# xaskasdf/ntransformer

Measured on AMD Instinct MI355X. Metric: decode tokens/sec (Llama-3.1-8B Q8_0 class, resident weights, greedy, batch 1), higher is better.
Workload: dtype f32; 1 GPU; Llama-3.1-8B-shaped Q8_0 GGUF tensors (seed 20260925), resident in HBM, 16-token prompt, greedy decode; ctx=4096, replicas=1, hipgraph=True

## Files before the change

### include/ntk_engine.h

```cpp
#ifndef NTK_ENGINE_H
#define NTK_ENGINE_H

#include "ntk.h"

#if defined(__GNUC__)
#pragma GCC visibility push(default)
#endif
#ifdef __cplusplus
extern "C" {
#endif

int ntk_rope_kv_store(float* q, const float* k, const float* v, const int* positions, int seq_len, int n_heads, int n_kv_heads, int head_dim,
                      float theta_base, float freq_scale, int interleaved, void* k_cache, void* v_cache, int start_pos, int max_seq, void* stream);
int ntk_rope_tab(float* q, float* k, const int* positions, int batch_size, int seq_len, int n_heads, int n_kv_heads, int head_dim, float theta_base,
                 float freq_scale, int interleaved, const float* inv_freq, void* stream);
int ntk_rope_kv_store_tab(float* q, const float* k, const float* v, const int* positions, int seq_len, int n_heads, int n_kv_heads, int head_dim,
                          float theta_base, float freq_scale, int interleaved, void* k_cache, void* v_cache, int start_pos, int max_seq,
                          const float* inv_freq, void* stream);
typedef struct ntk_gemv_seg {
    const void* W;
    float*      y;
    int         rows;
    int         dtype;
} ntk_gemv_seg;
// ... 17 lines not shown
#define NTK_ARENA_GATE 3
#define NTK_ARENA_HIDDEN_FLOATS 8192
#define NTK_ARENA_ATTN_FLOATS 8192
#define NTK_ARENA_GATE_FLOATS 32768
int ntk_decode_arena_acquire(void);
void ntk_decode_arena_release(int device);
float* ntk_decode_arena_slot(int slot);
int ntk_debug_gemv_static_x(void);

int ntk_debug_rp_prologue(uint8_t* out, const float* x, const float* norm_w, float eps, int in_features, int nsub, int nwaves, void* stream);
int ntk_debug_mfma_i8_probe(int* D, const int8_t* A, const int8_t* B, void* stream);

int ntk_attention_decode_fused(float* output, const float* q, const float* k, const float* v, void* k_cache,
                               void* v_cache, const int* d_pos, const float* inv_freq, int n_heads, int n_kv_heads,
                               int head_dim, int max_seq, float scale, float theta_base, float freq_scale,
                               void* stream);

size_t ntk_attention_split_scratch_bytes(int n_heads, int head_dim, int nsplit);
int ntk_attention_decode_split(float* output, const float* q, const float* k, const float* v, void* k_cache,
                               void* v_cache, const int* d_pos, const float* inv_freq, int n_heads, int n_kv_heads,
                               int head_dim, int max_seq, float scale, float theta_base, float freq_scale, int nsplit,
                               float* scratch, void* stream);
int ntk_attention_split_scratch_init(float* scratch, int n_heads, void* stream);
int ntk_attention_decode_split_merged(float* output, const float* q, const float* k, const float* v, void* k_cache,
                                      void* v_cache, const int* d_pos, const float* inv_freq, int n_heads, int n_kv_heads,
                                      int head_dim, int max_seq, float scale, float theta_base, float freq_scale, int nsplit,
                                      float* scratch, void* stream);

#define NTK_ATTN_BATCH_MAX 16
typedef struct ntk_kv_batch {
    void* k[NTK_ATTN_BATCH_MAX];
    void* v[NTK_ATTN_BATCH_MAX];
} ntk_kv_batch;
int ntk_attention_decode_batch(float* output, const float* q, const float* k, const float* v, const ntk_kv_batch* caches, const int* positions,
                               int n_rows, const float* inv_freq, int n_heads, int n_kv_heads, int head_dim, int max_seq, float scale,
                               float theta_base, float freq_scale, int nsplit, float* scratch, void* stream);

typedef struct ntk_kv_segments {
    int   n_seg;
    int   row0[NTK_ATTN_BATCH_MAX];
    int   n_rows[NTK_ATTN_BATCH_MAX];
    int   start_pos[NTK_ATTN_BATCH_MAX];
    void* k[NTK_ATTN_BATCH_MAX];
    void* v[NTK_ATTN_BATCH_MAX];
} ntk_kv_segments;
int ntk_kv_segments_validate(const ntk_kv_segments* segs, int total_rows, int max_seq);
int ntk_rope_kv_store_segments(float* q, const float* k, const float* v, const ntk_kv_segments* segs, int n_heads, int n_kv_heads, int head_dim,
                               float theta_base, float freq_scale, int interleaved, int max_seq, void* stream);
int ntk_rope_kv_store_segments_tab(float* q, const float* k, const float* v, const ntk_kv_segments* segs, int n_heads, int n_kv_heads, int head_dim,
                                   float theta_base, float freq_scale, int interleaved, int max_seq, const float* inv_freq, void* stream);
int ntk_attention_prefill_segments(float* output, const float* Q, const ntk_kv_segments* segs, int n_heads, int n_kv_heads, int head_dim, int max_seq,
                                   float scale, void* stream);

size_t ntk_kv_q8_cache_bytes(int max_seq, int n_kv_heads, int head_dim);
int ntk_kv_store_q8(void* k_cache, void* v_cache, const float* k, const float* v, int seq_len, int n_kv_heads, int head_dim, int start_pos,
                    int max_seq, void* stream);
int ntk_rope_kv_store_q8(float* q, const float* k, const float* v, const int* positions, int seq_len, int n_heads, int n_kv_heads, int head_dim,
                         float theta_base, float freq_scale, int interleaved, void* k_cache, void* v_cache, int start_pos, int max_seq,
                         void* stream);
int ntk_rope_kv_store_q8_tab(float* q, const float* k, const float* v, const int* positions, int seq_len, int n_heads, int n_kv_heads, int head_dim,
                             float theta_base, float freq_scale, int interleaved, void* k_cache, void* v_cache, int start_pos, int max_seq,
                             const float* inv_freq, void* stream);
int ntk_attention_decode_q8(float* output, const float* q, const float* k, const float* v, void* k_cache, void* v_cache, const int* d_pos,
                            const float* inv_freq, int n_heads, int n_kv_heads, int head_dim, int max_seq, float scale, float theta_base,
                            float freq_scale, int nsplit, float* scratch, void* stream);
int ntk_kv_dequant_q8_f16(void* k_f16, void* v_f16, const void* k_cache, const void* v_cache, int n_rows, int n_kv_heads, int head_dim,
                          int max_seq, void* stream);
int ntk_attention_decode_q8_batch(float* output, const float* q, const float* k, const float* v, const ntk_kv_batch* caches, const int* positions,
                                  int n_rows, const float* inv_freq, int n_heads, int n_kv_heads, int head_dim, int max_seq, float scale,
                                  float theta_base, float freq_scale, int nsplit, float* scratch, void* stream);

int ntk_kv_shift(uint16_t* k_cache, uint16_t* v_cache, int n_layers, int max_seq, int n_kv_heads, int head_dim, int src0, int dst0, int n_rows,
                 const float* inv_freq, float theta_base, float freq_scale, int interleaved, void* stream);
int ntk_kv_shift_q8(void* k_cache_q8, void* v_cache_q8, int n_layers, int max_seq, int n_kv_heads, int head_dim, int src0, int dst0, int n_rows,
                    const float* inv_freq, float theta_base, float freq_scale, int interleaved, void* stream);

int ntk_debug_gemv_fused_form(const ntk_gemv_seg* segs, int nseg, const float* x, int in_features, const float* norm_w, float eps,
                              const float* resid, int silu_pair, int integer_activations, void* stream);

size_t   ntk_tp_comm_bytes(size_t max_floats);
void*    ntk_tp_comm_alloc(size_t bytes);
int      ntk_tp_comm_reset(void* comm, void* stream);
float*   ntk_tp_slot(void* comm, size_t max_floats, unsigned call_index);
int      ntk_tp_allreduce_add(float* hidden, void* const* peers, int rank, int world, size_t max_floats, unsigned call_index, int n, void* stream);
int      ntk_tp_advance_epoch(void* comm, void* stream);
unsigned ntk_tp_error(void* comm);
int      ntk_ipc_export(void* devptr, void* handle64);
int      ntk_ipc_open(const void* handle64, void** devptr);
int      ntk_ipc_close(void* devptr);

int ntk_gemm_quant(float* Y, const void* W, const float* X, int n_tokens, int out_features, int in_features,
                   int weight_dtype, const float* resid, void* stream);

typedef struct ntk_gemm_partials {
    const float* part[3];
    float*       y[3];
    int          rows[3];
    int          nseg, n_tokens, nsplit;
} ntk_gemm_partials;
typedef struct ntk_gemm_desc {
    const ntk_gemv_seg* segs;
    int                 nseg;
    const float*        X;
    int                 n_tokens, in_features;
    const float*        resid;
    void*               workspace;
    size_t              workspace_bytes;
    int                 reuse_x;
    const float*        row_max;
    ntk_gemm_partials*  partials;
    int                 weights_repacked;
    int                 full_form;
} ntk_gemm_desc;
size_t ntk_gemm_quant_workspace_bytes(int in_features, int out_features);
int ntk_gemm_quant_f16(const ntk_gemm_desc* desc, void* stream);
int ntk_reduce_rmsnorm_rowmax(float* hidden, const ntk_gemm_partials* partials, const float* weight, float eps, float* x_out, float* row_max,
                              float* zero_tokens, void* stream);
int ntk_reduce_silu_mul_rowmax(float* output, const ntk_gemm_partials* partials, float* row_max, void* stream);
int ntk_rmsnorm_rowmax(float* output, const float* input, const float* weight, int n_tokens, int hidden_size, float eps, float* row_max,
                       float* zero_tokens, void* stream);
int ntk_silu_mul_rowmax(float* output, const float* gate, const float* up, int n_tokens, int width, float* row_max, void* stream);
int ntk_gemm_prepare_x(const float* X, int n_tokens, int in_features, void* workspace, void* stream);
int ntk_rmsnorm_prepare_x(float* output, const float* input, const float* weight, int n_tokens, int hidden_size, float eps, void* workspace, void* stream);
int ntk_reduce_rmsnorm_prepare_x(float* hidden, const ntk_gemm_partials* partials, const float* weight, float eps, float* x_out, void* workspace, void* stream);
int ntk_silu_mul_prepare_x(float* output, const float* gate, const float* up, int n_tokens, int width, void* workspace, void* stream);
int ntk_reduce_silu_mul_prepare_x(float* output, const ntk_gemm_partials* partials, void* workspace, void* stream);

size_t ntk_gemm_dense16_workspace_bytes(int in_features, int out_features, int dtype);
int ntk_gemm_dense16(const ntk_gemm_desc* desc, void* stream);

int ntk_embed_rows(float* out, const void* table, const int* tokens, int n_tokens, int hidden, int dtype,
                   void* stream);

int ntk_argmax(const float* logits, int n, int* d_out_token, int* h_mirror, float* scratch, void* stream);

int ntk_logprob_rows(const float* logits, int n_rows, int vocab, int ld, const int* targets, float* logprob, int* top1, void* stream);

size_t ntk_sample_scratch_bytes(int n);
int ntk_sample_top_k(float* logits, int n, const int* d_recent, int n_recent, float repeat_penalty, float temperature,
                     int top_k, float top_p, float r, int* d_out_token, int* h_mirror, void* scratch, void* stream);
int ntk_repeat_penalty(float* logits, int n, const int* d_recent, int n_recent, float repeat_penalty, void* stream);

#define NTK_SAMPLE_ROWS_MAX 16
typedef struct ntk_sample_rows {
    float temperature[NTK_SAMPLE_ROWS_MAX], top_p[NTK_SAMPLE_ROWS_MAX], repeat_penalty[NTK_SAMPLE_ROWS_MAX], r[NTK_SAMPLE_ROWS_MAX];
    int   top_k[NTK_SAMPLE_ROWS_MAX], n_recent[NTK_SAMPLE_ROWS_MAX];
} ntk_sample_rows;
size_t ntk_sample_rows_scratch_bytes(int n_rows, int vocab);
int ntk_sample_rows_top_k(float* logits, int n_rows, int vocab, int ld, const int* d_recent, int recent_ld, const ntk_sample_rows* rows, int* d_out,
                          int* h_mirror, void* scratch, void* stream);

int ntk_argmax_advance(const float* logits, int n, int* d_out_token, int* h_mirror, unsigned long long* h_ring4, int* d_pos,
                       float* scratch, void* stream);

int ntk_debug_sclk(unsigned long long* d_out2, void* stream);
int ntk_debug_sclk_begin(unsigned* d_flag, unsigned long long* d_out2, void* side_stream);
int ntk_debug_sclk_end(unsigned* d_flag, void* other_stream);

void ntk_debug_malloc_budget(long long bytes);

int ntk_advance_pos(int* d_pos, void* stream);

#ifdef __cplusplus
}
#endif
#if defined(__GNUC__)
#pragma GCC visibility pop
#endif
#endif
```

### ntransformer_amd/csrc/common.hip.h

```cpp
#pragma once
#include <hip/hip_runtime.h>
#include <stdint.h>
#include "../../include/ntk_engine.h"

#define NTK_WAVE 64

#define NTK_HIP_TRY(expr)                                   \
    do {                                                    \
        hipError_t e__ = (expr);                            \
        if (e__ != hipSuccess) return NTK_E_LAUNCH;         \
    } while (0)

#define NTK_EXTRA_API extern "C" __attribute__((visibility("default")))
#ifdef NTK_TUNE
#include <cstdlib>
#define NTK_TUNE_ENV_INT(name, dflt) ([] { const char* e__ = getenv(name); return e__ ? atoi(e__) : (dflt); }())
#else
#define NTK_TUNE_ENV_INT(name, dflt) (dflt)
#endif

namespace ntk {

hipStream_t resolve_stream(void* s);
int         last_launch_status();
int         q8l_gemv_fused(const ntk_gemv_seg* segs, int nseg, const float* x, int in, const float* norm_w, float eps, const float* resid,
                           int silu_pair, hipStream_t st);
int         dense16_gemv_fused(const ntk_gemv_seg* segs, int nseg, const float* x, int in, const float* norm_w, float eps, const float* resid,
                               int silu_pair, hipStream_t st);

__device__ __forceinline__ float h2f(uint16_t bits) {
    _Float16 h;
    __builtin_memcpy(&h, &bits, 2);
    return (float)h;
}
__device__ __forceinline__ uint16_t f2h(float f) {
    _Float16 h = (_Float16)f;
    uint16_t bits;
    __builtin_memcpy(&bits, &h, 2);
    return bits;
}

__device__ __forceinline__ void rope_rotate(const float a, const float b, const float c, const float s, float& ra, float& rb) {
#pragma clang fp contract(off)
    ra = a * c - b * s;
    rb = b * c + a * s;
}

__device__ __forceinline__ float rope_freq(const float* __restrict__ inv_freq, const int i, const int head_dim, const float theta) {
    return inv_freq ? inv_freq[i] : 1.0f / (float)pow((double)theta, (double)((2.0f * i) / head_dim));
}

template <int CTRL, int ROW_MASK>
__device__ __forceinline__ float dpp_or_zero(float v) {
    return __int_as_float(__builtin_amdgcn_update_dpp(0, __float_as_int(v), CTRL, ROW_MASK, 0xF, false));
}
template <int CTRL, int ROW_MASK>
__device__ __forceinline__ float dpp_or_self(float v) {
    return __int_as_float(__builtin_amdgcn_update_dpp(__float_as_int(v), __float_as_int(v), CTRL, ROW_MASK, 0xF, false));
}
constexpr int DPP_QUAD_1032 = 0xB1, DPP_QUAD_2301 = 0x4E, DPP_ROW_HALF_MIRROR = 0x141, DPP_ROW_MIRROR = 0x140,
              DPP_ROW_BCAST15 = 0x142, DPP_ROW_BCAST31 = 0x143;

__device__ __forceinline__ float wave_sum_lane63(float v) {
    v += dpp_or_zero<DPP_QUAD_1032, 0xF>(v);
    v += dpp_or_zero<DPP_QUAD_2301, 0xF>(v);
    v += dpp_or_zero<DPP_ROW_HALF_MIRROR, 0xF>(v);
    v += dpp_or_zero<DPP_ROW_MIRROR, 0xF>(v);
    v += dpp_or_zero<DPP_ROW_BCAST15, 0xA>(v);
    v += dpp_or_zero<DPP_ROW_BCAST31, 0xC>(v);
    return v;
}
__device__ __forceinline__ float wave_sum(float v) {
    return __int_as_float(__builtin_amdgcn_readlane(__float_as_int(wave_sum_lane63(v)), 63));
}
__device__ __forceinline__ float wave_max(float v) {
    v = fmaxf(v, dpp_or_self<DPP_QUAD_1032, 0xF>(v));
    v = fmaxf(v, dpp_or_self<DPP_QUAD_2301, 0xF>(v));
    v = fmaxf(v, dpp_or_self<DPP_ROW_HALF_MIRROR, 0xF>(v));
    v = fmaxf(v, dpp_or_self<DPP_ROW_MIRROR, 0xF>(v));
    v = fmaxf(v, dpp_or_self<DPP_ROW_BCAST15, 0xA>(v));
    v = fmaxf(v, dpp_or_self<DPP_ROW_BCAST31, 0xC>(v));
    return __int_as_float(__builtin_amdgcn_readlane(__float_as_int(v), 63));
}

template <int N>
__device__ __forceinline__ float group_sum(float v) {
    static_assert(N == 1 || N == 2 || N == 4 || N == 8 || N == 16 || N == 32, "group size");
    if constexpr (N >= 2) v += dpp_or_zero<DPP_QUAD_1032, 0xF>(v);
    if constexpr (N >= 4) v += dpp_or_zero<DPP_QUAD_2301, 0xF>(v);
    if constexpr (N >= 8) v += dpp_or_zero<DPP_ROW_HALF_MIRROR, 0xF>(v);
    if constexpr (N >= 16) v += dpp_or_zero<DPP_ROW_MIRROR, 0xF>(v);
    if constexpr (N >= 32) v += __shfl_xor(v, 16, 64);
    return v;
}

__device__ __forceinline__ float block_sum(float v, float* red) {
    const int lane = threadIdx.x & 63, wave = threadIdx.x >> 6, nw = (blockDim.x + 63) >> 6;
    v = wave_sum(v);
    __syncthreads();
    if (lane == 0) red[wave] = v;
    __syncthreads();
    float t = 0.0f;
    for (int i = 0; i < nw; ++i) t += red[i];
    return t;
}
__device__ __forceinline__ float block_max(float v, float* red) {
    const int lane = threadIdx.x & 63, wave = threadIdx.x >> 6, nw = (blockDim.x + 63) >> 6;
    v = wave_max(v);
    __syncthreads();
    if (lane == 0) red[wave] = v;
    __syncthreads();
    float t = red[0];
    for (int i = 1; i < nw; ++i) t = fmaxf(t, red[i]);
    return t;
}

template <int N>
__device__ __forceinline__ void lds_read_dwords(uint32_t (&dst)[N], const uint8_t* base, int off) {
    const int a = off & ~3;
    const uint32_t sh = (uint32_t)(off & 3);
    uint32_t w[N + 1];
#pragma unroll
    for (int i = 0; i <= N; ++i) w[i] = *reinterpret_cast<const uint32_t*>(base + a + 4 * i);
#pragma unroll
    for (int i = 0; i < N; ++i) dst[i] = __builtin_amdgcn_alignbyte(w[i + 1], w[i], sh);
}
__device__ __forceinline__ uint16_t lds_u16_at(const uint8_t* base, int off) {
    return *reinterpret_cast<const uint16_t*>(base + off);
}

__device__ __forceinline__ float ub2f(uint32_t w, int k) { return (float)((w >> (8 * k)) & 0xFFu); }
__device__ __forceinline__ float sb2f(uint32_t w, int k) { return (float)(int)(int8_t)(w >> (8 * k)); }

__device__ __forceinline__ void kq_scale_min(uint32_t s0, uint32_t s1, uint32_t s2, int j, float& sc, float& mn) {
    const uint64_t lo = (uint64_t)s0 | ((uint64_t)s1 << 32);
    auto byte = [&](int n) -> uint32_t {
        return n < 8 ? (uint32_t)((lo >> (8 * n)) & 0xFFu) : ((s2 >> (8 * (n - 8))) & 0xFFu);
    };
    uint32_t s, m;
    if (j < 4) {
        s = byte(j) & 63u;
        m = byte(j + 4) & 63u;
    } else {
        s = (byte(j + 4) & 0xFu) | ((byte(j - 4) >> 6) << 4);
        m = (byte(j + 4) >> 4) | ((byte(j) >> 6) << 4);
    }
    sc = (float)s;
    mn = (float)m;
}

}
```

### ntransformer_amd/csrc/elementwise.hip

```cpp
#include "common.hip.h"
#include <cfloat>

namespace ntk {

template <bool HALF_OUT>
__global__ __launch_bounds__(1024) void rmsnorm_kernel(void* __restrict__ output, const float* __restrict__ input,
                                                       const float* __restrict__ weight, int hidden, float eps) {
    __shared__ float red[16];
    const float* x = input + (size_t)blockIdx.x * hidden;
    float ssq = 0.0f;
    for (int i = threadIdx.x; i < hidden; i += blockDim.x) ssq = fmaf(x[i], x[i], ssq);
    const float tot = block_sum(ssq, red);
    const float rms_inv = 1.0f / sqrtf(tot / (float)hidden + eps);
    for (int i = threadIdx.x; i < hidden; i += blockDim.x) {
        const float v = x[i] * rms_inv * weight[i];
        if constexpr (HALF_OUT) reinterpret_cast<uint16_t*>(output)[(size_t)blockIdx.x * hidden + i] = f2h(v);
        else reinterpret_cast<float*>(output)[(size_t)blockIdx.x * hidden + i] = v;
    }
}

template <bool MASKED>
__global__ __launch_bounds__(1024) void softmax_kernel(float* __restrict__ out, const float* __restrict__ in,
                                                       const uint8_t* __restrict__ mask, int cols) {
    __shared__ float red[16];
    const float* x = in + (size_t)blockIdx.x * cols;
    const uint8_t* mk = MASKED ? mask + (size_t)blockIdx.x * cols : nullptr;
    float* y = out + (size_t)blockIdx.x * cols;
    float m = -FLT_MAX;
    for (int i = threadIdx.x; i < cols; i += blockDim.x)
        if (!MASKED || mk[i]) m = fmaxf(m, x[i]);
    m = block_max(m, red);
    float l = 0.0f;
    for (int i = threadIdx.x; i < cols; i += blockDim.x)
        if (!MASKED || mk[i]) l += expf(x[i] - m);
    l = block_sum(l, red);
    const float inv = l > 0.0f ? 1.0f / l : 0.0f;
    for (int i = threadIdx.x; i < cols; i += blockDim.x) y[i] = (!MASKED || mk[i]) ? expf(x[i] - m) * inv : 0.0f;
}

__global__ void silu_mul_kernel(float* __restrict__ out, const float* __restrict__ gate, const float* __restrict__ up, int n) {
    const int i = blockIdx.x * blockDim.x + threadIdx.x;
    if (i < n) {
        const float g = gate[i];
        out[i] = g / (1.0f + expf(-g)) * up[i];
    }
}
__global__ void add_kernel(float* __restrict__ o, const float* __restrict__ a, const float* __restrict__ b, int n) {
    const int i = blockIdx.x * blockDim.x + threadIdx.x;
    if (i < n) o[i] = a[i] + b[i];
}
__global__ void copy_kernel(float* __restrict__ d, const float* __restrict__ s, int n) {
    const int i = blockIdx.x * blockDim.x + threadIdx.x;
    if (i < n) d[i] = s[i];
}
__global__ void gemm_f32_kernel(float* __restrict__ C, const float* __restrict__ A, const float* __restrict__ B, int M, int N, int K) {
    const int col = blockIdx.x * blockDim.x + threadIdx.x, row = blockIdx.y * blockDim.y + threadIdx.y;
    if (row >= M || col >= N) return;
    float s = 0.0f;
    for (int k = 0; k < K; ++k) s = fmaf(A[(size_t)row * K + k], B[(size_t)col * K + k], s);
    C[(size_t)row * N + col] = s;
}
__global__ __launch_bounds__(256) void cosine_kernel(float* __restrict__ result, const float* __restrict__ a,
                                                     const float* __restrict__ b, int n) {
    __shared__ float red[16];
    float d = 0.0f, na = 0.0f, nb = 0.0f;
    for (int i = threadIdx.x; i < n; i += blockDim.x) {
        d = fmaf(a[i], b[i], d); na = fmaf(a[i], a[i], na); nb = fmaf(b[i], b[i], nb);
    }
    d = block_sum(d, red); na = block_sum(na, red); nb = block_sum(nb, red);
    if (threadIdx.x == 0) {
        const float den = sqrtf(na) * sqrtf(nb);
        *result = den > 1e-8f ? d / den : 0.0f;
    }
}

__device__ float embed_elem(const uint8_t* __restrict__ table, int tok, int hidden, int dt, int e) {
    switch (dt) {
        case NTK_DT_F32: return reinterpret_cast<const float*>(table)[(size_t)tok * hidden + e];
        case NTK_DT_F16: return h2f(reinterpret_cast<const uint16_t*>(table)[(size_t)tok * hidden + e]);
        case NTK_DT_BF16: return __uint_as_float((uint32_t)reinterpret_cast<const uint16_t*>(table)[(size_t)tok * hidden + e] << 16);
        case NTK_DT_Q8_0: {
            const uint8_t* b = table + ((size_t)tok * (hidden / 32) + e / 32) * 34;
            const float d = h2f((uint16_t)(b[0] | (b[1] << 8)));
            return __fmul_rn(d, (float)(int8_t)b[2 + (e & 31)]);
        }
        case NTK_DT_Q4_0: {
            const uint8_t* b = table + ((size_t)tok * (hidden / 32) + e / 32) * 18;
            const float d = h2f((uint16_t)(b[0] | (b[1] << 8)));
            const int j = e & 31;
            const int nib = j < 16 ? (b[2 + j] & 0x0F) : (b[2 + j - 16] >> 4);
            return __fmul_rn(d, (float)(nib - 8));
        }
        case NTK_DT_Q4_K: {
            const uint8_t* b = table + ((size_t)tok * (hidden / 256) + e / 256) * 144;
            const float d = h2f((uint16_t)(b[0] | (b[1] << 8))), dmin = h2f((uint16_t)(b[2] | (b[3] << 8)));
            const int w = e & 255, sub = w >> 5, l = w & 31, chunk = sub >> 1;
            const uint8_t* s = b + 4;
            uint32_t sc, mn;
            if (sub < 4) { sc = s[sub] & 63; mn = s[sub + 4] & 63; }
            else { sc = (s[sub + 4] & 0x0F) | ((s[sub - 4] >> 6) << 4); mn = (s[sub + 4] >> 4) | ((s[sub] >> 6) << 4); }
            const uint8_t qb = b[16 + 32 * chunk + l];
            const int nib = (sub & 1) ? (qb >> 4) : (qb & 0x0F);
            return __fsub_rn(__fmul_rn(__fmul_rn(d, (float)sc), (float)nib), __fmul_rn(dmin, (float)mn));
        }
        case NTK_DT_Q6_K: {
            const uint8_t* b = table + ((size_t)tok * (hidden / 256) + e / 256) * 210;
            const float d = h2f((uint16_t)(b[208] | (b[209] << 8)));
            const int w = e & 255, hf = w >> 7, g = (w >> 5) & 3, l = w & 31, is = l >> 4;
            const uint8_t* ql = b + 64 * hf;
            const uint8_t* qh = b + 128 + 32 * hf;
            const int8_t sc = (int8_t)b[192 + 8 * hf + is + 2 * g];
            const uint8_t qlb = ql[l + 32 * (g & 1)];
            const int lo = (g >> 1) ? (qlb >> 4) : (qlb & 0x0F);
            const int q = (lo | (((qh[l] >> (2 * g)) & 3) << 4)) - 32;
            return __fmul_rn(__fmul_rn(d, (float)sc), (float)q);
        }
        default: return 0.0f;
    }
}
__global__ void embed_rows_kernel(float* __restrict__ out, const uint8_t* __restrict__ table, const int* __restrict__ tokens,
                                  int hidden, int dt) {
    const int tok = tokens[blockIdx.x];
    const int e = blockIdx.y * blockDim.x + threadIdx.x;
    if (e < hidden) out[(size_t)blockIdx.x * hidden + e] = embed_elem(table, tok, hidden, dt, e);
}

__device__ __forceinline__ void amax_merge(float& v, int& i, float ov, int oi) {
    if (ov > v || (ov == v && oi < i)) { v = ov; i = oi; }
}
__global__ __launch_bounds__(256) void argmax_stage1(const float* __restrict__ x, int n, float* __restrict__ sv, int* __restrict__ si) {
    __shared__ float rv[4];
    __shared__ int ri[4];
    float v = -FLT_MAX;
    int idx = 0x7FFFFFFF;
    for (int i = blockIdx.x * blockDim.x + threadIdx.x; i < n; i += gridDim.x * blockDim.x) amax_merge(v, idx, x[i], i);
    for (int off = 32; off > 0; off >>= 1) amax_merge(v, idx, __shfl_xor(v, off, 64), __shfl_xor(idx, off, 64));
    if ((threadIdx.x & 63) == 0) { rv[threadIdx.x >> 6] = v; ri[threadIdx.x >> 6] = idx; }
    __syncthreads();
    if (threadIdx.x == 0) {
        for (int w = 1; w < 4; ++w) amax_merge(v, idx, rv[w], ri[w]);
        sv[blockIdx.x] = v; si[blockIdx.x] = idx;
    }
}
__global__ __launch_bounds__(256) void argmax_stage2(const float* __restrict__ sv, const int* __restrict__ si, int nblk,
                                                     int* __restrict__ d_out, int* __restrict__ h_mirror) {
    __shared__ float rv[4];
    __shared__ int ri[4];
    float v = -FLT_MAX;
    int idx = 0x7FFFFFFF;
    for (int i = threadIdx.x; i < nblk; i += blockDim.x) amax_merge(v, idx, sv[i], si[i]);
    for (int off = 32; off > 0; off >>= 1) amax_merge(v, idx, __shfl_xor(v, off, 64), __shfl_xor(idx, off, 64));
    if ((threadIdx.x & 63) == 0) { rv[threadIdx.x >> 6] = v; ri[threadIdx.x >> 6] = idx; }
    __syncthreads();
    if (threadIdx.x == 0) {
        for (int w = 1; w < 4; ++w) amax_merge(v, idx, rv[w], ri[w]);
        if (idx == 0x7FFFFFFF) idx = 0;
        *d_out = idx;
        if (h_mirror) *h_mirror = idx;
    }
}
__global__ void advance_pos_kernel(int* p) { if (threadIdx.x == 0 && blockIdx.x == 0) *p += 1; }

__global__ __launch_bounds__(64) void sclk_probe_kernel(unsigned long long* out) {
    const unsigned long long t0 = __builtin_amdgcn_s_memtime(), r0 = __builtin_amdgcn_s_memrealtime();
    unsigned long long r1 = r0;
    float acc = (float)threadIdx.x;
    while (r1 - r0 < 5000ull) {
#pragma unroll
        for (int i = 0; i < 64; ++i) acc = fmaf(acc, 1.0000001f, 1e-9f);
        r1 = __builtin_amdgcn_s_memrealtime();
    }
    const unsigned long long t1 = __builtin_amdgcn_s_memtime();
    if (threadIdx.x == 0) { out[0] = t1 - t0; out[1] = r1 - r0; }
    if (acc == 12345.678f) out[2] = 0;
}

__global__ __launch_bounds__(64) void sclk_span_kernel(const unsigned* flag, unsigned long long* out) {
    const unsigned long long t0 = __builtin_amdgcn_s_memtime(), r0 = __builtin_amdgcn_s_memrealtime();
    unsigned long long r1 = r0;
    for (;;) {
        __builtin_amdgcn_s_sleep(64);
        r1 = __builtin_amdgcn_s_memrealtime();
        if (__hip_atomic_load(flag, __ATOMIC_RELAXED, __HIP_MEMORY_SCOPE_SYSTEM) != 0u || r1 - r0 > 300000000ull) break;
    }
    const unsigned long long t1 = __builtin_amdgcn_s_memtime();
    if (threadIdx.x == 0) { out[0] = t1 - t0; out[1] = r1 - r0; }
}

__global__ __launch_bounds__(256) void argmax_advance_stage2(const float* __restrict__ sv, const int* __restrict__ si, int nblk,
                                                             int* __restrict__ d_out, int* __restrict__ h_mirror,
                                                             unsigned long long* __restrict__ h_ring, int* __restrict__ d_pos) {
    __shared__ float rv[4];
    __shared__ int ri[4];
    float v = -FLT_MAX;
    int idx = 0x7FFFFFFF;
    for (int i = threadIdx.x; i < nblk; i += blockDim.x) amax_merge(v, idx, sv[i], si[i]);
    for (int off = 32; off > 0; off >>= 1) amax_merge(v, idx, __shfl_xor(v, off, 64), __shfl_xor(idx, off, 64));
    if ((threadIdx.x & 63) == 0) { rv[threadIdx.x >> 6] = v; ri[threadIdx.x >> 6] = idx; }
    __syncthreads();
    if (threadIdx.x == 0) {
        for (int w = 1; w < 4; ++w) amax_merge(v, idx, rv[w], ri[w]);
        if (idx == 0x7FFFFFFF) idx = 0;
        const int pos = *d_pos;
        *d_out = idx;
        if (h_mirror) *h_mirror = idx;
        if (h_ring)
            __hip_atomic_store(h_ring + (pos & 3), (unsigned long long)(unsigned)idx | ((unsigned long long)(unsigned)(pos + 1) << 32),
                               __ATOMIC_RELEASE, __HIP_MEMORY_SCOPE_SYSTEM);
        *d_pos = pos + 1;
    }
}

static inline dim3 g1(int n) { return dim3((n + 255) / 256); }

}

extern "C" {
using namespace ntk;

static int rms_block(int hidden) { return hidden <= 1024 ? 256 : (hidden <= 4096 ? 512 : 1024); }

int ntk_rmsnorm(float* output, const float* input, const float* weight, int batch_size, int hidden_size, float eps, void* stream) {
    if (!output || !input || !weight) return NTK_E_NULL;
    if (batch_size < 0 || hidden_size <= 0) return NTK_E_SHAPE;
    if (batch_size == 0) return NTK_OK;
    hipLaunchKernelGGL(rmsnorm_kernel<false>, dim3(batch_size), dim3(rms_block(hidden_size)), 0, resolve_stream(stream),
                       (void*)output, input, weight, hidden_size, eps);
    return last_launch_status();
}
int ntk_rmsnorm_f16(void* output, const float* input, const float* weight, int batch_size, int hidden_size, float eps, void* stream) {
    if (!output || !input || !weight) return NTK_E_NULL;
    if (batch_size < 0 || hidden_size <= 0) return NTK_E_SHAPE;
    if (batch_size == 0) return NTK_OK;
    hipLaunchKernelGGL(rmsnorm_kernel<true>, dim3(batch_size), dim3(rms_block(hidden_size)), 0, resolve_stream(stream),
                       output, input, weight, hidden_size, eps);
    return last_launch_status();
}
int ntk_softmax(float* output, const float* input, int rows, int cols, void* stream) {
    if (!output || !input) return NTK_E_NULL;
    if (rows < 0 || cols <= 0) return NTK_E_SHAPE;
    if (rows == 0) return NTK_OK;
    hipLaunchKernelGGL(softmax_kernel<false>, dim3(rows), dim3(cols <= 1024 ? 256 : 1024), 0, resolve_stream(stream), output,
                       input, (const uint8_t*)nullptr, cols);
    return last_launch_status();
}
int ntk_masked_softmax(float* output, const float* input, const uint8_t* mask, int rows, int cols, void* stream) {
    if (!output || !input || !mask) return NTK_E_NULL;
    if (rows < 0 || cols <= 0) return NTK_E_SHAPE;
    if (rows == 0) return NTK_OK;
    hipLaunchKernelGGL(softmax_kernel<true>, dim3(rows), dim3(cols <= 1024 ? 256 : 1024), 0, resolve_stream(stream), output,
                       input, mask, cols);
    return last_launch_status();
}
int ntk_gemm_f32(float* C, const float* A, const float* B, int M, int N, int K, void* stream) {
    if (!C || !A || !B) return NTK_E_NULL;
    if (M < 0 || N < 0 || K < 0) return NTK_E_SHAPE;
    if (M == 0 || N == 0) return NTK_OK;
    hipLaunchKernelGGL(gemm_f32_kernel, dim3((N + 15) / 16, (M + 15) / 16), dim3(16, 16), 0, resolve_stream(stream), C, A, B, M, N, K);
    return last_launch_status();
}
int ntk_silu_mul(float* output, const float* gate, const float* up, int size, void* stream) {
    if (!output || !gate || !up) return NTK_E_NULL;
    if (size < 0) return NTK_E_SHAPE;
    if (size == 0) return NTK_OK;
    hipLaunchKernelGGL(silu_mul_kernel, g1(size), dim3(256), 0, resolve_stream(stream), output, gate, up, size);
    return last_launch_status();
}
int ntk_add(float* out, const float* a, const float* b, int size, void* stream) {
    if (!out || !a || !b) return NTK_E_NULL;
    if (size < 0) return NTK_E_SHAPE;
    if (size == 0) return NTK_OK;
    hipLaunchKernelGGL(add_kernel, g1(size), dim3(256), 0, resolve_stream(stream), out, a, b, size);
    return last_launch_status();
}
int ntk_add_inplace(float* a, const float* b, int size, void* stream) { return ntk_add(a, a, b, size, stream); }
int ntk_add_bias(float* y, const float* bias, int size, void* stream) { return ntk_add(y, y, bias, size, stream); }
int ntk_copy(float* dst, const float* src, int size, void* stream) {
    if (!dst || !src) return NTK_E_NULL;
    if (size < 0) return NTK_E_SHAPE;
    if (size == 0) return NTK_OK;
    hipLaunchKernelGGL(copy_kernel, g1(size), dim3(256), 0, resolve_stream(stream), dst, src, size);
    return last_launch_status();
}
int ntk_cosine_similarity(float* result, const float* a, const float* b, int size, void* stream) {
    if (!result || !a || !b) return NTK_E_NULL;
    if (size < 0) return NTK_E_SHAPE;
    hipLaunchKernelGGL(cosine_kernel, dim3(1), dim3(256), 0, resolve_stream(stream), result, a, b, size);
    return last_launch_status();
}
int ntk_embed_rows(float* out, const void* table, const int* tokens, int n_tokens, int hidden, int dtype, void* stream) {
    if (!out || !table || !tokens) return NTK_E_NULL;
    if (n_tokens < 0 || hidden <= 0) return NTK_E_SHAPE;
    if (n_tokens == 0) return NTK_OK;
    hipLaunchKernelGGL(embed_rows_kernel, dim3(n_tokens, (hidden + 255) / 256), dim3(256), 0, resolve_stream(stream), out, (const uint8_t*)table,
                       tokens, hidden, dtype);
    const int st = last_launch_status();
    if (st != NTK_OK) return st;
    switch (dtype) {
        case NTK_DT_F32: case NTK_DT_F16: case NTK_DT_BF16: case NTK_DT_Q8_0: case NTK_DT_Q4_0: case NTK_DT_Q4_K: case NTK_DT_Q6_K: return NTK_OK;
        default: return NTK_E_DTYPE;
    }
}
int ntk_argmax(const float* logits, int n, int* d_out_token, int* h_mirror, float* scratch, void* stream) {
    if (!logits || !d_out_token || !scratch) return NTK_E_NULL;
    if (n <= 0) return NTK_E_SHAPE;
    const int nblk = n < 256 * 8 ? 1 : (n / (256 * 8) < 1024 ? n / (256 * 8) : 1024);
    float* sv = scratch;
    int* si = reinterpret_cast<int*>(scratch + 1024);
    hipStream_t st = resolve_stream(stream);
    hipLaunchKernelGGL(argmax_stage1, dim3(nblk), dim3(256), 0, st, logits, n, sv, si);
    hipLaunchKernelGGL(argmax_stage2, dim3(1), dim3(256), 0, st, (const float*)sv, (const int*)si, nblk, d_out_token, h_mirror);
    return last_launch_status();
}
int ntk_argmax_advance(const float* logits, int n, int* d_out_token, int* h_mirror, unsigned long long* h_ring4, int* d_pos, float* scratch,
                       void* stream) {
    if (!logits || !d_out_token || !scratch || !d_pos) return NTK_E_NULL;
    if (n <= 0) return NTK_E_SHAPE;
    const int nblk = n < 256 * 8 ? 1 : (n / (256 * 8) < 1024 ? n / (256 * 8) : 1024);
    float* sv = scratch;
    int* si = reinterpret_cast<int*>(scratch + 1024);
    hipStream_t st = resolve_stream(stream);
    hipLaunchKernelGGL(argmax_stage1, dim3(nblk), dim3(256), 0, st, logits, n, sv, si);
    hipLaunchKernelGGL(argmax_advance_stage2, dim3(1), dim3(256), 0, st, (const float*)sv, (const int*)si, nblk, d_out_token, h_mirror, h_ring4, d_pos);
    return last_launch_status();
}
int ntk_debug_sclk(unsigned long long* d_out2, void* stream) {
    if (!d_out2) return NTK_E_NULL;
    hipLaunchKernelGGL(sclk_probe_kernel, dim3(1), dim3(64), 0, resolve_stream(stream), d_out2);
    return last_launch_status();
}
int ntk_debug_sclk_begin(unsigned* d_flag, unsigned long long* d_out2, void* side_stream) {
    if (!d_flag || !d_out2 || !side_stream) return NTK_E_NULL;
    hipStream_t st = static_cast<hipStream_t>(side_stream);
    if (hipMemsetAsync(d_flag, 0, 4, st) != hipSuccess) return NTK_E_LAUNCH;
    hipLaunchKernelGGL(sclk_span_kernel, dim3(1), dim3(64), 0, st, (const unsigned*)d_flag, d_out2);
    return last_launch_status();
}
int ntk_debug_sclk_end(unsigned* d_flag, void* other_stream) {
    if (!d_flag || !other_stream) return NTK_E_NULL;
    static const unsigned one = 1u;
    return hipMemcpyAsync(d_flag, &one, 4, hipMemcpyHostToDevice, static_cast<hipStream_t>(other_stream)) == hipSuccess ? NTK_OK : NTK_E_LAUNCH;
}
int ntk_advance_pos(int* d_pos, void* stream) {
    if (!d_pos) return NTK_E_NULL;
    hipLaunchKernelGGL(advance_pos_kernel, dim3(1), dim3(64), 0, resolve_stream(stream), d_pos);
    return last_launch_status();
}

}
```

### ntransformer_amd/csrc/engine/capi.cpp

```cpp
#include "../../../include/ntransformer.h"
#include "../../../include/ntk_engine.h"
#include "engine.h"

#include <cstdlib>
#include <cstring>
#include <new>
#include <thread>

using nt::Engine;

namespace {
Engine* E(nt_engine_t e) { return static_cast<Engine*>(e); }
nt::SynthSpec to_spec(const nt_synth_spec& s) {
    nt::SynthSpec o;
    o.hidden = s.hidden; o.inter = s.inter; o.layers = s.layers; o.heads = s.heads; o.kv_heads = s.kv_heads;
    o.vocab = s.vocab; o.ctx = s.ctx; o.eps = s.eps; o.theta = s.theta; o.bos = s.bos; o.eos = s.eos;
    o.mix = s.mix ? s.mix : "Q8_0";
    o.seed = s.seed;
    return o;
}
int threads_or_default(int n) {
    if (n > 0) return n;
    const int h = (int)std::thread::hardware_concurrency();
    return h > 0 ? h : 8;
}
}

extern "C" {

nt_engine_t nt_engine_create(void) { return new (std::nothrow) Engine(); }
void nt_engine_destroy(nt_engine_t e) { delete E(e); }

int nt_engine_load(nt_engine_t e, const char* path) { return nt_engine_load_ex(e, path, 4096); }

int nt_engine_load_ex(nt_engine_t e, const char* path, int max_context) {
    if (!e || !path) return NTK_E_NULL;
    try { return E(e)->load(path, max_context > 0 ? max_context : 4096); } catch (...) { return NTK_E_NOMEM; }
}

int nt_engine_load_synthetic(nt_engine_t e, const nt_synth_spec* spec, int max_context) {
    if (!e || !spec) return NTK_E_NULL;
    try { return E(e)->load_synthetic(to_spec(*spec), max_context > 0 ? max_context : 4096); } catch (...) { return NTK_E_NOMEM; }
}

int nt_engine_load_shared(nt_engine_t e, nt_engine_t src, int max_context) {
    if (!e || !src || e == src) return NTK_E_NULL;
    try { return E(e)->load_shared(*E(src), max_context > 0 ? max_context : 4096); } catch (...) { return NTK_E_NOMEM; }
}

int nt_engine_set_option(nt_engine_t e, const char* key, const char* value) {
    if (!e || !key || !value) return NTK_E_NULL;
    const bool on = atoi(value) != 0;
    const std::string k = key;
    auto before_load = [&](auto set) -> int {
        if (E(e)->loaded()) { E(e)->set_error(k + " must be set before the model is loaded"); return NTK_E_SHAPE; }
        const int rc = set();
        if (rc != NTK_OK) E(e)->set_error(E(e)->model().error());
        return rc;
    };
    if (k == "fused") E(e)->options().fused = on;
    else if (k == "graph") E(e)->options().graph = on;
    else if (k == "batched_prefill") { E(e)->options().batched_prefill = on; E(e)->model().set_batched_prefill(on); }
    else if (k == "device_sampling") E(e)->options().device_sampling = on;
    else if (k == "f16_prefill" || k == "bf16_prefill") E(e)->model().set_bf16_prefill(on);
    else if (k == "dense_fused") {
        const std::string v = value;
        if (v != "0" && v != "1") { E(e)->set_error("dense_fused must be 0 or 1"); return NTK_E_SHAPE; }
        return E(e)->model().set_dense_fused(on);
    }
    else if (k == "dense_mfma16") {
        const std::string v = value;
        if (v != "0" && v != "1") { E(e)->set_error("dense_mfma16 must be 0 or 1"); return NTK_E_SHAPE; }
        E(e)->model().set_dense_mfma16(on);
    }
    else if (k == "persistent" || k == "fuse_attention") {
        if (on) fprintf(stderr, "note: \"%s\" selected an experiment that lost to the fused launches and was removed (profiles/NEGATIVE_RESULTS.md); the option does nothing\n", key);
    }
    else if (k == "kv_cache") return before_load([&] { return E(e)->model().set_kv_cache(value); });
    else if (k == "rope_scaling") return before_load([&] { return E(e)->model().set_rope_scaling(value); });
    else if (k == "rope_freq_base") return before_load([&] { return E(e)->model().set_rope_freq_base(value); });
    else if (k == "rope_freq_scale") return before_load([&] { return E(e)->model().set_rope_freq_scale(value); });
    else if (k == "sequences") return before_load([&] { return E(e)->model().set_sequences(atoi(value)); });
    else if (k == "batch_kv_q8") {
        const std::string v = value;
        if (v != "0" && v != "1") { E(e)->set_error("batch_kv_q8 must be 0 or 1"); return NTK_E_SHAPE; }
        return before_load([&] { return E(e)->model().set_batch_kv_q8(on); });
    }
    else if (k == "static_activations") {
        const std::string v = value;
        if (v != "0" && v != "1") { E(e)->set_error("static_activations must be 0 or 1"); return NTK_E_SHAPE; }
        return before_load([&] { return E(e)->model().set_static_activations(on); });
    }
    else if (k == "batch_prefill") {
        const std::string v = value;
        if (v != "0" && v != "1") { E(e)->set_error("batch_prefill must be 0 or 1"); return NTK_E_SHAPE; }
        E(e)->options().batch_prefill = on;
    }
    else if (k == "context_shift") {
        const std::string v = value;
        if (v != "0" && v != "1") { E(e)->set_error("context_shift must be 0 or 1"); return NTK_E_SHAPE; }
        E(e)->options().context_shift = on;
    }
    else if (k == "context_keep") {
        char* end = nullptr;
        const long n = strtol(value, &end, 10);
        if (end == value || *end != 0 || n < 0 || n > 0x7FFFFFFF) { E(e)->set_error("context_keep must be an integer >= 0"); return NTK_E_SHAPE; }
        E(e)->options().context_keep = (int)n;
    }
    else if (k == "prefill_row_max") E(e)->model().set_prefill_row_max(on);
    else if (k == "prefill_fused_split") E(e)->model().set_prefill_fused_split(on);
    else if (k == "attention_merge") return E(e)->model().set_attention_merge(on);
    else if (k == "repack") return E(e)->model().set_repack(atoi(value));
    else if (k == "score_rows") {
        const int rc = E(e)->model().set_score_rows(atoi(value));
        if (rc != NTK_OK) E(e)->set_error(E(e)->model().error());
        return rc;
    }
    else if (k == "synth_threads") E(e)->options().synth_threads = atoi(value);
    else return NTK_E_SHAPE;
    return NTK_OK;
}

const char* nt_engine_last_error(nt_engine_t e) { return e ? E(e)->error().c_str() : "null engine"; }

void nt_gen_params_default(nt_gen_params* p) {
    if (!p) return;
    const nt::GenerateConfig d;
    p->max_tokens = d.max_tokens; p->temperature = d.temperature; p->top_k = d.top_k; p->top_p = d.top_p;
    p->repeat_penalty = d.repeat_penalty; p->repeat_window = d.repeat_window; p->seed = d.seed; p->stop_at_eos = 1;
}

char* nt_engine_generate(nt_engine_t e, const char* prompt, int max_tokens, float temperature, int top_k, float top_p) {
    if (!e || !prompt || !E(e)->loaded()) return nullptr;
    try {
        nt::GenerateConfig c;
        c.max_tokens = max_tokens; c.temperature = temperature; c.top_k = top_k; c.top_p = top_p;
        c.verbose = false;
        const std::string out = E(e)->generate(prompt, c);
        char* r = static_cast<char*>(malloc(out.size() + 1));
        if (!r) return nullptr;
        memcpy(r, out.c_str(), out.size() + 1);
        return r;
    } catch (...) { return nullptr; }
}
void nt_free(char* p) { free(p); }

int nt_engine_vocab_size(nt_engine_t e) { return e && E(e)->loaded() ? E(e)->model().config().vocab_size : -1; }
int nt_engine_n_layers(nt_engine_t e) { return e && E(e)->loaded() ? E(e)->model().config().n_layers : -1; }
int nt_engine_hidden_size(nt_engine_t e) { return e && E(e)->loaded() ? E(e)->model().config().hidden_size : -1; }
int nt_engine_max_context(nt_engine_t e) { return e && E(e)->loaded() ? E(e)->model().config().max_seq_len : -1; }

int nt_engine_generate_tokens(nt_engine_t e, const int* prompt, int n_prompt, const nt_gen_params* p, int* out, int out_cap) {
    if (!e || !prompt || !p || (!out && out_cap > 0)) return NTK_E_NULL;
    if (n_prompt <= 0) return NTK_E_SHAPE;
    try {
        nt::GenerateConfig c;
        c.max_tokens = p->max_tokens; c.temperature = p->temperature; c.top_k = p->top_k; c.top_p = p->top_p;
        c.repeat_penalty = p->repeat_penalty; c.repeat_window = p->repeat_window; c.seed = p->seed;
        std::vector<int> gen;
        const int rc = E(e)->generate_tokens(std::vector<int>(prompt, prompt + n_prompt), c, gen, p->stop_at_eos != 0);
        if (rc != NTK_OK) return rc;
        const int n = (int)std::min<size_t>(gen.size(), (size_t)out_cap);
        for (int i = 0; i < n; ++i) out[i] = gen[i];
        return n;
    } catch (...) { return NTK_E_NOMEM; }
}

int nt_engine_last_stats(nt_engine_t e, nt_stats* o) {
    if (!e || !o) return NTK_E_NULL;
    const nt::Stats& s = E(e)->last_stats();
    o->prompt_tokens = s.prompt_tokens; o->gen_tokens = s.gen_tokens; o->prefill_ms = s.prefill_ms;
    o->decode_ms = s.decode_ms; o->decode_tok_s = s.decode_tok_s();
    return NTK_OK;
}

int nt_engine_forward(nt_engine_t e, const int* tokens, int n, int start_pos, float* logits_out) {
    if (!e || !tokens || !logits_out) return NTK_E_NULL;
    if (!E(e)->loaded()) return NTK_E_NULL;
    float* d = E(e)->model().forward(tokens, n, start_pos);
    if (!d) return NTK_E_LAUNCH;
    return E(e)->model().copy_logits(logits_out);
}

int nt_engine_seq_forward(nt_engine_t e, int slot, const int* tokens, int n, int start_pos, float* logits_out) {
    if (!e || !tokens || !logits_out) return NTK_E_NULL;
    if (!E(e)->loaded()) return NTK_E_NULL;
    if (slot < 0 || slot >= E(e)->model().sequences()) { E(e)->set_error("seq_forward: no such sequence slot"); return NTK_E_SHAPE; }
    float* d = E(e)->model().forward(tokens, n, start_pos, slot);
    if (!d) { E(e)->set_error(E(e)->model().error()); return NTK_E_LAUNCH; }
    return E(e)->model().copy_logits(logits_out);
}

int nt_engine_decode_batch(nt_engine_t e, const int* slots, const int* tokens, const int* positions, int n, float* logits_out, int* next_out) {
    if (!e || !E(e)->loaded()) return NTK_E_NULL;
    try {
        const int rc = E(e)->model().decode_batch(slots, tokens, positions, n, logits_out, next_out);
        if (rc != NTK_OK) E(e)->set_error(E(e)->model().error());
        return rc;
    } catch (...) { return NTK_E_NOMEM; }
}

int nt_engine_forward_batch(nt_engine_t e, const int* slots, const int* tokens, const int* lens, const int* start_pos, int n, float* logits_out,
                            int* next_out) {
    if (!e || !E(e)->loaded()) return NTK_E_NULL;
    try {
        E(e)->model().set_batched_prefill(E(e)->options().batched_prefill);
        const int rc = E(e)->model().forward_batch(slots, tokens, lens, start_pos, n, logits_out, next_out);
        if (rc != NTK_OK) E(e)->set_error(E(e)->model().error());
        return rc;
    } catch (...) { return NTK_E_NOMEM; }
}

int nt_forward_batch_validate(const int* slots, const int* lens, const int* start_pos, int n, int sequences, int max_seq) {
    return nt::Model::validate_forward_batch(slots, lens, start_pos, n, sequences, max_seq, nullptr);
}

int nt_engine_generate_batch(nt_engine_t e, const int* const* prompts, const int* prompt_lens, int n, const nt_gen_params* p, int* out, int out_stride,
                             int* out_counts) {
    if (!e || !prompts || !prompt_lens || !p || !out || !out_counts) return NTK_E_NULL;
    try { return E(e)->generate_batch(prompts, prompt_lens, n, *p, out, out_stride, out_counts); } catch (...) { return NTK_E_NOMEM; }
}

int nt_engine_decode_batch_sample(nt_engine_t e, const int* slots, const int* tokens, const int* positions, int n, const nt_gen_params* params,
                                  const int* const* recent, const int* n_recent, const float* r, float* logits_out, int* next_out) {
    if (!e || !E(e)->loaded()) return NTK_E_NULL;
    try { return E(e)->decode_batch_sample(slots, tokens, positions, n, params, recent, n_recent, r, logits_out, next_out); } catch (...) { return NTK_E_NOMEM; }
}

int nt_engine_generate_batch_ex(nt_engine_t e, const int* const* prompts, const int* prompt_lens, int n, const nt_gen_params* params, int* out, int out_stride,
                                int* out_counts) {
    if (!e || !prompts || !prompt_lens || !params || !out || !out_counts) return NTK_E_NULL;
    try { return E(e)->generate_batch_ex(prompts, prompt_lens, n, params, out, out_stride, out_counts); } catch (...) { return NTK_E_NOMEM; }
}

int nt_engine_kv_shift(nt_engine_t e, int slot, int keep, int discard, int n_past) {
    if (!e || !E(e)->loaded()) return NTK_E_NULL;
    try {
        const int rc = E(e)->model().kv_shift(slot, keep, discard, n_past);
        if (rc < 0) E(e)->set_error(E(e)->model().error());
        return rc;
    } catch (...) { return NTK_E_NOMEM; }
}

int nt_engine_kv_copy(nt_engine_t e, int src_slot, int dst_slot, int pos0, int n) {
    if (!e || !E(e)->loaded()) return NTK_E_NULL;
    try {
        const int rc = E(e)->model().kv_copy(src_slot, dst_slot, pos0, n);
        if (rc < 0) E(e)->set_error(E(e)->model().error());
        return rc;
    } catch (...) { return NTK_E_NOMEM; }
}

int nt_kv_shift_validate(int slot, int keep, int discard, int n_past, int sequences, int max_seq) {
    return nt::Model::validate_kv_shift(slot, keep, discard, n_past, sequences, max_seq, nullptr);
}
int nt_kv_copy_validate(int src_slot, int dst_slot, int pos0, int n, int sequences, int max_seq) {
    return nt::Model::validate_kv_copy(src_slot, dst_slot, pos0, n, sequences, max_seq, nullptr);
}
int nt_context_shift_discard(int n_past, int keep) { return nt::Model::context_shift_discard(n_past, keep); }

int nt_batch_validate(const int* slots, const int* tokens, const int* positions, int n, int sequences, int max_seq, int vocab) {
    return nt::Model::validate_batch(slots, tokens, positions, n, sequences, max_seq, vocab, nullptr);
}

// ... 293 lines not shown
```

### ntransformer_amd/csrc/engine/model.cpp

```cpp
#include "model_impl.h"
#include <thread>

namespace nt {

Model::~Model() { free_all(); }

void Model::drop_graphs() {
    for (auto& row : graphs_)
        for (auto& g : row) {
            if (g) (void)hipGraphExecDestroy(reinterpret_cast<hipGraphExec_t>(g));
            g = nullptr;
        }
}

void* Model::dev_alloc(size_t bytes, bool zero) {
    void* p = nt_hip_malloc(bytes + 256);
    if (!p) return nullptr;
    allocs_.push_back(p);
    if (zero) nt_hip_memset(p, 0, bytes);
    return p;
}

void Model::dev_free(void* p) {
    if (!p) return;
    allocs_.erase(std::remove(allocs_.begin(), allocs_.end(), p), allocs_.end());
    nt_hip_free(p);
}

void Model::free_all() {
    drop_graphs();
    for (int r = 0; r < 8; ++r) {
        if (tp_peer_opened_[r] && tp_peers_[r]) (void)ntk_ipc_close(tp_peers_[r]);
        tp_peers_[r] = nullptr;
        tp_peer_opened_[r] = false;
    }
    tp_connected_ = false;
    tp_comm_ = nullptr;
    tp_call_ = 0;
    if (own_stream_ && stream_) (void)hipStreamDestroy(static_cast<hipStream_t>(stream_));
    own_stream_ = false;
    stream_ = nullptr;
    for (void* p : allocs_) nt_hip_free(p);
    allocs_.clear();
    if (arena_owner_) ntk_decode_arena_release(arena_device_);
    arena_owner_ = false;
    arena_device_ = -1;
    hidden1_ = arena_attn_ = arena_gate_ = nullptr;
    auto free_host = [](auto*& p) { if (p) nt_hip_free_host(p); p = nullptr; };
    free_host(h_token_); free_host(h_ring_); free_host(h_recent_); free_host(h_batch_recent_); free_host(h_batch_next_);
    sample_scratch_ = gemm_ws_ = gemm_ws2_ = nullptr;
    d_recent_ = nullptr;
    shares_weights_ = false;
    layers_.clear();
    token_embd_ = output_norm_ = output_ = DevTensor();
    weight_bytes_ = repack_bytes_ = raw_freed_bytes_ = 0;
    raw_scratch_ = nullptr; raw_scratch_bytes_ = raw_cursor_ = 0; raw_err_ = 0;
    repack_done_ = output_tied_ = false;
    host_pos_ = attn_regime_ = 0;
    kv_.reset();
    rope_factors_.clear();
    batch_logits_ = batch_logprob_ = batch_attn_scratch_ = nullptr; batch_in_ = batch_next_ = batch_recent_ = nullptr; batch_sample_scratch_ = nullptr;
    kv_capture_ = nullptr; kv_capture_layer_ = -1; kv_capture_T_ = 0;
    hidden_ = residual_ = workspace_ = logits_ = argmax_scratch_ = rope_inv_freq_ = attn_scratch_ = row_max_ = nullptr;
    positions_ = tokens_dev_ = d_pos_ = d_token_ = nullptr;
    score_logits_ = score_logprob_ = nullptr; score_targets_ = score_top1_ = nullptr; score_cap_ = 0;
    score_ws_ = nullptr; score_ws_bytes_ = 0;
}

int Model::share_weights(const Model& src, int max_context) {
    if (&src == this) { err_ = "share_weights: a model cannot share its own weights"; return NTK_E_NULL; }
    free_all();
    if (src.layers_.empty()) { err_ = "share_weights: the source model is not loaded"; return NTK_E_NULL; }
    if (src.tp_world_ != 1 || src.shares_weights_) {
        err_ = "share_weights: the source must hold whole tensors of its own (no tensor parallelism, not itself a sharing sequence)";
        return NTK_E_SHAPE;
    }
    cfg_ = src.cfg_;
    rope_factors_ = src.rope_factors_;
    cfg_full_ = src.cfg_;
    if (max_context > 0) cfg_.max_seq_len = max_context;
    vocab_ = src.vocab_;
    layers_ = src.layers_;
    token_embd_ = src.token_embd_; output_norm_ = src.output_norm_; output_ = src.output_;
    output_tied_ = src.output_tied_;
    weight_bytes_ = src.weight_bytes_;
    repack_ = src.repack_; repack_wanted_ = src.repack_; repack_done_ = true;
    repack_bytes_ = 0;
    shares_weights_ = true;
    if (src.raw_freed_bytes_ > 0 && src.raw_scratch_bytes_ > 0) {
        void* d = dev_alloc(src.raw_scratch_bytes_, false);
        if (!d) { err_ = "share_weights: no device memory for the unpack scratch"; free_all(); return NTK_E_NOMEM; }
        raw_scratch_ = d; raw_scratch_bytes_ = src.raw_scratch_bytes_;
        raw_freed_bytes_ = src.raw_freed_bytes_;
    }
    int rc = own_stream();
    if (rc == NTK_OK) rc = alloc_buffers();
    if (rc != NTK_OK) free_all();
    return rc;
}

int Model::set_attention_merge(bool on) {
    if (on == attn_merge_) return NTK_OK;
    if (!layers_.empty()) {
        NT_TRY(sync());
        drop_graphs();
    }
    attn_merge_ = on;
    return NTK_OK;
}

int Model::set_dense_fused(bool on) {
    if (on == dense_fused_) return NTK_OK;
    if (!layers_.empty()) {
        NT_TRY(sync());
        drop_graphs();
    }
    dense_fused_ = on;
    return NTK_OK;
}

bool Model::fusable(int dt) const { return is_quant(dt) || (dense_fused_ && is_dense16(dt)); }

int Model::set_repack(int level) {
    level = level < 0 ? 0 : level > 3 ? 3 : level;
    if (shares_weights_) { err_ = "set_repack: this sequence shares another model's tensors"; return NTK_E_SHAPE; }
    repack_wanted_ = level;
    if (layers_.empty()) { repack_ = level; return NTK_OK; }
    if (level == 3) level = 2;
    if (level == repack_) return NTK_OK;
    NT_TRY(sync());
    drop_graphs();
    int rc = NTK_OK;
    if (level < 2 && raw_freed_bytes_ > 0) rc = restore_raw_all();
    if (rc == NTK_OK && level > 0 && !repack_done_) {
        rc = repack_all();
        if (rc == NTK_E_NOMEM) { fprintf(stderr, "warning: decode repack incomplete (device memory): the rest stays on the raw path\n"); rc = NTK_OK; err_.clear(); }
    }
    if (rc != NTK_OK) { err_ = std::string("set_repack: ") + ntk_status_string(rc); return rc; }
    repack_ = level;
    if (level == 2) rc = drop_raw_all();
    return rc;
}

uint64_t Model::bytes_per_token(int pos) const {
    uint64_t b = 0;
    for (const auto& L : layers_)
        for (auto m : kLayerMatrices) b += (L.*m).nbytes;
    b += output_.nbytes;
    b += (uint64_t)(2 * cfg_.n_layers + 1) * cfg_.hidden_size * 4;
    const uint64_t kv_row = kv_.row_bytes();
    b += 2ull * cfg_.n_layers * kv_row * (uint64_t)(pos + 1) + 2ull * cfg_.n_layers * kv_row;
    b += ntk_row_bytes(token_embd_.dtype, cfg_.hidden_size);
    return b;
}

int Model::set_device_token(int token) {
    if (token < 0 || token >= cfg_.vocab_size) { err_ = "token id out of range"; return NTK_E_SHAPE; }
    *h_token_ = token;
    return ntk_memcpy_h2d_async(d_token_, h_token_, 4, stream_);
}
int Model::set_device_pos(int pos) {
    host_pos_ = pos;
    NT_TRY(ntk_memcpy_h2d_async(d_pos_, &pos, 4, stream_));
    NT_TRY(ntk_stream_synchronize(stream_));
    if (h_ring_) memset(h_ring_, 0, 64);
    return NTK_OK;
}
int Model::sync() { return ntk_stream_synchronize(stream_); }
int Model::host_token() const { return *h_token_; }
int Model::copy_logits(float* host) {
    NT_TRY(ntk_memcpy_d2h_async(host, logits_, (size_t)cfg_.vocab_size * 4, stream_));
    return ntk_stream_synchronize(stream_);
}

int Model::sample_on_device(const int* recent, int n_recent, float repeat_penalty, float temperature, int top_k, float top_p, float r) {
    if (!sample_scratch_ || !d_recent_ || !h_recent_) return NTK_E_NOMEM;
    if (n_recent > kRecentCap) { recent += n_recent - kRecentCap; n_recent = kRecentCap; }
    void* s = stream_;
    if (repeat_penalty > 1.0f && n_recent > 0) {
        memcpy(h_recent_, recent, (size_t)n_recent * 4);
        NT_TRY(ntk_memcpy_h2d_async(d_recent_, h_recent_, (size_t)n_recent * 4, s));
    } else {
        n_recent = 0;
    }
    if (temperature <= 0.0f) {
        NT_TRY(ntk_repeat_penalty(logits_, cfg_.vocab_size, d_recent_, n_recent, repeat_penalty, s));
        return ntk_argmax(logits_, cfg_.vocab_size, d_token_, h_token_, argmax_scratch_, s);
    }
    return ntk_sample_top_k(logits_, cfg_.vocab_size, d_recent_, n_recent, repeat_penalty, temperature, top_k, top_p, r, d_token_,
                            h_token_, sample_scratch_, s);
}

int Model::wait_token(int pos, int* token) {
    volatile unsigned long long* slot = h_ring_ + (pos & 3);
    const unsigned want = (unsigned)(pos + 1);
    for (unsigned spins = 0;; ++spins) {
        const unsigned long long v = *slot;
        if ((unsigned)(v >> 32) == want) { *token = (int)(unsigned)v; return NTK_OK; }
#if defined(__x86_64__) || defined(__i386__)
        __builtin_ia32_pause();
#else
        std::this_thread::yield();
#endif
        if ((spins & 0xFFFFu) == 0xFFFFu) {
            const auto now = std::chrono::steady_clock::now();
            if (spins == 0xFFFFu) wait_t0_ = now;
            else if (std::chrono::duration<double>(now - wait_t0_).count() > 2.0) break;
        }
    }
    static bool warned = false;
    if (!warned) { warned = true; fprintf(stderr, "warning: the pinned token ring was not seen updating for 2 s (host memory not coherent with a running kernel?); falling back to a stream synchronisation per token\n"); }
    NT_TRY(ntk_stream_synchronize(stream_));
    const unsigned long long v = *slot;
    if ((unsigned)(v >> 32) != want) { err_ = "decode step finished without publishing its token"; return NTK_E_LAUNCH; }
    *token = (int)(unsigned)v;
    return NTK_OK;
}

int Model::set_sequences(int n) {
    if (n < 1 || n > kMaxSequences) { err_ = "sequences must lie in 1 .. " + std::to_string(kMaxSequences); return NTK_E_SHAPE; }
    sequences_ = n;
    return NTK_OK;
}

int Model::set_batch_kv_q8(bool on) {
    if (!layers_.empty()) { err_ = "batch_kv_q8 must be set before the model is loaded"; return NTK_E_SHAPE; }
    batch_kv_q8_ = on;
    return NTK_OK;
}

int Model::set_static_activations(bool on) {
    if (!layers_.empty()) { err_ = "static_activations must be set before the model is loaded"; return NTK_E_SHAPE; }
    static_act_ = on;
    return NTK_OK;
}

int Model::set_kv_cache(const std::string& kind) {
    if (kind != "f16" && kind != "q8_0") { err_ = "kv_cache: unknown format '" + kind + "' (f16 or q8_0)"; return NTK_E_DTYPE; }
    if (!layers_.empty()) { err_ = "kv_cache must be set before the model is loaded"; return NTK_E_SHAPE; }
    const bool q8 = kind == "q8_0";
    kv_q8_ = q8;
    return NTK_OK;
}

int Model::set_rope_scaling(const std::string& text) {
    if (!layers_.empty()) { err_ = "rope_scaling must be set before the model is loaded"; return NTK_E_SHAPE; }
    RopeScalingOption o;
    if (!parse_rope_scaling(text, &o, &err_)) return NTK_E_SHAPE;
    rope_opt_ = o;
    return NTK_OK;
}

int Model::set_rope_freq_base(const std::string& text) {
    if (!layers_.empty()) { err_ = "rope_freq_base must be set before the model is loaded"; return NTK_E_SHAPE; }
    if (!parse_positive_float(text, &rope_base_opt_)) { err_ = "rope_freq_base must be a number > 0"; return NTK_E_SHAPE; }
    return NTK_OK;
}

int Model::set_rope_freq_scale(const std::string& text) {
    if (!layers_.empty()) { err_ = "rope_freq_scale must be set before the model is loaded"; return NTK_E_SHAPE; }
    if (!parse_positive_float(text, &rope_scale_opt_)) { err_ = "rope_freq_scale must be a number > 0"; return NTK_E_SHAPE; }
    return NTK_OK;
}

int Model::resolve_rope(const GgufFile* f) {
    rope_factors_.clear();
    const int half = cfg_.head_dim / 2;
    if (rope_base_opt_ > 0.0f) cfg_.rope_theta = rope_base_opt_;
    const bool file_factors = rope_opt_.mode == RopeScalingOption::FILE || rope_opt_.mode == RopeScalingOption::LINEAR;
    const GgufTensor* t = f && file_factors ? f->find("rope_freqs.weight") : nullptr;
    if (t) {
        if (t->dtype != NTK_DT_F32 || !t->known_type) { err_ = "rope_freqs.weight must be F32"; return NTK_E_DTYPE; }
        if (t->numel() != half) {
            err_ = "rope_freqs.weight holds " + std::to_string(t->numel()) + " factors, head_dim / 2 = " + std::to_string(half) + " are needed";
            return NTK_E_SHAPE;
        }
        rope_factors_.resize((size_t)half);
        memcpy(rope_factors_.data(), f->data(*t), (size_t)half * 4);
        for (int i = 0; i < half; ++i)
            if (!std::isfinite(rope_factors_[i]) || !(rope_factors_[i] > 0.0f)) {
                err_ = "rope_freqs.weight: factor " + std::to_string(i) + " is not a finite number > 0";
                rope_factors_.clear();
                return NTK_E_SHAPE;
            }
    }
    switch (rope_opt_.mode) {
        case RopeScalingOption::FILE:
            if (cfg_.rope_scaling_type != "none" && cfg_.rope_scaling_type != "linear")
                fprintf(stderr, "note: RoPE scaling type '%s' is not applied: the model runs with unscaled positions\n", cfg_.rope_scaling_type.c_str());
            break;
        case RopeScalingOption::NONE:
            cfg_.rope_freq_scale = 1.0f; cfg_.rope_scaling_type = "none"; cfg_.rope_orig_ctx = 0;
            break;
        case RopeScalingOption::LINEAR:
            cfg_.rope_freq_scale = 1.0f / rope_opt_.factor; cfg_.rope_scaling_type = "linear"; cfg_.rope_orig_ctx = 0;
            break;
        case RopeScalingOption::LLAMA3: {
            rope_factors_.resize((size_t)half);
            const int st = rope_llama3_factors(cfg_.head_dim, cfg_.rope_theta, rope_opt_.factor, rope_opt_.low, rope_opt_.high, rope_opt_.orig_ctx, rope_factors_.data());
            if (st != NTK_OK) { rope_factors_.clear(); err_ = "rope_scaling: llama3 factors cannot be computed for this model"; return st; }
            cfg_.rope_freq_scale = 1.0f; cfg_.rope_scaling_type = "llama3"; cfg_.rope_orig_ctx = rope_opt_.orig_ctx;
            break;
        }
    }
    if (!rope_factors_.empty() && cfg_.head_dim != 64 && cfg_.head_dim != 128 && cfg_.head_dim != 256) {
        rope_factors_.clear();
        err_ = "RoPE frequency factors (rope_freqs.weight / rope_scaling=llama3) need head_dim 64, 128 or 256 (this model: " + std::to_string(cfg_.head_dim) + ")";
        return NTK_E_SHAPE;
    }
    if (rope_scale_opt_ > 0.0f) cfg_.rope_freq_scale = rope_scale_opt_;
    cfg_.rope_factors = (int)rope_factors_.size();
    return NTK_OK;
}

const char* Model::decode_path() const {
    return arena_owner_ ? "fused (5 launches/layer; static activations)" : "fused (5 launches/layer)";
}

Model::Views Model::views(int T, bool fused) const {
    const size_t qd = (size_t)T * cfg_.n_heads * cfg_.head_dim, kvd = (size_t)T * cfg_.n_kv_heads * cfg_.head_dim;
    float* const q = workspace_;
    Views v{q, q + qd, q + qd + kvd, q + qd + 2 * kvd, workspace_, workspace_ + (size_t)T * cfg_.intermediate_size};
    if (fused && T == 1 && arena_owner_) { v.attn_out = arena_attn_; v.gate = arena_gate_; }
    return v;
}

int Model::init_device() {
    const char* e = getenv("NTK_DEVICE");
    const int st = ntk_device_init(e ? atoi(e) : 0);
    if (st != NTK_OK) err_ = "no usable GPU (HIP device init failed)";
    return st;
}

int Model::own_stream() {
    hipStream_t own = nullptr;
    if (hipStreamCreateWithFlags(&own, hipStreamNonBlocking) != hipSuccess) { err_ = "stream creation failed"; return NTK_E_LAUNCH; }
    stream_ = own;
    own_stream_ = true;
    return NTK_OK;
}

}
```

### ntransformer_amd/csrc/engine/model.h

```cpp
#pragma once
#include <algorithm>
#include <array>
#include <chrono>
#include <cstdint>
#include <string>
#include <vector>
#include "gguf.h"
#include "kv_cache.h"
#include "rope_scaling.h"
#include "synth.h"

struct ntk_sample_rows;
struct ntk_kv_segments;

struct ihipGraphExec_t;

namespace nt {

struct DevTensor {
    void* ptr = nullptr;
    int dtype = 0;
    int64_t in_f = 0, out_f = 0;
    size_t nbytes = 0;
    void* rp = nullptr;
    size_t rp_bytes = 0;
};

struct PassStatus;

struct LayerWeights {
    DevTensor attn_norm, wq, wk, wv, wo, ffn_norm, w_gate, w_up, w_down;
};
inline constexpr std::array<DevTensor LayerWeights::*, 7> kLayerMatrices = {&LayerWeights::wq, &LayerWeights::wk, &LayerWeights::wv, &LayerWeights::wo,
                                                                            &LayerWeights::w_gate, &LayerWeights::w_up, &LayerWeights::w_down};

enum Shard { WHOLE, ROWS, COLS };

class Model {
public:
    Model() = default;
    ~Model();
    Model(const Model&) = delete;
    Model& operator=(const Model&) = delete;

    int load(const std::string& gguf_path, int max_context);
    int load_synthetic(const SynthSpec& spec, int max_context, int nthreads);
    int share_weights(const Model& src, int max_context);

    float* forward(const int* tokens, int seq_len, int start_pos, int slot = 0);

    int score(const int* tokens, const int* targets, int seq_len, int start_pos, float* logprob_out, int* top1_out, int slot = 0);

    static constexpr int kMaxSequences = 16;
    int set_sequences(int n);
    int sequences() const { return sequences_; }
    int set_batch_kv_q8(bool on);
    int set_static_activations(bool on);
    bool static_activations_active() const { return arena_owner_; }
    bool batch_kv_q8() const { return batch_kv_q8_; }
    int decode_batch(const int* slots, const int* tokens, const int* positions, int B, float* logits_out, int* next_out);
    static constexpr int kMaxRecent = 4096;
    int decode_batch_sample(const int* slots, const int* tokens, const int* positions, int B, const ntk_sample_rows& rows, const int* const* recent,
                            float* logits_out, float* const* row_logits, int* next_out);
    static int validate_batch(const int* slots, const int* tokens, const int* positions, int B, int sequences, int max_seq, int vocab, std::string* why);
    int forward_batch(const int* slots, const int* tokens_flat, const int* lens, const int* start_pos, int n, float* logits_out, int* next_out);
    static int validate_forward_batch(const int* slots, const int* lens, const int* start_pos, int n, int sequences, int max_seq, std::string* why);
    int kv_shift(int slot, int keep, int discard, int n_past);
    int kv_copy(int src_slot, int dst_slot, int pos0, int n);
    static int validate_kv_shift(int slot, int keep, int discard, int n_past, int sequences, int max_seq, std::string* why);
    static int validate_kv_copy(int src_slot, int dst_slot, int pos0, int n, int sequences, int max_seq, std::string* why);
    static int context_shift_discard(int n_past, int keep) { return std::max(1, (n_past - keep) / 2); }
    int set_score_rows(int rows);

    int decode_step_fused(bool greedy, bool use_graph);
    int set_device_token(int token);
    int set_device_pos(int pos);
    static constexpr int kAttnRegimes = 3;
    static int attention_regime(int pos, int head_dim) {
        if (pos < 544) return 0;
        return pos < (head_dim == 128 ? 3072 : 16384) ? 1 : 2;
    }
    static int attention_splits(int regime, int head_dim) { return regime <= 1 ? 8 : head_dim == 128 ? 32 : 16; }
    static constexpr int kMaxAttnSplits = 32;
    void pick_attention_regime();
    int sync();
    int host_token() const;
    int wait_token(int pos, int* token);
    float* logits_ptr() { return logits_; }
    int copy_logits(float* host);
    int sample_on_device(const int* recent, int n_recent, float repeat_penalty, float temperature, int top_k, float top_p, float r);
    static bool device_sampler_supports(float temperature, int top_k, int vocab) {
        return temperature <= 0.0f || (top_k > 0 && top_k <= 64 && top_k < vocab && vocab <= 131072);
    }

    const ModelConfig& config() const { return cfg_; }
    const GgufVocab& vocab() const { return vocab_; }
    const std::string& error() const { return err_; }
    uint64_t weight_bytes() const { return weight_bytes_; }
    uint64_t bytes_per_token(int pos) const;
    void set_batched_prefill(bool on) { batched_prefill_ = on; }
    int set_kv_cache(const std::string& kind);
    int set_rope_scaling(const std::string& text);
    int set_rope_freq_base(const std::string& text);
    int set_rope_freq_scale(const std::string& text);
    int rope_factor_count() const { return (int)rope_factors_.size(); }
    bool kv_q8() const { return kv_q8_; }
    static int kv_q8_splits(int regime) { return regime == 0 ? 4 : regime == 1 ? 16 : 32; }
    uint64_t kv_cache_bytes() const { return kv_.bytes(); }
    int debug_kv_inputs_capture(int layer);
    int debug_kv_inputs_read(int n, float* k, float* v);
    int debug_kv_q8(int layer, int pos0, int n, uint8_t* k_blocks, uint8_t* v_blocks, bool write, int slot = 0);
    void set_prefill_row_max(bool on) { prefill_row_max_ = on; }
    void set_prefill_fused_split(bool on) { prefill_fused_split_ = on; }
    int set_attention_merge(bool on);
    int set_repack(int level);
    bool repack() const { return repack_ != 0; }
    int repack_level() const { return repack_; }
    uint64_t repack_bytes() const { return repack_bytes_; }
    uint64_t resident_weight_bytes() const { return weight_bytes_ - raw_freed_bytes_ + repack_bytes_ + raw_scratch_bytes_; }
    int set_dense_fused(bool on);
    void set_dense_mfma16(bool on) { dense_mfma16_ = on; }
    bool fusable(int dt) const;
    void set_bf16_prefill(bool on) { bf16_prefill_ = on; }
    const char* decode_path() const;
    int check_tp();
    int debug_run_layers(const float* hidden_in, int T, int start_pos, int first, int count, int mode, float* hidden_out);
    int debug_kv(int layer, int pos0, int n, uint16_t* k, uint16_t* v, bool write, int slot = 0);
    int profile_token(float ms[4], int calls[4], bool coarse);
    void* stream() const { return stream_; }

    int tp_configure(int rank, int world);
    int tp_rank() const { return tp_rank_; }
    int tp_world() const { return tp_world_; }
    int tp_export(void* handle64, void** raw);
    int tp_connect(const void* handles, void* const* raws);
    unsigned tp_error();
    static int slice_columns(void* dst, const void* src, int dtype, int64_t out_f, int64_t in_f, int rank, int world);

private:
    int load_impl(const std::string& gguf_path, int max_context);
    int finish_load();
    int resolve_rope(const GgufFile* f);
    int init_device();
    int own_stream();
    int alloc_buffers();
    int upload(DevTensor& dst, const void* host, int dtype, int64_t in_f, int64_t out_f, size_t nbytes);
    int upload_shard(DevTensor& dst, const void* host_full, int dtype, int64_t in_f, int64_t out_f, size_t nbytes_full, Shard how);
    struct TensorSlot { DevTensor* dst; Shard how; int64_t in_f, out_f; };
    bool slot_of(const std::string& name, TensorSlot* slot);
    template <class F> void for_each_projection(F&& fn) { for (auto& L : layers_) for (auto m : kLayerMatrices) fn(L.*m); fn(output_); }
    int repack_all();
    int repack_one(DevTensor& t);
    int drop_raw_all();
    int restore_raw_all();
    void raw_begin() { raw_cursor_ = 0; }
    const void* raw_of(const DevTensor& t);
    int tp_check_shapes();
    int tp_allreduce(float* hidden, int n);
    float* tp_slot() const;
    void free_all();
    void drop_graphs();
    struct Views { float *q, *k, *v, *attn_out, *gate, *up; };
    Views views(int T, bool fused = false) const;
    int enqueue_token(bool greedy);
    int enqueue_layers(int first, int last);
    int decode_project(const DevTensor* const* ws, float* const* ys, int n, const float* x, const DevTensor* norm, const float* resid, int kind,
                       int silu_pair = 0, bool timed = true);
    struct KvTarget { int slot; const int* slots; int max_pos; const ntk_kv_segments* segs; };
    int layers_1to1(int T, int start_pos, int first, int last, const KvTarget& kv = KvTarget{0, nullptr, 0, nullptr});
    int attend(int layer, int T, int start_pos, const KvTarget& kv, const Views& act, bool fused_store);
    int embed_rows(float* out, const int* ids_dev, int n);
    int upload_positions(int T, int start_pos);
    const float* final_norm(float* dst, const float* src, int n, PassStatus& ok);
    int finish_pass(const char* failed, int rc);
    int gemv_logged(float* y, const DevTensor& w, const void* wp, const float* x);
    int lm_head(float* logits, const float* X, int n, const float* row_max);
    bool lm_head_f16() const;
    int lm_head_workspace(const char* who);
    int batch_buffers();
    int batch_logits(const int* slots, const int* tokens, const int* positions, int B);
    int batch_sample_buffers();
    int score_buffers();
    void* dev_alloc(size_t bytes, bool zero);
    void dev_free(void* p);
    template <class T> void dev_release(T*& p) { dev_free(p); p = nullptr; }
    template <class T> bool dev_need(T*& p, size_t bytes, bool zero) { if (!p) p = static_cast<T*>(dev_alloc(bytes, zero)); return p != nullptr; }
    void prof_mark(int cls, bool begin);

    ModelConfig cfg_;
    GgufVocab vocab_;
    std::string err_;
    std::vector<LayerWeights> layers_;
    DevTensor token_embd_, output_norm_, output_;
    bool output_tied_ = false;
    uint64_t weight_bytes_ = 0;
    std::vector<void*> allocs_;
    bool shares_weights_ = false;

    KvCache kv_;
    bool kv_q8_ = false;
    int sequences_ = 1;
    float* batch_logits_ = nullptr;
    int* batch_in_ = nullptr;
    int batch_host_[3 * 16] = {};
    std::vector<int> packed_tokens_;
    float* batch_logprob_ = nullptr;
    int* batch_next_ = nullptr;
    float* batch_attn_scratch_ = nullptr;
    int* batch_recent_ = nullptr;
    int* h_batch_recent_ = nullptr;
    void* batch_sample_scratch_ = nullptr;
    int* h_batch_next_ = nullptr;
    bool batch_kv_q8_ = false;
    float* kv_capture_ = nullptr;
    int kv_capture_layer_ = -1, kv_capture_T_ = 0;
    float* hidden_ = nullptr;
    float* hidden1_ = nullptr;
    bool static_act_ = true;
    bool arena_owner_ = false;
    int arena_device_ = -1;
    float* arena_attn_ = nullptr;
    float* arena_gate_ = nullptr;
    float* residual_ = nullptr;
    float* workspace_ = nullptr;
    size_t workspace_floats_ = 0;
    float* logits_ = nullptr;
    int score_rows_ = 256;
    float* score_logits_ = nullptr;
    int score_cap_ = 0;
    int* score_targets_ = nullptr;
    float* score_logprob_ = nullptr;
    int* score_top1_ = nullptr;
    void* score_ws_ = nullptr;
    size_t score_ws_bytes_ = 0;
    int* positions_ = nullptr;
    std::vector<int> host_positions_;
    int* tokens_dev_ = nullptr;
    int* d_pos_ = nullptr;
    int* d_token_ = nullptr;
    int* h_token_ = nullptr;
    unsigned long long* h_ring_ = nullptr;
    std::chrono::steady_clock::time_point wait_t0_;
    float* argmax_scratch_ = nullptr;
    void* sample_scratch_ = nullptr;
    int* d_recent_ = nullptr;
    int* h_recent_ = nullptr;
    static constexpr int kRecentCap = kMaxRecent;
    float* rope_inv_freq_ = nullptr;
    std::vector<float> rope_factors_;
    const float* rope_tab() const { return rope_factors_.empty() ? nullptr : rope_inv_freq_; }
    RopeScalingOption rope_opt_;
    float rope_base_opt_ = 0.0f, rope_scale_opt_ = 0.0f;
    void* stream_ = nullptr;
    bool batched_prefill_ = true;
    struct Timed { int cls; void* a; void* b; int n; bool shared_a; };
    bool prof_coarse_ = false;
    std::vector<Timed>* prof_ = nullptr;
    ihipGraphExec_t* graphs_[2][kAttnRegimes] = {};
    int host_pos_ = 0;
    int attn_regime_ = 0;
    float* attn_scratch_ = nullptr;
    bool prefill_row_max_ = true;
    float* row_max_ = nullptr;
    void* gemm_ws_ = nullptr;
    void* gemm_ws2_ = nullptr;
    bool prefill_fused_split_ = true;
    size_t gemm_ws_bytes_ = 0;
    bool bf16_prefill_ = true;
    bool dense_fused_ = true;
    bool dense_mfma16_ = true;
    int repack_ = 3;
    int repack_wanted_ = 3;
    bool repack_done_ = false;
    uint64_t repack_bytes_ = 0;
    uint64_t raw_freed_bytes_ = 0;
    void* raw_scratch_ = nullptr;
    size_t raw_scratch_bytes_ = 0, raw_cursor_ = 0;
    int raw_err_ = 0;
    bool attn_merge_ = false;
    int tp_rank_ = 0, tp_world_ = 1;
    void* tp_comm_ = nullptr;
    size_t tp_max_floats_ = 0;
    void* tp_peers_[8] = {nullptr, nullptr, nullptr, nullptr, nullptr, nullptr, nullptr, nullptr};
    bool tp_peer_opened_[8] = {false, false, false, false, false, false, false, false};
    bool tp_connected_ = false;
    unsigned tp_call_ = 0;
    bool own_stream_ = false;
    ModelConfig cfg_full_;
};

}
```

### ntransformer_amd/csrc/engine/model_debug.cpp

```cpp
#include "model_impl.h"

namespace nt {

int Model::debug_run_layers(const float* hidden_in, int T, int start_pos, int first, int count, int mode, float* hidden_out) {
    if (!hidden_in || !hidden_out) return NTK_E_NULL;
    if (T <= 0 || start_pos < 0 || start_pos + T > cfg_.max_seq_len || first < 0 || count < 0 || first + count > cfg_.n_layers) return NTK_E_SHAPE;
    if (mode != 0 && T != 1) return NTK_E_SHAPE;
    if (tp_world_ > 1) return NTK_E_SHAPE;
    const size_t bytes = (size_t)T * cfg_.hidden_size * 4;
    void* s = stream_;
    float* const hid = mode == 0 ? hidden_ : hidden1_;
    NT_TRY(ntk_memcpy_h2d_async(hid, hidden_in, bytes, s));
    int rc;
    if (mode == 0) {
        NT_TRY(upload_positions(T, start_pos));
        NT_TRY(ntk_stream_synchronize(s));
        rc = layers_1to1(T, start_pos, first, first + count);
    } else {
        NT_TRY(set_device_pos(start_pos));
        pick_attention_regime();
        if (mode == 1) {
            rc = enqueue_layers(first, first + count);
        } else {
            hipStream_t st = static_cast<hipStream_t>(s);
            hipGraphExec_t ex = nullptr;
            rc = capture_graph(st, hipStreamCaptureModeThreadLocal, [&] { return enqueue_layers(first, first + count); }, &ex);
            if (rc == NTK_OK && hipGraphLaunch(ex, st) != hipSuccess) rc = NTK_E_LAUNCH;
            if (rc == NTK_OK) rc = ntk_stream_synchronize(s);
            if (ex) (void)hipGraphExecDestroy(ex);
        }
    }
    if (rc != NTK_OK) return rc;
    NT_TRY(ntk_memcpy_d2h_async(hidden_out, hid, bytes, s));
    return ntk_stream_synchronize(s);
}

int Model::debug_kv(int layer, int pos0, int n, uint16_t* k, uint16_t* v, bool write, int slot) {
    if (!k || !v) return NTK_E_NULL;
    if (kv_q8_) { err_ = "debug_kv: the KV cache is q8_0 (use the _q8 form)"; return NTK_E_DTYPE; }
    if (layer < 0 || layer >= cfg_.n_layers || pos0 < 0 || n < 0 || pos0 + n > cfg_.max_seq_len || slot < 0 || slot >= kv_.slots()) return NTK_E_SHAPE;
    KvRange r[2];
    kv_.row_ranges(pos0, n, r);
    uint8_t* const kd = static_cast<uint8_t*>(kv_.k(slot, layer)) + r[0].off;
    uint8_t* const vd = static_cast<uint8_t*>(kv_.v(slot, layer)) + r[0].off;
    void* s = stream_;
    NT_TRY(write ? ntk_memcpy_h2d_async(kd, k, r[0].bytes, s) : ntk_memcpy_d2h_async(k, kd, r[0].bytes, s));
    NT_TRY(write ? ntk_memcpy_h2d_async(vd, v, r[0].bytes, s) : ntk_memcpy_d2h_async(v, vd, r[0].bytes, s));
    return ntk_stream_synchronize(s);
}

int Model::debug_kv_q8(int layer, int pos0, int n, uint8_t* k_blocks, uint8_t* v_blocks, bool write, int slot) {
    if (!k_blocks || !v_blocks) return NTK_E_NULL;
    if (!kv_q8_) { err_ = "debug_kv_q8: the KV cache is f16"; return NTK_E_DTYPE; }
    if (layer < 0 || layer >= cfg_.n_layers || pos0 < 0 || n < 0 || pos0 + n > cfg_.max_seq_len || slot < 0 || slot >= kv_.slots()) return NTK_E_SHAPE;
    if (n == 0) return NTK_OK;
    const size_t nb = (size_t)cfg_.n_kv_heads * cfg_.head_dim / 32;
    KvRange r[2];
    kv_.row_ranges(pos0, n, r);
    const size_t qbytes = r[0].bytes, sbytes = r[1].bytes;
    void* s = stream_;
    std::vector<uint8_t> qh(qbytes), sh(sbytes);
    for (int side = 0; side < 2; ++side) {
        uint8_t* base = static_cast<uint8_t*>(side ? kv_.v(slot, layer) : kv_.k(slot, layer));
        uint8_t *qd = base + r[0].off, *sd = base + r[1].off;
        uint8_t* blocks = side ? v_blocks : k_blocks;
        if (write) {
            for (size_t b = 0; b < (size_t)n * nb; ++b) {
                memcpy(&sh[2 * b], blocks + 34 * b, 2);
                memcpy(&qh[32 * b], blocks + 34 * b + 2, 32);
            }
            NT_TRY(ntk_memcpy_h2d_async(qd, qh.data(), qbytes, s));
            NT_TRY(ntk_memcpy_h2d_async(sd, sh.data(), sbytes, s));
            NT_TRY(ntk_stream_synchronize(s));
        } else {
            NT_TRY(ntk_memcpy_d2h_async(qh.data(), qd, qbytes, s));
            NT_TRY(ntk_memcpy_d2h_async(sh.data(), sd, sbytes, s));
            NT_TRY(ntk_stream_synchronize(s));
            for (size_t b = 0; b < (size_t)n * nb; ++b) {
                memcpy(blocks + 34 * b, &sh[2 * b], 2);
                memcpy(blocks + 34 * b + 2, &qh[32 * b], 32);
            }
        }
    }
    return NTK_OK;
}

int Model::debug_kv_inputs_capture(int layer) {
    if (layers_.empty()) return NTK_E_NULL;
    if (layer >= cfg_.n_layers) return NTK_E_SHAPE;
    kv_capture_layer_ = layer < 0 ? -1 : layer;
    kv_capture_T_ = 0;
    if (layer >= 0 && !kv_capture_) {
        const size_t bytes = 2 * (size_t)cfg_.max_seq_len * cfg_.n_kv_heads * cfg_.head_dim * 4;
        kv_capture_ = (float*)dev_alloc(bytes, false);
        if (!kv_capture_) { err_ = "debug_kv_inputs_capture: out of device memory"; return NTK_E_NOMEM; }
    }
    return NTK_OK;
}
int Model::debug_kv_inputs_read(int n, float* k, float* v) {
    if (!k || !v) return NTK_E_NULL;
    if (!kv_capture_ || kv_capture_layer_ < 0 || n < 0 || n > kv_capture_T_) return NTK_E_SHAPE;
    const size_t kvd = (size_t)cfg_.n_kv_heads * cfg_.head_dim;
    NT_TRY(ntk_memcpy_d2h_async(k, kv_capture_, (size_t)n * kvd * 4, stream_));
    NT_TRY(ntk_memcpy_d2h_async(v, kv_capture_ + (size_t)cfg_.max_seq_len * kvd, (size_t)n * kvd * 4, stream_));
    return ntk_stream_synchronize(stream_);
}

}
```

### ntransformer_amd/csrc/engine/model_decode.cpp

```cpp
#include "model_impl.h"

namespace nt {

void Model::prof_mark(int cls, bool begin) {
    if (!prof_) return;
    void* s = stream_;
    if (prof_coarse_) {
        if (!begin) return;
        if (!prof_->empty() && prof_->back().cls == cls) { ++prof_->back().n; return; }
        void* e = ntk_event_create();
        ntk_event_record(e, s);
        const bool shared = !prof_->empty();
        if (shared) prof_->back().b = e;
        prof_->push_back({cls, e, nullptr, 1, shared});
        return;
    }
    void* e = ntk_event_create();
    ntk_event_record(e, s);
    if (begin) prof_->push_back({cls, e, nullptr, 1, false}); else prof_->back().b = e;
}

int Model::enqueue_token(bool greedy) {
    const int H = cfg_.hidden_size;
    void* s = stream_;
    tp_call_ = 0;
    prof_mark(2, true);
    const int est = ntk_embed_rows(hidden1_, token_embd_.ptr, d_token_, 1, H, token_embd_.dtype, s);
    prof_mark(2, false);
    if (est != NTK_OK && est != NTK_E_DTYPE) return est;
    NT_TRY(enqueue_layers(0, cfg_.n_layers));
    const DevTensor* const w = &output_;
    const bool timed = fusable(w->dtype);
    if (timed) prof_mark(0, true);
    NT_TRY(decode_project(&w, &logits_, 1, hidden1_, &output_norm_, nullptr, 16, 0, false));
    if (timed) prof_mark(0, false);
    prof_mark(2, true);
    if (greedy) NT_TRY(ntk_argmax_advance(logits_, cfg_.vocab_size, d_token_, h_token_, h_ring_, d_pos_, argmax_scratch_, s));
    else NT_TRY(ntk_advance_pos(d_pos_, s));
    if (tp_world_ > 1) NT_TRY(ntk_tp_advance_epoch(tp_comm_, s));
    prof_mark(2, false);
    return NTK_OK;
}

int Model::decode_project(const DevTensor* const* ws, float* const* ys, int n, const float* x, const DevTensor* norm, const float* resid, int kind,
                          int silu_pair, bool timed) {
    const int H = cfg_.hidden_size;
    void* s = stream_;
    auto mark = [&](bool begin) { if (timed) prof_mark(0, begin); };
    const float* nw = norm ? (const float*)norm->ptr : nullptr;
    auto one_launch = [&](bool rp, const float* r, int silu) {
        ntk_gemv_seg segs[3];
        if (!rp) raw_begin();
        for (int a = 0; a < n; ++a) segs[a] = {rp ? ws[a]->rp : raw_of(*ws[a]), ys[a], (int)ws[a]->out_f, ws[a]->dtype};
        mark(true);
        const int st = (rp ? ntk_gemv_rp_fused : ntk_gemv_fused)(segs, n, x, (int)ws[0]->in_f, nw, cfg_.norm_eps, r, silu, s);
        mark(false);
        return st;
    };
    bool all_rp = repack_ && (rp_mask() & kind), all_quant = true, mixed = false;
    for (int a = 0; a < n; ++a) {
        all_rp = all_rp && ws[a]->rp != nullptr && ws[a]->in_f == ws[0]->in_f;
        all_quant = all_quant && is_quant(ws[a]->dtype);
        mixed = mixed || ws[a]->dtype != ws[0]->dtype;
    }
    if (all_rp) {
        const int st = one_launch(true, resid, silu_pair);
        if (!not_taken(st)) return st;
    }
    if (n > 1 && !resid && all_quant && mixed) {
        const int st = one_launch(false, nullptr, 0);
        if (!not_taken(st)) return st;
    }
    bool done[3] = {false, false, false};
    auto one_to_one = [&](int a) -> int {
        const DevTensor& w = *ws[a];
        const float* xin = x;
        if (nw) {
            NT_TRY(ntk_rmsnorm(residual_ + H, x, nw, 1, (int)w.in_f, cfg_.norm_eps, s));
            xin = residual_ + H;
        }
        float* y = resid ? residual_ : ys[a];
        raw_begin();
        NT_TRY(ntk_gemv(y, raw_of(w), xin, (int)w.out_f, (int)w.in_f, w.dtype, s));
        if (resid) NT_TRY(ntk_add(ys[a], resid, residual_, (int)w.out_f, s));
        done[a] = true;
        return NTK_OK;
    };
    for (int a = 0; a < n; ++a) {
        if (done[a]) continue;
        const DevTensor& w = *ws[a];
        if (!fusable(w.dtype)) { NT_TRY(one_to_one(a)); continue; }
        ntk_gemv_seg segs[3];
        int idx[3], m = 0;
        raw_begin();
        for (int b = a; b < n; ++b) {
            if (done[b] || ws[b]->dtype != w.dtype) continue;
            idx[m] = b;
            segs[m++] = {raw_of(*ws[b]), ys[b], (int)ws[b]->out_f, ws[b]->dtype};
        }
        mark(true);
        const int st = ntk_gemv_fused(segs, m, x, (int)w.in_f, nw, cfg_.norm_eps, resid, silu_pair, s);
        mark(false);
        if (is_dense16(w.dtype) && (st == NTK_E_ALIGN || st == NTK_E_SHAPE)) {
            for (int k = 0; k < m; ++k) NT_TRY(one_to_one(idx[k]));
            if (silu_pair) NT_TRY(ntk_silu_mul(ys[idx[0]], ys[idx[0]], ys[idx[1]], (int)w.out_f, s));
            continue;
        }
        NT_TRY(st);
        for (int k = 0; k < m; ++k) done[idx[k]] = true;
    }
    return NTK_OK;
}

int Model::enqueue_layers(int first, int last_layer) {
    const int H = cfg_.hidden_size, I = cfg_.intermediate_size, hd = cfg_.head_dim, nh = cfg_.n_heads, nkv = cfg_.n_kv_heads;
    void* s = stream_;
    const float scale = 1.0f / sqrtf((float)hd);
    const Views act = views(1, true);
    auto project_add = [&](const DevTensor& w, const float* x, int kind) -> int {
        const DevTensor* const wp = &w;
        float* y = tp_world_ > 1 ? tp_slot() : hidden1_;
        NT_TRY(decode_project(&wp, &y, 1, x, nullptr, tp_world_ > 1 ? nullptr : hidden1_, kind));
        return tp_world_ > 1 ? tp_allreduce(hidden1_, H) : (int)NTK_OK;
    };

    for (int i = first; i < last_layer; ++i) {
        const LayerWeights& L = layers_[i];
        const DevTensor* const qkv[3] = {&L.wq, &L.wk, &L.wv};
        float* const qkv_out[3] = {act.q, act.k, act.v};
        NT_TRY(decode_project(qkv, qkv_out, 3, hidden1_, &L.attn_norm, nullptr, 1));
        prof_mark(1, true);
        if (kv_q8_)
            NT_TRY(ntk_attention_decode_q8(act.attn_out, act.q, act.k, act.v, kv_.k(0, i), kv_.v(0, i), d_pos_, rope_inv_freq_, nh, nkv, hd,
                                           cfg_.max_seq_len, scale, cfg_.rope_theta, cfg_.rope_freq_scale, kv_q8_splits(attn_regime_), attn_scratch_, s));
        else if (attn_regime_ == 0)
            NT_TRY(ntk_attention_decode_fused(act.attn_out, act.q, act.k, act.v, kv_.k_f16(0, i), kv_.v_f16(0, i), d_pos_, rope_inv_freq_, nh, nkv, hd,
                                              cfg_.max_seq_len, scale, cfg_.rope_theta, cfg_.rope_freq_scale, s));
        else
            NT_TRY((attn_merge_ ? ntk_attention_decode_split_merged : ntk_attention_decode_split)(
                act.attn_out, act.q, act.k, act.v, kv_.k_f16(0, i), kv_.v_f16(0, i), d_pos_, rope_inv_freq_, nh, nkv, hd, cfg_.max_seq_len, scale,
                cfg_.rope_theta, cfg_.rope_freq_scale, attention_splits(attn_regime_, hd), attn_scratch_, s));
        prof_mark(1, false);
        NT_TRY(project_add(L.wo, act.attn_out, 2));
        const DevTensor* const ffn[2] = {&L.w_gate, &L.w_up};
        float* const ffn_out[2] = {act.gate, act.up};
        const bool pair = fusable(L.w_gate.dtype) && L.w_gate.dtype == L.w_up.dtype;
        if (pair) prof_mark(0, true);
        NT_TRY(decode_project(ffn, ffn_out, 2, hidden1_, &L.ffn_norm, nullptr, 4, pair, !pair));
        if (pair) prof_mark(0, false);
        else NT_TRY(ntk_silu_mul(act.gate, act.gate, act.up, I, s));
        NT_TRY(project_add(L.w_down, act.gate, 8));
    }
    return NTK_OK;
}

void Model::pick_attention_regime() {
    attn_regime_ = (attn_scratch_ && (cfg_.head_dim == 64 || cfg_.head_dim == 128 || cfg_.head_dim == 256))
                       ? attention_regime(host_pos_, cfg_.head_dim) : 0;
    ++host_pos_;
}

int Model::decode_step_fused(bool greedy, bool use_graph) {
    pick_attention_regime();
    if (!use_graph) return enqueue_token(greedy);
    ihipGraphExec_t*& slot = graphs_[greedy ? 1 : 0][attn_regime_];
    hipStream_t st = static_cast<hipStream_t>(stream_);
    if (!slot) {
        hipGraphExec_t ex = nullptr;
        NT_TRY(capture_graph(st, tp_world_ > 1 ? hipStreamCaptureModeRelaxed : hipStreamCaptureModeThreadLocal, [&] { return enqueue_token(greedy); }, &ex));
        slot = reinterpret_cast<ihipGraphExec_t*>(ex);
    }
    return hipGraphLaunch(reinterpret_cast<hipGraphExec_t>(slot), st) == hipSuccess ? NTK_OK : NTK_E_LAUNCH;
}

int Model::profile_token(float ms[4], int calls[4], bool coarse) {
    std::vector<Timed> rec;
    rec.reserve(1024);
    prof_ = &rec;
    prof_coarse_ = coarse;
    pick_attention_regime();
    int rc = enqueue_token(true);
    if (coarse && !rec.empty()) {
        void* e = ntk_event_create();
        ntk_event_record(e, stream_);
        rec.back().b = e;
    }
    prof_ = nullptr;
    prof_coarse_ = false;
    if (rc == NTK_OK) rc = ntk_stream_synchronize(stream_);
    for (int c = 0; c < 4; ++c) { ms[c] = 0.0f; calls[c] = 0; }
    for (auto& t : rec) {
        float m = 0.0f;
        if (t.a && t.b && ntk_event_elapsed_ms(t.a, t.b, &m) == NTK_OK) { ms[t.cls] += m; calls[t.cls] += t.n; }
        ++calls[3];
    }
    for (auto& t : rec) {
        if (t.a && !t.shared_a) ntk_event_destroy(t.a);
        if (t.b) ntk_event_destroy(t.b);
    }
    return rc;
}

}
```

### ntransformer_amd/csrc/engine/model_prompt.cpp

```cpp
#include "model_impl.h"
#include "../gemm_dense16_plan.h"

namespace nt {

float* Model::forward(const int* tokens, int T, int start_pos, int slot) {
    if (T <= 0 || start_pos < 0 || start_pos + T > cfg_.max_seq_len) { err_ = "forward: sequence exceeds context"; return nullptr; }
    if (slot < 0 || slot >= sequences_) { err_ = "forward: no such sequence slot"; return nullptr; }
    for (int i = 0; i < T; ++i)
        if (tokens[i] < 0 || tokens[i] >= cfg_.vocab_size) { err_ = "forward: token id out of range"; return nullptr; }
    const int H = cfg_.hidden_size;
    void* s = stream_;
    tp_call_ = 0;
    if (ntk_memcpy_h2d_async(tokens_dev_, tokens, (size_t)T * 4, s) != NTK_OK) return nullptr;
    if (embed_rows(hidden_, tokens_dev_, T) != NTK_OK) return nullptr;
    if (upload_positions(T, start_pos) != NTK_OK) return nullptr;
    if (ntk_stream_synchronize(s) != NTK_OK) return nullptr;

    const KvTarget kv{slot, nullptr, 0};
    PassStatus ok{layers_1to1(T, start_pos, 0, cfg_.n_layers, kv)};
    float* last = hidden_ + (size_t)(T - 1) * H;
    ok(ntk_rmsnorm(last, last, (const float*)output_norm_.ptr, 1, H, cfg_.norm_eps, s));
    raw_begin();
    const int st = gemv_logged(logits_, output_, raw_of(output_), last);
    if (st != NTK_E_DTYPE) ok(st);
    if (tp_world_ > 1) ok(ntk_tp_advance_epoch(tp_comm_, s));
    int rc = finish_pass("forward failed: ", ok.rc);
    if (rc == NTK_OK) rc = check_tp();
    return rc == NTK_OK ? logits_ : nullptr;
}

int Model::embed_rows(float* out, const int* ids_dev, int n) {
    const int st = ntk_embed_rows(out, token_embd_.ptr, ids_dev, n, cfg_.hidden_size, token_embd_.dtype, stream_);
    if (st != NTK_E_DTYPE) return st;
    fprintf(stderr, "Error: Unsupported embedding dtype: %s\n", dtype_name(token_embd_.dtype));
    return NTK_OK;
}

int Model::upload_positions(int T, int start_pos) {
    host_positions_.resize((size_t)T);
    for (int i = 0; i < T; ++i) host_positions_[i] = start_pos + i;
    return ntk_memcpy_h2d_async(positions_, host_positions_.data(), (size_t)T * 4, stream_);
}

const float* Model::final_norm(float* dst, const float* src, int n, PassStatus& ok) {
    const float* nw = (const float*)output_norm_.ptr;
    const float* rm = lm_head_f16() && row_max_ && prefill_row_max_ ? row_max_ : nullptr;
    if (rm) ok(ntk_rmsnorm_rowmax(dst, src, nw, n, cfg_.hidden_size, cfg_.norm_eps, row_max_, nullptr, stream_));
    else ok(ntk_rmsnorm(dst, src, nw, n, cfg_.hidden_size, cfg_.norm_eps, stream_));
    return rm;
}

int Model::finish_pass(const char* failed, int rc) {
    const int sy = ntk_stream_synchronize(stream_);
    if (rc == NTK_OK) rc = sy;
    if (raw_err_ != NTK_OK) { rc = raw_err_; raw_err_ = NTK_OK; }
    if (rc != NTK_OK && (err_.empty() || rc != NTK_E_LAUNCH)) err_ = std::string(failed) + ntk_status_string(rc);
    return rc;
}

int Model::gemv_logged(float* y, const DevTensor& w, const void* wp, const float* x) {
    const int st = ntk_gemv(y, wp, x, (int)w.out_f, (int)w.in_f, w.dtype, stream_);
    if (st == NTK_E_DTYPE) fprintf(stderr, "Unsupported dtype for GEMV: %s\n", dtype_name(w.dtype));
    return st;
}

struct OperandPlanes {
    enum Kind { fp16, bf16 };
    void* ws[2];
    int cur = 0;
    const float* of = nullptr;
    Kind kind = fp16;
    void* current() const { return ws[cur]; }
    bool hold(const float* X, Kind k = fp16) const { return X == of && k == kind; }
    void* other() { cur ^= 1; of = nullptr; return ws[cur]; }
    void written(const float* X, bool split) { of = split ? X : nullptr; kind = fp16; }
    void in_current(const float* X, Kind k = fp16) { of = X; kind = k; }
};

static bool f16_ok(const DevTensor& w) {
    const bool kq = w.dtype == NTK_DT_Q4_0 || w.dtype == NTK_DT_Q4_K || w.dtype == NTK_DT_Q5_K || w.dtype == NTK_DT_Q6_K;
    return (w.dtype == NTK_DT_Q8_0 || kq) && w.in_f % (kq ? 256 : 128) == 0 && w.out_f % 16 == 0 && (w.ptr || w.rp);
}
static bool dense16_ok(const DevTensor& w) { return is_dense16(w.dtype) && w.in_f % 32 == 0 && w.out_f % 16 == 0 && w.ptr; }
static bool rp_only(const DevTensor& w) {
    return !w.ptr && w.rp && (w.dtype == NTK_DT_Q4_K || w.dtype == NTK_DT_Q5_K || w.dtype == NTK_DT_Q6_K) && w.out_f % 16 == 0;
}

int Model::layers_1to1(int T, int start_pos, int first, int last_layer, const KvTarget& kv) {
    const int H = cfg_.hidden_size, I = cfg_.intermediate_size, qd = cfg_.n_heads * cfg_.head_dim, kvd = cfg_.n_kv_heads * cfg_.head_dim;
    void* s = stream_;
    const Views act = views(T);
    PassStatus ok;
    const bool batched = batched_prefill_ && T > 1;
    const bool bf16_now = bf16_prefill_ && gemm_ws_ && T > 1;
    OperandPlanes planes{{gemm_ws_, gemm_ws2_}};
    const bool with_max = batched && bf16_now && row_max_ != nullptr && prefill_row_max_;
    float* rm_a = with_max ? row_max_ : nullptr;
    float* rm_b = with_max ? row_max_ + cfg_.max_seq_len : nullptr;
    enum class XForm { plain, row_max, split };
    auto x_form = [&](int width, const DevTensor& next_w) {
        const bool f16_planes = f16_ok(next_w) || (dense_mfma16_ && fusable(next_w.dtype) && next_w.dtype == NTK_DT_F16 && dense16_ok(next_w) && ntk::gd_worth(T));
        if (with_max && prefill_fused_split_ && gemm_ws2_ != nullptr && T <= 64 && tp_world_ == 1 && f16_planes && (int)next_w.in_f == width) return XForm::split;
        return with_max ? XForm::row_max : XForm::plain;
    };
    auto gemm_group = [&](float* const* Ys, const DevTensor* const* Ws, int n, const float* X, const float* resid, const float* rm, ntk_gemm_partials* pt,
                          const void* const* raw) {
        bool repacked = raw == nullptr;
        for (int k = 0; k < n; ++k) repacked = repacked && rp_only(*Ws[k]);
        if (!repacked && !raw) raw_begin();
        ntk_gemv_seg segs[3];
        for (int k = 0; k < n; ++k) segs[k] = {repacked ? Ws[k]->rp : raw ? raw[k] : raw_of(*Ws[k]), Ys[k], (int)Ws[k]->out_f, Ws[k]->dtype};
        ntk_gemm_desc d{};
        d.segs = segs; d.nseg = n; d.X = X; d.n_tokens = T; d.in_features = (int)Ws[0]->in_f; d.resid = resid;
        d.workspace = planes.current(); d.workspace_bytes = gemm_ws_bytes_; d.reuse_x = planes.hold(X) ? 1 : 0; d.row_max = rm; d.partials = pt;
        d.weights_repacked = repacked ? 1 : 0;
        const int st = ntk_gemm_quant_f16(&d, s);
        if (st == NTK_OK) planes.in_current(X);
        return st;
    };
    auto dense16_group = [&](float* const* Ys, const DevTensor* const* Ws, int n, const float* X, const float* resid) {
        if (!dense_mfma16_ || !gemm_ws_ || !ntk::gd_worth(T)) return (int)NTK_E_DTYPE;
        ntk_gemv_seg segs[3];
        for (int k = 0; k < n; ++k) {
            if (!dense16_ok(*Ws[k])) return (int)NTK_E_SHAPE;
            segs[k] = {Ws[k]->ptr, Ys[k], (int)Ws[k]->out_f, Ws[k]->dtype};
        }
        const OperandPlanes::Kind kind = Ws[0]->dtype == NTK_DT_BF16 ? OperandPlanes::bf16 : OperandPlanes::fp16;
        ntk_gemm_desc d{};
        d.segs = segs; d.nseg = n; d.X = X; d.n_tokens = T; d.in_features = (int)Ws[0]->in_f; d.resid = resid;
        d.workspace = planes.current(); d.workspace_bytes = gemm_ws_bytes_; d.reuse_x = planes.hold(X, kind) ? 1 : 0;
        const int st = ntk_gemm_dense16(&d, s);
        if (st == NTK_OK) planes.in_current(X, kind);
        return st;
    };
    auto gemm_f16 = [&](float* Y, const DevTensor& w, const float* X, const float* resid, const float* rm, ntk_gemm_partials* pt, const void** wp) {
        const DevTensor* const one = &w;
        if (bf16_now && rp_only(w)) {
            const int st = gemm_group(&Y, &one, 1, X, resid, rm, pt, nullptr);
            if (!not_taken(st)) return st;
        }
        raw_begin();
        *wp = raw_of(w);
        return bf16_now ? gemm_group(&Y, &one, 1, X, resid, rm, pt, wp) : (int)NTK_E_DTYPE;
    };
    auto gemm_mfma = [&](float* Y, const DevTensor& w, const float* X, const float* resid, const float* rm, const void** wp) {
        int st = NTK_E_DTYPE;
        if (is_dense16(w.dtype)) {
            raw_begin(); *wp = raw_of(w);
            const DevTensor* const one = &w;
            st = dense16_group(&Y, &one, 1, X, resid);
        }
        else st = gemm_f16(Y, w, X, resid, rm, nullptr, wp);
        if (not_taken(st)) st = ntk_gemm_quant(Y, *wp, X, T, (int)w.out_f, (int)w.in_f, w.dtype, resid, s);
        if (st == NTK_E_ALIGN || st == NTK_E_SHAPE) return false;
        ok(st);
        return true;
    };
    auto project = [&](float* Y, const DevTensor& w, const float* X, size_t ystride, size_t xstride, const float* rm) {
        const bool dense = ystride == (size_t)w.out_f && xstride == (size_t)w.in_f;
        const void* wp = nullptr;
        if (batched && fusable(w.dtype) && dense) {
            if (gemm_mfma(Y, w, X, nullptr, rm, &wp)) return;
        } else { raw_begin(); wp = raw_of(w); }
        for (int t = 0; t < T; ++t) {
            const int st = gemv_logged(Y + (size_t)t * ystride, w, wp, X + (size_t)t * xstride);
            if (st != NTK_E_DTYPE) ok(st);
        }
    };
    auto project_many = [&](float* const* Ys, const DevTensor* const* Ws, int n, const float* X, const float* rm) {
        bool done[3] = {false, false, false};
        for (int a = 0; a < n && batched && (bf16_now || is_dense16(Ws[a]->dtype)); ++a) {
            if (done[a]) continue;
            const bool d16 = is_dense16(Ws[a]->dtype);
            if (d16 ? !(fusable(Ws[a]->dtype) && dense_mfma16_) : !bf16_now) continue;
            float* ys[3];
            const DevTensor* ws[3];
            int idx[3], m = 0;
            for (int b = a; b < n; ++b)
                if (!done[b] && Ws[b]->dtype == Ws[a]->dtype && Ws[b]->in_f == Ws[a]->in_f) { ys[m] = Ys[b]; ws[m] = Ws[b]; idx[m++] = b; }
            if (m < 2) continue;
            const int st = d16 ? dense16_group(ys, ws, m, X, nullptr) : gemm_group(ys, ws, m, X, nullptr, rm, nullptr, nullptr);
            if (st == NTK_OK) for (int k = 0; k < m; ++k) done[idx[k]] = true;
            else if (!not_taken(st)) { ok(st); return; }
        }
        for (int a = 0; a < n; ++a)
            if (!done[a]) project(Ys[a], *Ws[a], X, (size_t)Ws[a]->out_f, (size_t)Ws[a]->in_f, rm);
    };
    auto prepare_x = [&](const float* X, const DevTensor& w) {
        if (x_form((int)w.in_f, w) != XForm::split || planes.hold(X)) return;
        planes.written(X, ntk_gemm_prepare_x(X, T, (int)w.in_f, planes.other(), s) == NTK_OK);
    };
    auto project_add = [&](const DevTensor& w, const float* X, size_t xstride, const float* rm) {
        if (tp_world_ > 1) {
            project(tp_slot(), w, X, H, xstride, rm);
            ok(tp_allreduce(hidden_, T * H));
            return;
        }
        const bool dense = batched && (size_t)w.out_f == (size_t)H && xstride == (size_t)w.in_f;
        if (dense && (bf16_now || is_dense16(w.dtype))) prepare_x(X, w);
        const void* wp = nullptr;
        if (dense && fusable(w.dtype) && gemm_mfma(hidden_, w, X, hidden_, rm, &wp)) return;
        project(residual_, w, X, H, xstride, rm);
        ok(ntk_add_inplace(hidden_, residual_, T * H, s));
    };
    auto norm = [&](const DevTensor& nw, bool zero_b, const DevTensor& next_w) {
        const XForm f = x_form(H, next_w);
        if (f == XForm::split) ok(ntk_rmsnorm_prepare_x(residual_, hidden_, (const float*)nw.ptr, T, H, cfg_.norm_eps, planes.other(), s));
        else if (f == XForm::row_max) ok(ntk_rmsnorm_rowmax(residual_, hidden_, (const float*)nw.ptr, T, H, cfg_.norm_eps, rm_a, zero_b ? rm_b : nullptr, s));
        else ok(ntk_rmsnorm(residual_, hidden_, (const float*)nw.ptr, T, H, cfg_.norm_eps, s));
        planes.written(residual_, f == XForm::split);
    };
    auto project_add_norm = [&](const DevTensor& w, const float* X, const float* rm, const DevTensor& nw, bool zero_b, const DevTensor& next_w) -> bool {
        if (!with_max || tp_world_ > 1 || !is_quant(w.dtype) || (size_t)w.out_f != (size_t)H) return false;
        ntk_gemm_partials pt;
        prepare_x(X, w);
        const void* wp = nullptr;
        int st = gemm_f16(hidden_, w, X, hidden_, rm, &pt, &wp);
        if (not_taken(st)) return false;
        const bool split = st == NTK_OK && x_form(H, next_w) == XForm::split;
        if (split) st = ntk_reduce_rmsnorm_prepare_x(hidden_, &pt, (const float*)nw.ptr, cfg_.norm_eps, residual_, planes.other(), s);
        else if (st == NTK_OK) st = ntk_reduce_rmsnorm_rowmax(hidden_, &pt, (const float*)nw.ptr, cfg_.norm_eps, residual_, rm_a, zero_b ? rm_b : nullptr, s);
        planes.written(residual_, split);
        ok(st);
        return true;
    };
    auto gate_up_silu = [&](const LayerWeights& L) -> bool {
        if (!with_max || !rm_b || tp_world_ > 1 || L.w_gate.dtype != L.w_up.dtype || !is_quant(L.w_gate.dtype) || L.w_gate.in_f != L.w_up.in_f ||
            (size_t)L.w_gate.out_f != (size_t)I || (size_t)L.w_up.out_f != (size_t)I || I % 4 != 0) return false;
        float* const ys[2] = {act.gate, act.up};
        const DevTensor* const ws[2] = {&L.w_gate, &L.w_up};
        ntk_gemm_partials pt;
        int st = gemm_group(ys, ws, 2, residual_, nullptr, rm_a, &pt, nullptr);
        if (not_taken(st)) return false;
        const bool split = st == NTK_OK && x_form(I, L.w_down) == XForm::split;
        if (split) st = ntk_reduce_silu_mul_prepare_x(act.gate, &pt, planes.other(), s);
        else if (st == NTK_OK) st = ntk_reduce_silu_mul_rowmax(act.gate, &pt, rm_b, s);
        planes.written(act.gate, split);
        ok(st);
        return true;
    };
    auto silu_mul = [&](const DevTensor& next_w) {
        const XForm f = x_form(I, next_w);
        int st = NTK_E_SHAPE;
        if (f == XForm::split) st = ntk_silu_mul_prepare_x(act.gate, act.gate, act.up, T, I, planes.other(), s);
        else if (f == XForm::row_max && rm_b) st = ntk_silu_mul_rowmax(act.gate, act.gate, act.up, T, I, rm_b, s);
// ... 192 lines not shown
```

### ntransformer_amd/csrc/gemv.hip

```cpp
#include "gemv_core.hip.h"
#include <algorithm>
#include <atomic>
#include <cmath>
#include <cstddef>
#include <mutex>
#include <cstdio>
#include <cstdlib>

namespace ntk {

enum { NS_ANY = 0, NS_ONE = 1, NS_SPLIT = 2 };

enum { XS_NONE = 0, XS_HIDDEN = NTK_ARENA_HIDDEN, XS_ATTN = NTK_ARENA_ATTN_OUT, XS_GATE = NTK_ARENA_GATE };
struct DecodeArena {
    float hidden[NTK_ARENA_HIDDEN_FLOATS];
    float attn_out[NTK_ARENA_ATTN_FLOATS];
    float gate[NTK_ARENA_GATE_FLOATS];
};
__device__ __attribute__((aligned(256))) DecodeArena g_decode_arena;
template <int XS> struct XSlot { static constexpr int IN = XS == XS_GATE ? 14336 : 4096; };
template <int XS> __device__ __forceinline__ const float* xslot_ptr() {
    return XS == XS_HIDDEN ? g_decode_arena.hidden : XS == XS_ATTN ? g_decode_arena.attn_out : g_decode_arena.gate;
}

template <int DT, bool NORM, bool XFAST, bool A16, bool XI = false, bool LM = false, int NSF = NS_ANY, int XS = XS_NONE>
__device__ __forceinline__ void gemv_quant_body(const GemvParams& p, const int bid, const int nblk) {
    using F = Fmt<DT>;
    static_assert(!LM || (DT == NTK_DT_Q8_0 && !A16 && !XI), "lane-major rows: Q8_0");
    static_assert(NSF == NS_ANY || LM, "compile-time slice forms: the lane-major kernels");
    static_assert(XS == XS_NONE || (LM && XFAST && NSF != NS_ANY), "early-x forms: the lane-major kernels, fast prologue");
    constexpr int NL = LM ? 4 : F::NL;
    constexpr int STAGE = LM ? 0 : NL * 1024 + 64;
    extern __shared__ __attribute__((aligned(16))) uint8_t smem[];
#ifdef NTK_GEMV_TRACE
    unsigned long long gv_t[GT_EV] = {0, 0, 0, 0, 0, 0, 0, 0, 0, 0, 0, 0, 0, 0};
#endif
    GV_STAMP(0);
#ifndef NTK_GEMV_NO_KARG_PREFETCH
    const auto* ka = __builtin_amdgcn_kernarg_segment_ptr();
    unsigned d0, d1, d2, d3, d4;
    if constexpr (XS == XS_NONE) {
        asm volatile("s_load_dword %0, %5, 0x0\n\ts_load_dword %1, %5, 0x40\n\ts_load_dword %2, %5, 0x80\n\ts_load_dword %3, %5, 0xc0\n\t"
                     "s_load_dword %4, %5, 0x100\n\ts_waitcnt lgkmcnt(0)"
                     : "=&s"(d0), "=&s"(d1), "=&s"(d2), "=&s"(d3), "=&s"(d4) : "s"(ka) : "memory");
    } else {
        asm volatile("s_load_dword %0, %5, 0x0\n\ts_load_dword %1, %5, 0x40\n\ts_load_dword %2, %5, 0x80\n\ts_load_dword %3, %5, 0xc0\n\t"
                     "s_load_dword %4, %5, 0x100"
                     : "=&s"(d0), "=&s"(d1), "=&s"(d2), "=&s"(d3), "=&s"(d4) : "s"(ka) : "memory");
    }
    __builtin_amdgcn_sched_barrier(0);
#endif

    const int tid = threadIdx.x;
    constexpr int XIT = 8, WIT = 4;
    u32x4 xv[XIT], wv[WIT];
    if constexpr (XS != XS_NONE) {
        constexpr int IN = XSlot<XS>::IN, step0 = 512 * 4;
        const float* const xs = xslot_ptr<XS>();
#pragma unroll
        for (int i = 0; i < XIT; ++i) {
            xv[i] = u32x4{0u, 0u, 0u, 0u};
            if (i * step0 < IN) xv[i] = *reinterpret_cast<const u32x4*>(xs + min(tid * 4 + i * step0, IN - 4));
        }
        GV_STAMP(7);
        __builtin_amdgcn_sched_barrier(0);
#ifndef NTK_GEMV_NO_KARG_PREFETCH
        asm volatile("s_waitcnt lgkmcnt(0)" : "+s"(d0), "+s"(d1), "+s"(d2), "+s"(d3), "+s"(d4) : : "memory");
        __builtin_amdgcn_sched_barrier(0);
#endif
        if constexpr (NORM) {
#pragma unroll
            for (int i = 0; i < WIT; ++i) {
                wv[i] = u32x4{0u, 0u, 0u, 0u};
                if (i * step0 < IN) wv[i] = *reinterpret_cast<const u32x4*>(p.norm_w + min(tid * 4 + i * step0, IN - 4));
            }
        }
    } else
    if constexpr (XFAST) {
        const int step0 = (int)blockDim.x * 4;
#pragma unroll
        for (int i = 0; i < XIT; ++i) {
            xv[i] = u32x4{0u, 0u, 0u, 0u};
            if (i * step0 < p.in) xv[i] = *reinterpret_cast<const u32x4*>(p.x + min(tid * 4 + i * step0, p.in - 4));
        }
        if constexpr (NORM) {
#pragma unroll
            for (int i = 0; i < WIT; ++i) {
                wv[i] = u32x4{0u, 0u, 0u, 0u};
                if (i * step0 < p.in) wv[i] = *reinterpret_cast<const u32x4*>(p.norm_w + min(tid * 4 + i * step0, p.in - 4));
            }
        }
        GV_STAMP(7);
    }
    const int lane = tid & 63;
    const int wave = __builtin_amdgcn_readfirstlane(tid >> 6);
    const int ns = NSF == NS_ONE ? 1 : p.ns;
    const bool single = NSF == NS_ANY ? p.ns == 1 : NSF == NS_ONE;
    const int nwaves = ns * p.rw;
    const int s = wave % ns;
    const int g = wave / ns;
    constexpr bool norm = NORM;

    const size_t image_bytes = (size_t)std::min(ns, 4) * 64 * XPITCH * 4;
    const size_t stage0 = single ? image_bytes : 0;
    const size_t regionA = single ? image_bytes + (size_t)nwaves * STAGE : std::max((size_t)nwaves * STAGE, image_bytes);
    float* part = reinterpret_cast<float*>(smem + regionA);
    float* red = part + 2 * p.rw * ns * RB;
    const size_t lds_floats_total = regionA / 4 + (size_t)(2 * p.rw * ns * RB + 16 + 16);

    uint8_t* stage = smem + stage0 + (size_t)wave * STAGE;
    const int my_len = min(p.slice_cols, p.in - s * p.slice_cols);
    const int ncols = min(64, max(0, my_len - 64 * lane));
    const unsigned slice_byte0 = (unsigned)((size_t)s * p.slice_cols / F::BW * F::BB);
    const unsigned slice_bytes = (unsigned)(my_len / F::BW * F::BB);
    const int group = bid * p.rw + g;
    const int ngroups = nblk * p.rw;
    const int mats = p.silu_pair ? 2 : 1;
    const int n_my = (p.total_rows > group) ? ((p.total_rows - 1 - group) / ngroups + 1) * mats : 0;

    static_assert(MAX_SEG == 3, "locate / seg_y: unrolled for three segments");
    const int seg_rows0 = p.seg[0].rows, seg_rows1 = p.seg[1].rows;
    float* const seg_y0 = p.seg[0].y;
    float* const seg_y1 = p.seg[1].y;
    float* const seg_y2 = p.seg[2].y;
    auto locate = [&](int q, int& seg, int& row) {
        int r = group + (q >> (mats - 1)) * ngroups;
        if (p.silu_pair) { seg = q & 1; row = r; return; }
        seg = 0;
        if (p.nseg > 1 && r >= seg_rows0) {
            r -= seg_rows0; seg = 1;
            if (p.nseg > 2 && r >= seg_rows1) { r -= seg_rows1; seg = 2; }
        }
        row = r;
    };
    auto seg_y = [&](int seg) { return seg == 0 ? seg_y0 : seg == 1 ? seg_y1 : seg_y2; };
    int cu_seg = 0, cu_row = group, cu_rows = p.silu_pair ? 0x7fffffff : p.seg[0].rows;
    auto cursor_normalise = [&]() {
        while (cu_seg + 1 < p.nseg && cu_row >= cu_rows) { cu_row -= cu_rows; ++cu_seg; cu_rows = p.seg[cu_seg].rows; }
    };
    if (!p.silu_pair) cursor_normalise();
    auto cursor_advance = [&]() {
        if (p.silu_pair) {
            if (cu_seg == 0) { cu_seg = 1; } else { cu_seg = 0; cu_row += ngroups; }
        } else {
            cu_row += ngroups;
            cursor_normalise();
        }
    };

    u32x4 pf[NL], pf2[LM ? NL : 1];
    uint32_t pf_sc = 0u, pf2_sc = 0u;
    const int lm_nl = my_len >> 6, lm_lane = min(lane, max(lm_nl - 1, 0));
    unsigned pre_off[NL];
    if constexpr (A16) {
        const unsigned last0 = (slice_bytes - 1u) & ~15u;
#pragma unroll
        for (int j = 0; j < NL; ++j) pre_off[j] = min(16u * (unsigned)(lane + 64 * j), last0);
    }
    int pf_seg = 0, pf_row = 0, pf_shift = 0;
    float pf_res = 0.0f;
    auto issue = [&]() {
        pf_seg = cu_seg; pf_row = cu_row;
        if (p.resid != nullptr && single) {
            int idx = cu_row;
            asm volatile("" : "+v"(idx));
            pf_res = p.resid[idx];
        }
        if constexpr (LM) return;
        const unsigned rel = (unsigned)p.seg[cu_seg].delta + (unsigned)cu_row * p.row_bytes + slice_byte0;
        pf_shift = (int)(rel & 15u);
        const unsigned nbytes = (rel & 15u) + slice_bytes;
        const unsigned last = (nbytes - 1u) & ~15u;
        const uint8_t* a = p.seg[cu_seg].W + (rel & ~15u);
#pragma unroll
        for (int j = 0; j < NL; ++j) {
            unsigned off;
            if constexpr (A16) off = pre_off[j]; else off = min(16u * (unsigned)(lane + 64 * j), last);
            pf[j] = __builtin_nontemporal_load(reinterpret_cast<const u32x4*>(a + off));
        }
    };
    auto issue_lm = [&](u32x4 (&c)[NL], uint32_t& sc) {
        const uint8_t* a = p.seg[cu_seg].W + ((unsigned)cu_row * p.row_bytes + slice_byte0);
#pragma unroll
// ... 67 lines not shown
            }
            if constexpr (XI) {
                uint8_t* dimg = smem;
                auto xi_store = [&](const u32x4 q, const int sp, const int cc, const bool live) {
                    const float v0 = live ? __uint_as_float(q.x) : 0.0f, v1 = live ? __uint_as_float(q.y) : 0.0f,
                                v2 = live ? __uint_as_float(q.z) : 0.0f, v3 = live ? __uint_as_float(q.w) : 0.0f;
                    float am = fmaxf(fmaxf(fabsf(v0), fabsf(v1)), fmaxf(fabsf(v2), fabsf(v3)));
                    am = fmaxf(am, dpp_or_self<DPP_QUAD_1032, 0xF>(am));
                    am = fmaxf(am, dpp_or_self<DPP_QUAD_2301, 0xF>(am));
                    am = fmaxf(am, dpp_or_self<DPP_ROW_HALF_MIRROR, 0xF>(am));
                    float sm = (v0 + v1) + (v2 + v3);
                    sm += dpp_or_zero<DPP_QUAD_1032, 0xF>(sm);
                    sm += dpp_or_zero<DPP_QUAD_2301, 0xF>(sm);
                    const int e = am > 0.0f ? __builtin_amdgcn_frexp_expf(am) : 0;
                    const float up = __builtin_ldexpf(1.0f, 22 - e), inv = __builtin_ldexpf(1.0f, e - 22);
                    const uint32_t x0 = __float_as_uint(fmaf(v0, up, 12582912.0f)) - 0x4B400000u, x1 = __float_as_uint(fmaf(v1, up, 12582912.0f)) - 0x4B400000u,
                                   x2i = __float_as_uint(fmaf(v2, up, 12582912.0f)) - 0x4B400000u, x3 = __float_as_uint(fmaf(v3, up, 12582912.0f)) - 0x4B400000u;
                    const uint32_t ta = __builtin_amdgcn_perm(x1, x0, 0x05010400u);
                    const uint32_t tb = __builtin_amdgcn_perm(x1, x0, 0x07030602u);
                    const uint32_t tc = __builtin_amdgcn_perm(x3, x2i, 0x05010400u);
                    const uint32_t td = __builtin_amdgcn_perm(x3, x2i, 0x07030602u);
                    const uint32_t p0 = __builtin_amdgcn_perm(tc, ta, 0x05040100u);
                    const uint32_t p1 = __builtin_amdgcn_perm(tc, ta, 0x07060302u);
                    const uint32_t p2 = __builtin_amdgcn_perm(td, tb, 0x05040100u);
                    if (live) {
                        uint8_t* row = dimg + (size_t)(sp * 64 + (cc >> 6)) * (XPITCH * 4);
                        *reinterpret_cast<uint32_t*>(row + (cc & 63)) = p0;
                        *reinterpret_cast<uint32_t*>(row + 64 + (cc & 63)) = p1;
                        *reinterpret_cast<uint32_t*>(row + 128 + (cc & 63)) = p2;
                        float* meta = reinterpret_cast<float*>(row + 192);
                        if ((cc & 31) == 0) meta[(cc >> 5) & 1] = inv;
                        if ((cc & 15) == 0) meta[2 + ((cc >> 4) & 3)] = sm;
                    }
                };
                auto xi_read = [&](const int g0) {
                    const bool have_lo_ = ncols > 0, have_hi_ = ncols > 32;
                    const uint8_t* rowA = dimg + (size_t)((s - g0) * 64 + lane) * (XPITCH * 4);
                    const uint8_t* rowB = rowA;
                    int offA = 0, offB = 32;
                    if constexpr (DT == NTK_DT_Q6_K) {
                        rowA = dimg + (size_t)((s - g0) * 64 + (lane & ~1)) * (XPITCH * 4);
                        rowB = rowA + XPITCH * 4;
                        offA = offB = 32 * (lane & 1);
                    }
#pragma unroll
                    for (int pl = 0; pl < 3; ++pl)
#pragma unroll
                        for (int k4 = 0; k4 < 4; ++k4) {
                            const uint8_t* src = (k4 < 2 ? rowA + offA : rowB + offB) + 64 * pl + 16 * (k4 & 1);
                            const u32x4 v = *reinterpret_cast<const u32x4*>(src);
                            const bool have = k4 < 2 ? have_lo_ : have_hi_;
                            xi.d[pl][4 * k4] = have ? v.x : 0u; xi.d[pl][4 * k4 + 1] = have ? v.y : 0u;
                            xi.d[pl][4 * k4 + 2] = have ? v.z : 0u; xi.d[pl][4 * k4 + 3] = have ? v.w : 0u;
                        }
                    const float* mA = reinterpret_cast<const float*>(rowA + 192);
                    const float* mB = reinterpret_cast<const float*>(rowB + 192);
                    xi.inv[0] = have_lo_ ? mA[offA >> 5] : 0.0f;
                    xi.inv[1] = have_hi_ ? mB[offB >> 5] : 0.0f;
                    xi.sx[0] = have_lo_ ? mA[2 + (offA >> 4)] : 0.0f; xi.sx[1] = have_lo_ ? mA[3 + (offA >> 4)] : 0.0f;
                    xi.sx[2] = have_hi_ ? mB[2 + (offB >> 4)] : 0.0f; xi.sx[3] = have_hi_ ? mB[3 + (offB >> 4)] : 0.0f;
                };
                int isp = 0, icc = tid * 4;
#pragma unroll
                for (int i = 0; i < XIT; ++i) {
                    if (i * step >= p.in) continue;
                    xi_store(xv[i], isp, icc, tid * 4 + i * step < p.in);
                    icc += step;
                    if (icc >= p.slice_cols) { icc -= p.slice_cols; ++isp; }
                }
                __syncthreads();
                xi_read(0);
            } else
            {
                const int cend = min(p.in, GS * p.slice_cols);
                int isp = 0, icc = tid * 4;
#pragma unroll
                for (int i = 0; i < XIT; ++i) {
                    if (i * step >= cend) continue;
                    const int c = tid * 4 + i * step;
                    *reinterpret_cast<u32x4*>(ximg + (c < cend ? (isp * 64 + (icc >> 6)) * XPITCH + (icc & 63) : dummy)) = xv[i];
                    icc += step;
                    if (icc >= p.slice_cols) { icc -= p.slice_cols; ++isp; }
                }
                for (int c = XIT * step + tid * 4; c < cend; c += step)
                    *reinterpret_cast<float4*>(ximg + img_index(c, 0)) = *reinterpret_cast<const float4*>(p.x + c);
                GV_STAMP(9);
                __syncthreads();
                GV_STAMP(10);
                if (s < GS) read_own_row(0);
#ifdef NTK_GEMV_TRACE
                asm volatile("s_waitcnt lgkmcnt(0)" ::: "memory");
                GV_STAMP(11);
#endif
            }
            if constexpr (!XI)
            for (int g0 = GS; g0 < ns; g0 += GS) {
                const int cbeg = g0 * p.slice_cols, cend = min(p.in, (g0 + GS) * p.slice_cols);
                __syncthreads();
                for (int c = cbeg + tid * 4; c < cend; c += step)
                    *reinterpret_cast<float4*>(ximg + img_index(c, g0)) = *reinterpret_cast<const float4*>(p.x + c);
                __syncthreads();
                if (s >= g0 && s < g0 + GS) read_own_row(g0);
            }
        } else {
            issue_first();
            float rms_inv = 1.0f;
            if (NORM && !(kAblate & 1)) {
                float ssq = 0.0f;
                for (int c = tid; c < p.in; c += blockDim.x) ssq = fmaf(p.x[c], p.x[c], ssq);
                ssq = wave_sum(ssq);
                if (lane == 0) red[wave] = ssq;
                __syncthreads();
                float tot = 0.0f;
                for (int w = 0; w < nwaves; ++w) tot += red[w];
                rms_inv = 1.0f / sqrtf(tot / (float)p.in + p.eps);
            }
            for (int g0 = 0; g0 < ns; g0 += GS) {
                const int cbeg = g0 * p.slice_cols, cend = min(p.in, (g0 + GS) * p.slice_cols);
                if (g0 > 0) __syncthreads();
                if (!(kAblate & 1)) {
                    for (int c = cbeg + tid; c < cend; c += blockDim.x)
                        ximg[img_index(c, g0)] = NORM ? p.x[c] * rms_inv * p.norm_w[c] : p.x[c];
                }
                __syncthreads();
                if (s >= g0 && s < g0 + GS) read_own_row(g0);
            }
        }
        if ((kAblate & 1) || XI) {
#pragma unroll
            for (int j = 0; j < 32; ++j) x2[j] = f32x2{1.0f, 1.0f};
        }
        if (!single && !LM) __syncthreads();
        GV_STAMP(2);
    }
    float sx16[4], sx32[2];
#pragma unroll
    for (int r = 0; r < 4; ++r) {
        float t = 0.0f;
#pragma unroll
        for (int j = 0; j < 8; ++j) t += x2[8 * r + j].x + x2[8 * r + j].y;
        sx16[r] = t;
    }
    sx32[0] = sx16[0] + sx16[1];
    sx32[1] = sx16[2] + sx16[3];
    if constexpr (DT == NTK_DT_Q4_K) {
#pragma unroll
        for (int j = 16; j < 32; ++j) x2[j] *= 0.0625f;
    }
    if constexpr (DT == NTK_DT_Q4_0) {
#pragma unroll
        for (int j = 0; j < 32; ++j) if ((j & 8) != 0) x2[j] *= 0.0625f;
    }
    float gate_carry = 0.0f;
    float pair_g = 0.0f, pair_u = 0.0f;
    auto silu_flush = [&](const int last_pair) {
        const int base = last_pair & ~63;
        if (lane <= last_pair - base) {
            const int row = group + (base + lane) * ngroups;
            p.seg[0].y[row] = pair_g / (1.0f + expf(-pair_g)) * pair_u;
        }
    };

    float res_pf = 0.0f;
    auto prefetch_resid = [&](int b) {
        if (p.resid == nullptr || s != 0 || lane >= RB || b * RB + lane >= n_my) return;
        int seg, row;
        locate(b * RB + lane, seg, row);
        res_pf = p.resid[row];
    };
    if (!single) prefetch_resid(0);
    auto combine = [&](int b, int cnt) {
        if (s != 0) return;
        const float* pg = part + (size_t)(b & 1) * p.rw * ns * RB + (size_t)(g * ns) * RB;
        float t = 0.0f;
        if (lane < cnt)
            for (int ss = 0; ss < ns; ++ss) t += pg[ss * RB + lane];
        const float nxt = __shfl_down(t, 1, 64);
        if (lane < cnt) {
            int seg, row;
            locate(b * RB + lane, seg, row);
            if (p.silu_pair) {
                if ((lane & 1) == 0) seg_y0[row] = t / (1.0f + expf(-t)) * nxt;
            } else {
                float v = t;
                if (p.resid != nullptr && seg == 0) v = res_pf + v;
                seg_y(seg)[row] = v;
            }
        }
        prefetch_resid(b + 1);
    };

    auto row_step = [&](const int q, u32x4 (&cur)[NL], uint32_t& cur_sc, u32x4 (&nxt)[LM ? NL : 1], uint32_t& nxt_sc) __attribute__((always_inline)) {
        const int seg = pf_seg, row = pf_row, shift = A16 ? 0 : pf_shift;
        const float res = pf_res;
        float acc;
        if constexpr (LM) {
            asm volatile("" : "+v"(cur[0]), "+v"(cur[1]), "+v"(cur[2]), "+v"(cur[3]), "+v"(cur_sc));
#ifdef NTK_GEMV_TRACE
            if (q == 0) GV_STAMP(3);
            if (q == n_my - 1) GV_STAMP(5);
#endif
            if (q + 1 < n_my) { cursor_advance(); issue(); issue_lm(nxt, nxt_sc); }
            __builtin_amdgcn_sched_barrier(0);
            acc = dot_q8_regs(cur, cur_sc, ncols, x2);
        } else {
#pragma unroll
            for (int j = 0; j < NL; ++j) {
                if (kAblate & 4) { asm volatile("" ::"v"(pf[j])); continue; }
                *reinterpret_cast<u32x4*>(stage + 16 * (lane + 64 * j)) = pf[j];
            }
            __builtin_amdgcn_wave_barrier();
#ifdef NTK_GEMV_TRACE
            if (q == 0) GV_STAMP(3);
            if (q == n_my - 1) GV_STAMP(5);
#endif
            if (q + 1 < n_my) { cursor_advance(); issue(); }
            if constexpr (XI && DT == NTK_DT_Q6_K) acc = DotI<DT>::run(stage, shift, lane, ncols, xi);
            else if constexpr (XI) acc = DotI<DT>::run(stage, lane, ncols, xi);
            else acc = (kAblate & 2) ? x2[0].x + (float)q : Dot<DT, A16>::run(stage, shift, lane, ncols, x2, sx16, sx32);
            __builtin_amdgcn_wave_barrier();
        }
        const float tot = wave_sum_lane63(acc);
#ifdef NTK_GEMV_TRACE
        if (q == 0) { asm volatile("" :: "v"(tot)); GV_STAMP(4); }
#endif

        if (single) {
            if (p.silu_pair) {
                const float t63 = __int_as_float(__builtin_amdgcn_readlane(__float_as_int(tot), 63));
                const int pi = (q >> 1) & 63;
                if ((q & 1) == 0) { if (lane == pi) pair_g = t63; }
                else {
                    if (lane == pi) pair_u = t63;
                    if (pi == 63 || q == n_my - 1) silu_flush(q >> 1);
                }
            } else if (lane == 63) {
                float v = tot;
                if (p.resid != nullptr && seg == 0) v = res + v;
                p.seg[seg].y[row] = v;
            }
        } else {
            const int b = q / RB, i = q % RB;
            if (lane == 63) part[(size_t)(b & 1) * p.rw * ns * RB + (size_t)(g * ns + s) * RB + i] = tot;
            if (i == RB - 1) {
                __syncthreads();
                combine(b, RB);
            }
        }
    };
    for (int q = 0; q < n_my; ++q) {
        row_step(q, pf, pf_sc, pf2, pf2_sc);
        if constexpr (LM) { if (++q < n_my) row_step(q, pf2, pf2_sc, pf, pf_sc); }
    }
    if (!single) {
        int done = n_my / RB;
        if (n_my % RB) {
            __syncthreads();
            combine(done, n_my % RB);
            ++done;
        }
        for (; done < p.nbatch; ++done) __syncthreads();
    }
#ifdef NTK_GEMV_TRACE
    GV_STAMP(6);
    if (tid == 0 && bid < GT_WG) {
        gv_t[13] = (unsigned long long)n_my;
        for (int e = 0; e < GT_EV; ++e) g_gemv_trace[p.trace_slot & (GT_SLOTS - 1)][bid][e] = gv_t[e];
    }
#endif
}

template <bool NORM, bool XFAST, int NSF, int XS = XS_NONE>
__global__ __launch_bounds__(512, Fmt<NTK_DT_Q8_0>::MINW) void gemv_q8l_kernel(const GemvParams p) {
    gemv_quant_body<NTK_DT_Q8_0, NORM, XFAST, false, false, true, NSF, XS>(p, (int)blockIdx.x, (int)gridDim.x);
}
template <bool UNPACK>
__global__ __launch_bounds__(256) void q8l_pack_kernel(uint8_t* __restrict__ dst, const uint8_t* __restrict__ src, const int rows, const int in,
                                                       const int slice_cols) {
    const int lanes_row = in >> 6;
    const size_t t = (size_t)blockIdx.x * blockDim.x + threadIdx.x;
    if (t >= (size_t)rows * lanes_row) return;
    const int row = (int)(t / lanes_row), gl = (int)(t % lanes_row);
    const int lanes_slice = slice_cols >> 6, sl = gl / lanes_slice, l = gl - sl * lanes_slice;
    const int nl = min(lanes_slice, lanes_row - sl * lanes_slice);
    const size_t row0 = (size_t)row * lanes_row * 68;
    uint32_t* file = reinterpret_cast<uint32_t*>(const_cast<uint8_t*>(UNPACK ? dst : src) + row0 + (size_t)gl * 68);
    uint8_t* slice = const_cast<uint8_t*>(UNPACK ? src : dst) + row0 + (size_t)sl * lanes_slice * 68;
    uint32_t w[17], q[16], sc;
    if constexpr (!UNPACK) {
#pragma unroll
        for (int k = 0; k < 17; ++k) w[k] = file[k];
#pragma unroll
        for (int k = 0; k < 8; ++k) { q[k] = (w[k] >> 16) | (w[k + 1] << 16); q[8 + k] = w[9 + k]; }
        sc = (w[0] & 0xFFFFu) | (w[8] & 0xFFFF0000u);
#pragma unroll
        for (int j = 0; j < 4; ++j) *reinterpret_cast<u32x4*>(slice + (size_t)(j * nl + l) * 16) = u32x4{q[4 * j], q[4 * j + 1], q[4 * j + 2], q[4 * j + 3]};
        *reinterpret_cast<uint32_t*>(slice + (size_t)64 * nl + 4 * l) = sc;
    } else {
#pragma unroll
        for (int j = 0; j < 4; ++j) {
            const u32x4 v = *reinterpret_cast<const u32x4*>(slice + (size_t)(j * nl + l) * 16);
            q[4 * j] = v.x; q[4 * j + 1] = v.y; q[4 * j + 2] = v.z; q[4 * j + 3] = v.w;
        }
        sc = *reinterpret_cast<const uint32_t*>(slice + (size_t)64 * nl + 4 * l);
        w[0] = (sc & 0xFFFFu) | (q[0] << 16);
#pragma unroll
        for (int k = 1; k < 8; ++k) w[k] = (q[k - 1] >> 16) | (q[k] << 16);
        w[8] = (q[7] >> 16) | (sc & 0xFFFF0000u);
#pragma unroll
        for (int k = 0; k < 8; ++k) w[9 + k] = q[8 + k];
#pragma unroll
        for (int k = 0; k < 17; ++k) file[k] = w[k];
    }
}

template <int DT, bool NORM, bool XFAST, bool A16>
__global__ __launch_bounds__(512, Fmt<DT>::MINW) void gemv_quant_kernel(const GemvParams p) {
    gemv_quant_body<DT, NORM, XFAST, A16>(p, (int)blockIdx.x, (int)gridDim.x);
}
template <int DT, bool NORM>
__global__ __launch_bounds__(512, Fmt<DT>::MINW) void gemv_quant_xi_kernel(const GemvParams p) {
    gemv_quant_body<DT, NORM, true, A16_OK<DT>, true>(p, (int)blockIdx.x, (int)gridDim.x);
}
template <int DTA, int DTB, bool NORM>
__global__ __launch_bounds__(512, 4) void gemv_quant_pair_kernel(const GemvParams pa, const GemvParams pb, const int split) {
    if ((int)blockIdx.x < split) gemv_quant_body<DTA, NORM, true, A16_OK<DTA>>(pa, (int)blockIdx.x, split);
    else gemv_quant_body<DTB, NORM, true, A16_OK<DTB>>(pb, (int)blockIdx.x - split, (int)gridDim.x - split);
}

template <bool BF> __device__ __forceinline__ float w16f(uint16_t bits) {
    if constexpr (BF) return __uint_as_float((uint32_t)bits << 16); else return h2f(bits);
}
template <typename T, bool ADD, bool BF = false>
__global__ __launch_bounds__(256) void gemv_dense_kernel(float* __restrict__ y, const T* __restrict__ W,
                                                         const float* __restrict__ x, int out, int in) {
    const int lane = threadIdx.x & 63;
    const int wave = blockIdx.x * (blockDim.x >> 6) + (threadIdx.x >> 6);
    const int nwaves = gridDim.x * (blockDim.x >> 6);
    constexpr int V = 16 / (int)sizeof(T);
    for (int r = wave; r < out; r += nwaves) {
        const T* w = W + (size_t)r * in;
        float acc = 0.0f;
        int done = 0;
        if ((reinterpret_cast<uintptr_t>(w) & 15) == 0 && (reinterpret_cast<uintptr_t>(x) & 15) == 0) {
            const int nv = in / V;
            for (int i = lane; i < nv; i += 64) {
                const u32x4 raw = __builtin_nontemporal_load(reinterpret_cast<const u32x4*>(w) + i);
                if constexpr (sizeof(T) == 4) {
                    const float4 xv = *reinterpret_cast<const float4*>(x + 4 * i);
                    acc = fmaf(__uint_as_float(raw.x), xv.x, acc); acc = fmaf(__uint_as_float(raw.y), xv.y, acc);
                    acc = fmaf(__uint_as_float(raw.z), xv.z, acc); acc = fmaf(__uint_as_float(raw.w), xv.w, acc);
                } else {
                    const float4 x0 = *reinterpret_cast<const float4*>(x + 8 * i);
                    const float4 x1 = *reinterpret_cast<const float4*>(x + 8 * i + 4);
                    acc = fmaf(w16f<BF>((uint16_t)(raw.x & 0xFFFF)), x0.x, acc); acc = fmaf(w16f<BF>((uint16_t)(raw.x >> 16)), x0.y, acc);
                    acc = fmaf(w16f<BF>((uint16_t)(raw.y & 0xFFFF)), x0.z, acc); acc = fmaf(w16f<BF>((uint16_t)(raw.y >> 16)), x0.w, acc);
                    acc = fmaf(w16f<BF>((uint16_t)(raw.z & 0xFFFF)), x1.x, acc); acc = fmaf(w16f<BF>((uint16_t)(raw.z >> 16)), x1.y, acc);
                    acc = fmaf(w16f<BF>((uint16_t)(raw.w & 0xFFFF)), x1.z, acc); acc = fmaf(w16f<BF>((uint16_t)(raw.w >> 16)), x1.w, acc);
                }
            }
            done = nv * V;
        }
        for (int i = done + lane; i < in; i += 64) {
            float wv;
            if constexpr (sizeof(T) == 4) wv = (float)w[i]; else wv = w16f<BF>((uint16_t)w[i]);
            acc = fmaf(wv, x[i], acc);
        }
        acc = wave_sum(acc);
        if (lane == 0) y[r] = ADD ? y[r] + acc : acc;
    }
}

static bool is_quant(int dt) {
    return dt == NTK_DT_Q8_0 || dt == NTK_DT_Q4_0 || dt == NTK_DT_Q4_K || dt == NTK_DT_Q5_K || dt == NTK_DT_Q6_K;
}

struct GemvLaunch {
    GemvParams p;
    int grid, nwaves;
    size_t lds;
    bool xfast, a16;
};

static bool raise_lds_limit(const void* fn) {
    return hipFuncSetAttribute(fn, hipFuncAttributeMaxDynamicSharedMemorySize, 160 * 1024) == hipSuccess;
}

template <int DT>
static int prepare_quant(const ntk_gemv_seg* segs, int nseg, const float* x, int in, const float* norm_w, float eps,
                         const float* resid, int silu_pair, int max_wg, GemvLaunch& L, bool lm = false) {
    using F = Fmt<DT>;
    if (in <= 0 || in % F::BW != 0) return NTK_E_SHAPE;
    GemvParams& p = L.p;
    p = GemvParams{};
    long total = 0;
    const size_t row_bytes = (size_t)in / F::BW * F::BB;
    for (int i = 0; i < nseg; ++i) {
        if (segs[i].rows < 0) return NTK_E_SHAPE;
        if (segs[i].rows > 0 && (!segs[i].W || !segs[i].y)) return NTK_E_NULL;
        if ((size_t)segs[i].rows * row_bytes > 0xFFFFFFF0ull) return NTK_E_SHAPE;
        const uintptr_t w = reinterpret_cast<uintptr_t>(segs[i].W);
        if (w & 1) return NTK_E_ALIGN;
        p.seg[i].W = reinterpret_cast<const uint8_t*>(w & ~(uintptr_t)15);
        p.seg[i].delta = (int)(w & 15);
        p.seg[i].y = segs[i].y;
        p.seg[i].rows = segs[i].rows;
        total += segs[i].rows;
    }
    if (silu_pair) {
        if (nseg != 2 || segs[0].rows != segs[1].rows || resid) return NTK_E_SHAPE;
        total = segs[0].rows;
    }
    p.nseg = nseg;
    p.total_rows = (int)total;
    p.x = x;
    p.in = in;
    if (!gemv_slices(in, F::BW == 256 ? 256 : 64, p.ns, p.slice_cols)) return NTK_E_SHAPE;
    static const int env_waves = std::max(1, NTK_TUNE_ENV_INT("NTK_GEMV_WAVES", 8));
    p.rw = std::max(1, env_waves / p.ns);
    L.nwaves = p.ns * p.rw;
    p.x_vec = ((reinterpret_cast<uintptr_t>(x) & 15) == 0 &&
               (!norm_w || (reinterpret_cast<uintptr_t>(norm_w) & 15) == 0) && (p.slice_cols % 4 == 0)) ? 1 : 0;
    p.norm_w = norm_w;
    p.eps = eps;
    p.resid = resid;
    p.silu_pair = silu_pair;
    p.row_bytes = (unsigned)row_bytes;
    const int mats = silu_pair ? 2 : 1;
    int grid = (int)std::min<long>((total + p.rw - 1) / p.rw, max_wg);
    grid = std::max(grid, 1);
    L.grid = grid;
    const long ngroups = (long)grid * p.rw;
    const long rows_per_group = (total + ngroups - 1) / ngroups;
    p.nbatch = (int)((rows_per_group * mats + RB - 1) / RB);
    const int STAGE = lm ? 0 : F::NL * 1024 + 64;
    const size_t image_bytes = (size_t)std::min(p.ns, 4) * 64 * XPITCH * 4;
    const size_t regionA = p.ns == 1 ? image_bytes + (size_t)L.nwaves * STAGE : std::max((size_t)L.nwaves * STAGE, image_bytes);
    L.lds = regionA + (size_t)(2 * p.rw * p.ns * RB + 16 + 16) * sizeof(float);
    L.xfast = p.x_vec && (in % 4 == 0) && in >= 4 && !(kAblate & 1) && (!norm_w || in <= 4 * 4 * 64 * L.nwaves) &&
              (p.ns == 1 || 4 * 64 * L.nwaves <= p.slice_cols);
    bool a16 = (DT == NTK_DT_Q4_K || DT == NTK_DT_Q5_K);
    for (int i = 0; i < nseg; ++i) a16 = a16 && p.seg[i].delta == 0;
    L.a16 = a16;
    return NTK_OK;
}

constexpr size_t kXiMinBytes = (size_t)48 << 20;
enum { XI_DEFAULT = -1, XI_NEVER = 0, XI_ALWAYS = 1 };

static int max_workgroups() {
    static const int max_wg = std::max(1, NTK_TUNE_ENV_INT("NTK_GEMV_MAX_WG", 512));
    return max_wg;
}

template <int DT>
static int launch_quant(const ntk_gemv_seg* segs, int nseg, const float* x, int in, const float* norm_w, float eps,
                        const float* resid, int silu_pair, hipStream_t st, int xi_mode = XI_DEFAULT) {
    GemvLaunch L;
    const int rc = prepare_quant<DT>(segs, nseg, x, in, norm_w, eps, resid, silu_pair, max_workgroups(), L);
    if (rc != NTK_OK) return rc;
    if (L.p.total_rows == 0) return NTK_OK;
    using KernelFn = void (*)(const GemvParams);
    static const KernelFn table[2][2][2] = {
        {{gemv_quant_kernel<DT, false, false, false>, gemv_quant_kernel<DT, false, false, A16_OK<DT>>},
         {gemv_quant_kernel<DT, false, true, false>, gemv_quant_kernel<DT, false, true, A16_OK<DT>>}},
        {{gemv_quant_kernel<DT, true, false, false>, gemv_quant_kernel<DT, true, false, A16_OK<DT>>},
         {gemv_quant_kernel<DT, true, true, false>, gemv_quant_kernel<DT, true, true, A16_OK<DT>>}}};
    if (L.lds > 64 * 1024) {
        static bool once = [] {
            bool ok = true;
            for (int a = 0; a < 2; ++a)
                for (int b = 0; b < 2; ++b)
                    for (int c = 0; c < 2; ++c)
                        ok = ok && hipFuncSetAttribute((const void*)table[a][b][c], hipFuncAttributeMaxDynamicSharedMemorySize,
                                                       160 * 1024) == hipSuccess;
            return ok;
        }();
        if (!once || L.lds > 160 * 1024) return NTK_E_SHAPE;
    }
    const dim3 g(L.grid), b(64 * L.nwaves);
#ifdef NTK_GEMV_TRACE
    static int trace_counter = 0;
    L.p.trace_slot = trace_counter++;
#endif
    if constexpr (DT == NTK_DT_Q4_K || DT == NTK_DT_Q6_K) {
        const size_t launch_bytes = (size_t)L.p.total_rows * (silu_pair ? 2 : 1) * L.p.row_bytes;
        const bool want = xi_mode == XI_ALWAYS || (xi_mode == XI_DEFAULT && launch_bytes >= kXiMinBytes);
        if (want && L.xfast && (L.a16 || DT == NTK_DT_Q6_K) && L.p.ns <= 2 && in <= 8 * 4 * 64 * L.nwaves) {
            using XFn = void (*)(const GemvParams);
            static const XFn xt[2] = {gemv_quant_xi_kernel<DT, false>, gemv_quant_xi_kernel<DT, true>};
            if (L.lds > 64 * 1024) {
                static bool once2 = hipFuncSetAttribute((const void*)xt[0], hipFuncAttributeMaxDynamicSharedMemorySize, 160 * 1024) == hipSuccess &&
                                    hipFuncSetAttribute((const void*)xt[1], hipFuncAttributeMaxDynamicSharedMemorySize, 160 * 1024) == hipSuccess;
                if (!once2) return NTK_E_SHAPE;
            }
            hipLaunchKernelGGL(xt[norm_w ? 1 : 0], g, b, L.lds, st, L.p);
            return last_launch_status();
        }
    }
    hipLaunchKernelGGL(table[norm_w ? 1 : 0][L.xfast ? 1 : 0][L.a16 ? 1 : 0], g, b, L.lds, st, L.p);
    return last_launch_status();
}

static size_t q8l_bytes(int rows, int in) {
    int ns, sc;
    return rows > 0 && q8l_layout(in, ns, sc) ? (size_t)rows * (size_t)(in / 32 * 34) : 0;
}

static int q8l_pack(void* dst, const void* raw, int rows, int in, bool unpack, hipStream_t st) {
    int ns, sc;
    if (rows <= 0 || !q8l_layout(in, ns, sc)) return NTK_E_SHAPE;
    if ((reinterpret_cast<uintptr_t>(unpack ? raw : dst) & 15) || (reinterpret_cast<uintptr_t>(unpack ? dst : raw) & 3)) return NTK_E_ALIGN;
    const size_t n = (size_t)rows * (in / 64);
    if ((n + 255) / 256 > 0x7FFFFFFFull) return NTK_E_SHAPE;
    const dim3 g((unsigned)((n + 255) / 256)), b(256);
    uint8_t* d = static_cast<uint8_t*>(dst);
    const uint8_t* r = static_cast<const uint8_t*>(raw);
    if (unpack) hipLaunchKernelGGL(q8l_pack_kernel<true>, g, b, 0, st, d, r, rows, in, sc);
    else hipLaunchKernelGGL(q8l_pack_kernel<false>, g, b, 0, st, d, r, rows, in, sc);
    return last_launch_status();
}

constexpr int kArenaDevices = 16;
struct ArenaDev {
    std::atomic<int> known{0};
    std::atomic<int> owned{0};
    const float* addr[4] = {nullptr, nullptr, nullptr, nullptr};
};
static ArenaDev g_arena_dev[kArenaDevices];
static std::mutex g_arena_mu;
static thread_local int t_last_static_x = XS_NONE;

static ArenaDev* arena_dev(bool lookup) {
    int dev = -1;
    if (hipGetDevice(&dev) != hipSuccess || dev < 0 || dev >= kArenaDevices) return nullptr;
    ArenaDev& a = g_arena_dev[dev];
    if (a.known.load(std::memory_order_acquire) == 0 && lookup) {
        std::lock_guard<std::mutex> lk(g_arena_mu);
        if (a.known.load(std::memory_order_relaxed) == 0) {
            void* base = nullptr;
            const bool ok = hipGetSymbolAddress(&base, HIP_SYMBOL(g_decode_arena)) == hipSuccess && base != nullptr;
            if (ok) {
                auto* f = static_cast<const float*>(base);
                a.addr[XS_HIDDEN] = f + offsetof(DecodeArena, hidden) / 4;
                a.addr[XS_ATTN] = f + offsetof(DecodeArena, attn_out) / 4;
                a.addr[XS_GATE] = f + offsetof(DecodeArena, gate) / 4;
            }
            a.known.store(ok ? 1 : -1, std::memory_order_release);
        }
    }
    return a.known.load(std::memory_order_acquire) == 1 ? &a : nullptr;
}
static int static_x_slot(const float* x, int in) {
    const ArenaDev* a = arena_dev(false);
    if (!a) return XS_NONE;
    if (x == a->addr[XS_HIDDEN] && in == XSlot<XS_HIDDEN>::IN) return XS_HIDDEN;
    if (x == a->addr[XS_ATTN] && in == XSlot<XS_ATTN>::IN) return XS_ATTN;
    if (x == a->addr[XS_GATE] && in == XSlot<XS_GATE>::IN) return XS_GATE;
    return XS_NONE;
}

int q8l_gemv_fused(const ntk_gemv_seg* segs, int nseg, const float* x, int in, const float* norm_w, float eps, const float* resid,
                   int silu_pair, hipStream_t st) {
    int ns, sc;
    t_last_static_x = XS_NONE;
    if (!q8l_layout(in, ns, sc)) return NTK_E_SHAPE;
    for (int i = 0; i < nseg; ++i)
        if (reinterpret_cast<uintptr_t>(segs[i].W) & 15) return NTK_E_ALIGN;
    GemvLaunch L;
    const int rc = prepare_quant<NTK_DT_Q8_0>(segs, nseg, x, in, norm_w, eps, resid, silu_pair, max_workgroups(), L, true);
    if (rc != NTK_OK) return rc;
    if (L.p.total_rows == 0) return NTK_OK;
    using KernelFn = void (*)(const GemvParams);
#define Q8L_FORMS(NORM, XFAST) {gemv_q8l_kernel<NORM, XFAST, NS_ONE>, gemv_q8l_kernel<NORM, XFAST, NS_SPLIT>}
    static const KernelFn table[2][2][2] = {{Q8L_FORMS(false, false), Q8L_FORMS(false, true)}, {Q8L_FORMS(true, false), Q8L_FORMS(true, true)}};
#undef Q8L_FORMS
    if (L.lds > 64 * 1024) {
        static const bool once = [] {
            bool ok = true;
            for (int a = 0; a < 2; ++a)
                for (int b = 0; b < 2; ++b)
                    for (int c = 0; c < 2; ++c) ok = ok && raise_lds_limit((const void*)table[a][b][c]);
            return ok;
        }();
        if (!once || L.lds > 160 * 1024) return NTK_E_SHAPE;
    }
#ifdef NTK_GEMV_TRACE
    static int trace_counter = 0;
    L.p.trace_slot = trace_counter++;
#endif
    KernelFn fn = table[norm_w ? 1 : 0][L.xfast ? 1 : 0][L.p.ns == 1 ? 0 : 1];
    if (L.xfast && L.nwaves == 8) {
        const int xs = static_x_slot(x, in);
        KernelFn early = nullptr;
        if (xs == XS_HIDDEN && L.p.ns == 1 && norm_w) early = gemv_q8l_kernel<true, true, NS_ONE, XS_HIDDEN>;
        else if (xs == XS_ATTN && L.p.ns == 1 && !norm_w) early = gemv_q8l_kernel<false, true, NS_ONE, XS_ATTN>;
        else if (xs == XS_GATE && L.p.ns > 1 && !norm_w) {
            static const bool raised = raise_lds_limit((const void*)gemv_q8l_kernel<false, true, NS_SPLIT, XS_GATE>);
            if (raised || L.lds <= 64 * 1024) early = gemv_q8l_kernel<false, true, NS_SPLIT, XS_GATE>;
        }
        if (early && L.lds <= 160 * 1024) { fn = early; t_last_static_x = xs; }
    }
    hipLaunchKernelGGL(fn, dim3(L.grid), dim3(64 * L.nwaves), L.lds, st, L.p);
    return last_launch_status();
}


template <int DTA, int DTB>
static int launch_pair(const ntk_gemv_seg* sa, int na, const ntk_gemv_seg* sb, int nb, const float* x, int in, const float* norm_w,
                       float eps, hipStream_t st) {
    const double ba = (double)Fmt<DTA>::BB / Fmt<DTA>::BW, bb = (double)Fmt<DTB>::BB / Fmt<DTB>::BW;
    long ra = 0, rb = 0;
    for (int i = 0; i < na; ++i) ra += sa[i].rows;
    for (int i = 0; i < nb; ++i) rb += sb[i].rows;
    if (ra <= 0 || rb <= 0) return NTK_E_SHAPE;
    const int total_wg = max_workgroups();
    int wa = (int)(total_wg * (ra * ba) / (ra * ba + rb * bb) + 0.5);
    wa = std::min(std::max(wa, 1), total_wg - 1);
    GemvLaunch A, B;
    int rc = prepare_quant<DTA>(sa, na, x, in, norm_w, eps, nullptr, 0, wa, A);
    if (rc == NTK_OK) rc = prepare_quant<DTB>(sb, nb, x, in, norm_w, eps, nullptr, 0, total_wg - wa, B);
    if (rc != NTK_OK) return rc;
    if (!A.xfast || !B.xfast || A.nwaves != B.nwaves || A.a16 != A16_OK<DTA> || B.a16 != A16_OK<DTB>) return NTK_E_ALIGN;
    for (int i = 0; i < na; ++i) if (A.p.seg[i].delta != 0 && A16_OK<DTA>) return NTK_E_ALIGN;
    using PairFn = void (*)(const GemvParams, const GemvParams, int);
    const size_t lds = std::max(A.lds, B.lds);
    static const PairFn table[2] = {gemv_quant_pair_kernel<DTA, DTB, false>, gemv_quant_pair_kernel<DTA, DTB, true>};
    if (lds > 64 * 1024) {
        static bool once = hipFuncSetAttribute((const void*)table[0], hipFuncAttributeMaxDynamicSharedMemorySize, 160 * 1024) == hipSuccess &&
                           hipFuncSetAttribute((const void*)table[1], hipFuncAttributeMaxDynamicSharedMemorySize, 160 * 1024) == hipSuccess;
        if (!once || lds > 160 * 1024) return NTK_E_SHAPE;
    }
    hipLaunchKernelGGL(table[norm_w ? 1 : 0], dim3(A.grid + B.grid), dim3(64 * A.nwaves), lds, st, A.p, B.p, A.grid);
    return last_launch_status();
}

static int dispatch_quant(int dt, const ntk_gemv_seg* segs, int nseg, const float* x, int in, const float* norm_w,
                          float eps, const float* resid, int silu_pair, hipStream_t st, int xi_mode = XI_DEFAULT) {
    switch (dt) {
        case NTK_DT_Q8_0: return launch_quant<NTK_DT_Q8_0>(segs, nseg, x, in, norm_w, eps, resid, silu_pair, st);
        case NTK_DT_Q4_0: return launch_quant<NTK_DT_Q4_0>(segs, nseg, x, in, norm_w, eps, resid, silu_pair, st);
        case NTK_DT_Q4_K: return launch_quant<NTK_DT_Q4_K>(segs, nseg, x, in, norm_w, eps, resid, silu_pair, st, xi_mode);
        case NTK_DT_Q5_K: return launch_quant<NTK_DT_Q5_K>(segs, nseg, x, in, norm_w, eps, resid, silu_pair, st);
        case NTK_DT_Q6_K: return launch_quant<NTK_DT_Q6_K>(segs, nseg, x, in, norm_w, eps, resid, silu_pair, st, xi_mode);
        default: return NTK_E_DTYPE;
    }
}

template <bool ADD>
static int launch_dense(float* y, const void* W, const float* x, int out, int in, int dt, hipStream_t st) {
    if (out == 0) return NTK_OK;
    const int grid = std::min((out + 3) / 4, 2048);
    if (dt == NTK_DT_F32)
        hipLaunchKernelGGL((gemv_dense_kernel<float, ADD>), dim3(grid), dim3(256), 0, st, y, (const float*)W, x, out, in);
    else if (dt == NTK_DT_BF16)
        hipLaunchKernelGGL((gemv_dense_kernel<uint16_t, ADD, true>), dim3(grid), dim3(256), 0, st, y, (const uint16_t*)W, x, out, in);
    else
        hipLaunchKernelGGL((gemv_dense_kernel<uint16_t, ADD>), dim3(grid), dim3(256), 0, st, y, (const uint16_t*)W, x, out, in);
    return last_launch_status();
}

}

extern "C" {

#ifdef NTK_GEMV_TRACE
NTK_EXTRA_API int ntk_debug_gemv_trace(unsigned long long* out, size_t n) {
    return hipMemcpyFromSymbol(out, HIP_SYMBOL(ntk::g_gemv_trace), n * sizeof(unsigned long long)) == hipSuccess ? 0 : -3;
}
#endif

int ntk_decode_arena_acquire(void) {
    ntk::ArenaDev* a = ntk::arena_dev(true);
    int free_ = 0;
    return a && a->owned.compare_exchange_strong(free_, 1) ? (int)(a - ntk::g_arena_dev) : -1;
}
void ntk_decode_arena_release(int device) {
    if (device >= 0 && device < ntk::kArenaDevices) ntk::g_arena_dev[device].owned.store(0);
}
float* ntk_decode_arena_slot(int slot) {
    const ntk::ArenaDev* a = ntk::arena_dev(true);
    return a && slot >= NTK_ARENA_HIDDEN && slot <= NTK_ARENA_GATE ? const_cast<float*>(a->addr[slot]) : nullptr;
}
int ntk_debug_gemv_static_x(void) { return ntk::t_last_static_x; }

size_t ntk_q8l_bytes(int rows, int in_features) { return ntk::q8l_bytes(rows, in_features); }
int ntk_q8l_pack(void* dst, const void* raw, int rows, int in_features, void* stream) {
    if (!dst || !raw) return NTK_E_NULL;
    return ntk::q8l_pack(dst, raw, rows, in_features, false, ntk::resolve_stream(stream));
}
int ntk_q8l_unpack(void* raw, const void* packed, int rows, int in_features, void* stream) {
    if (!raw || !packed) return NTK_E_NULL;
    return ntk::q8l_pack(raw, packed, rows, in_features, true, ntk::resolve_stream(stream));
}

int ntk_gemv(float* y, const void* W, const float* x, int out_features, int in_features, int weight_dtype, void* stream) {
    if (!y || !W || !x) return NTK_E_NULL;
    if (out_features < 0 || in_features <= 0) return NTK_E_SHAPE;
    hipStream_t st = ntk::resolve_stream(stream);
    if (weight_dtype == NTK_DT_F32 || weight_dtype == NTK_DT_F16 || weight_dtype == NTK_DT_BF16)
        return ntk::launch_dense<false>(y, W, x, out_features, in_features, weight_dtype, st);
    if (!ntk::is_quant(weight_dtype)) return NTK_E_DTYPE;
    ntk_gemv_seg seg{W, y, out_features, weight_dtype};
    return ntk::dispatch_quant(weight_dtype, &seg, 1, x, in_features, nullptr, 0.0f, nullptr, 0, st);
}

int ntk_gemv_add(float* y, const void* W, const float* x, int out_features, int in_features, int weight_dtype, void* stream) {
    if (!y || !W || !x) return NTK_E_NULL;
    if (out_features < 0 || in_features <= 0) return NTK_E_SHAPE;
    if (weight_dtype != NTK_DT_F16) return NTK_E_DTYPE;
    return ntk::launch_dense<true>(y, W, x, out_features, in_features, weight_dtype, ntk::resolve_stream(stream));
}


static int gemv_fused_form(const ntk_gemv_seg* segs, int nseg, const float* x, int in_features, const float* norm_w, float eps,
                           const float* resid, int silu_pair, void* stream, int xi_mode) {
    if (!segs || !x) return NTK_E_NULL;
    if (nseg < 1 || nseg > ntk::MAX_SEG) return NTK_E_SHAPE;
    if (segs[0].dtype == NTK_DT_F16 || segs[0].dtype == NTK_DT_BF16) {
        for (int i = 1; i < nseg; ++i)
            if (segs[i].dtype != segs[0].dtype) return NTK_E_DTYPE;
        return ntk::dense16_gemv_fused(segs, nseg, x, in_features, norm_w, eps, resid, silu_pair, ntk::resolve_stream(stream));
    }
    ntk_gemv_seg a[3], b[3];
    int na = 0, nb = 0;
    for (int i = 0; i < nseg; ++i) {
        if (!ntk::is_quant(segs[i].dtype)) return NTK_E_DTYPE;
        if (segs[i].dtype == segs[0].dtype) a[na++] = segs[i];
        else if (nb == 0 || segs[i].dtype == b[0].dtype) b[nb++] = segs[i];
        else return NTK_E_DTYPE;
    }
    hipStream_t st = ntk::resolve_stream(stream);
    if (nb == 0) return ntk::dispatch_quant(segs[0].dtype, segs, nseg, x, in_features, norm_w, eps, resid, silu_pair, st, xi_mode);
    if (resid || silu_pair) return NTK_E_DTYPE;
    const int da = a[0].dtype, db = b[0].dtype;
    if (da == NTK_DT_Q4_K && db == NTK_DT_Q6_K) return ntk::launch_pair<NTK_DT_Q4_K, NTK_DT_Q6_K>(a, na, b, nb, x, in_features, norm_w, eps, st);
    if (da == NTK_DT_Q6_K && db == NTK_DT_Q4_K) return ntk::launch_pair<NTK_DT_Q4_K, NTK_DT_Q6_K>(b, nb, a, na, x, in_features, norm_w, eps, st);
    if (da == NTK_DT_Q4_K && db == NTK_DT_Q5_K) return ntk::launch_pair<NTK_DT_Q4_K, NTK_DT_Q5_K>(a, na, b, nb, x, in_features, norm_w, eps, st);
    if (da == NTK_DT_Q5_K && db == NTK_DT_Q4_K) return ntk::launch_pair<NTK_DT_Q4_K, NTK_DT_Q5_K>(b, nb, a, na, x, in_features, norm_w, eps, st);
    return NTK_E_DTYPE;
}

int ntk_gemv_fused(const ntk_gemv_seg* segs, int nseg, const float* x, int in_features, const float* norm_w, float eps,
                   const float* resid, int silu_pair, void* stream) {
    return gemv_fused_form(segs, nseg, x, in_features, norm_w, eps, resid, silu_pair, stream, ntk::XI_DEFAULT);
}
int ntk_debug_gemv_fused_form(const ntk_gemv_seg* segs, int nseg, const float* x, int in_features, const float* norm_w, float eps,
                              const float* resid, int silu_pair, int integer_activations, void* stream) {
    if (integer_activations < -1 || integer_activations > 1) return NTK_E_SHAPE;
    return gemv_fused_form(segs, nseg, x, in_features, norm_w, eps, resid, silu_pair, stream, integer_activations);
}

}
```

### ntransformer_amd/csrc/gemv_core.hip.h

```cpp
#pragma once
#include "common.hip.h"
#include <algorithm>

namespace ntk {

typedef uint32_t u32x4 __attribute__((ext_vector_type(4)));

constexpr int RB = 4;
constexpr int XPITCH = 68;
constexpr int MAX_SEG = 3;
#ifndef NTK_GEMV_ABLATE
#define NTK_GEMV_ABLATE 0
#endif
constexpr int kAblate = NTK_GEMV_ABLATE;

#ifdef NTK_GEMV_TRACE
constexpr int GT_SLOTS = 64, GT_WG = 512, GT_EV = 14;
__device__ unsigned long long g_gemv_trace[GT_SLOTS][GT_WG][GT_EV];
#define GV_STAMP(ev) do { asm volatile("" ::: "memory"); gv_t[ev] = __builtin_amdgcn_s_memrealtime(); asm volatile("" ::: "memory"); } while (0)
#else
#define GV_STAMP(ev) do {} while (0)
#endif

template <int DT> struct Fmt;
template <> struct Fmt<NTK_DT_Q8_0> { static constexpr int BW = 32, BB = 34, NL = 5, MINW = 4; };
template <> struct Fmt<NTK_DT_Q4_0> { static constexpr int BW = 32, BB = 18, NL = 3, MINW = 4; };
template <> struct Fmt<NTK_DT_Q4_K> { static constexpr int BW = 256, BB = 144, NL = 3, MINW = 4; };
template <> struct Fmt<NTK_DT_Q5_K> { static constexpr int BW = 256, BB = 176, NL = 3, MINW = 4; };
template <> struct Fmt<NTK_DT_Q6_K> { static constexpr int BW = 256, BB = 210, NL = 4, MINW = 4; };

inline bool gemv_slices(int in, int align, int& ns, int& slice_cols) {
    ns = (in + 4095) / 4096;
    slice_cols = ((in + ns - 1) / ns + align - 1) / align * align;
    return ns <= 8 && (long)(ns - 1) * slice_cols < in;
}
inline bool q8l_layout(int in, int& ns, int& slice_cols) {
    if (in <= 0 || in % 256 != 0 || !gemv_slices(in, 64, ns, slice_cols)) return false;
    return slice_cols % 256 == 0 && (in - (ns - 1) * slice_cols) % 256 == 0;
}
template <int DT> constexpr bool A16_OK = (DT == NTK_DT_Q4_K || DT == NTK_DT_Q5_K);

struct GemvSeg {
    const uint8_t* W;
    float* y;
    int rows;
    int delta;
};

struct GemvParams {
    GemvSeg seg[MAX_SEG];
    int nseg;
    int total_rows;
    const float* x;
    int in;
    int ns;
    int rw;
    int slice_cols;
    int nbatch;
    int x_vec;
    const float* norm_w;
    float eps;
    const float* resid;
    int silu_pair;
    unsigned row_bytes;
#ifdef NTK_GEMV_TRACE
    int trace_slot;
#endif
};

template <int DT, bool A16> struct Dot;

typedef float f32x2 __attribute__((ext_vector_type(2)));
__device__ __forceinline__ f32x2 pkfma(f32x2 a, f32x2 b, f32x2 c) { return __builtin_elementwise_fma(a, b, c); }
__device__ __forceinline__ uint32_t opaque(uint32_t v) { asm("" : "+v"(v)); return v; }
__device__ __forceinline__ f32x2 ub01(uint32_t w) { return f32x2{ub2f(w, 0), ub2f(w, 1)}; }
__device__ __forceinline__ f32x2 ub23(uint32_t w) { return f32x2{ub2f(w, 2), ub2f(w, 3)}; }
__device__ __forceinline__ float hsum(f32x2 a, f32x2 b) { return (a.x + a.y) + (b.x + b.y); }


template <bool A16> struct Dot<NTK_DT_Q8_0, A16> {
    __device__ static float run(const uint8_t* st, int shift, int lane, int ncols, const f32x2 (&x2)[32],
                                const float (&)[4], const float (&)[2]) {
        float acc = 0.0f;
        const int o = shift + 68 * lane;
#pragma unroll
        for (int h = 0; h < 2; ++h) {
            if (ncols > 32 * h) {
                const int ob = o + 34 * h;
                const float d = h2f(lds_u16_at(st, ob));
                uint32_t q[8];
                lds_read_dwords<8>(q, st, ob + 2);
                f32x2 a0 = {0.0f, 0.0f}, a1 = {0.0f, 0.0f};
#pragma unroll
                for (int i = 0; i < 8; ++i) {
                    a0 = pkfma(f32x2{sb2f(q[i], 0), sb2f(q[i], 1)}, x2[16 * h + 2 * i], a0);
                    a1 = pkfma(f32x2{sb2f(q[i], 2), sb2f(q[i], 3)}, x2[16 * h + 2 * i + 1], a1);
                }
                acc = fmaf(d, hsum(a0, a1), acc);
            }
        }
        return acc;
    }
};

__device__ __forceinline__ float dot_q8_regs(const u32x4 (&c)[4], const uint32_t sc, const int ncols, const f32x2 (&x2)[32]) {
    float acc = 0.0f;
    if (ncols > 0) {
#pragma unroll
        for (int h = 0; h < 2; ++h) {
            const float d = h2f((uint16_t)(h ? sc >> 16 : sc & 0xFFFFu));
            const uint32_t q[8] = {c[2 * h].x, c[2 * h].y, c[2 * h].z, c[2 * h].w, c[2 * h + 1].x, c[2 * h + 1].y, c[2 * h + 1].z, c[2 * h + 1].w};
            f32x2 a0 = {0.0f, 0.0f}, a1 = {0.0f, 0.0f};
#pragma unroll
            for (int i = 0; i < 8; ++i) {
                a0 = pkfma(f32x2{sb2f(q[i], 0), sb2f(q[i], 1)}, x2[16 * h + 2 * i], a0);
                a1 = pkfma(f32x2{sb2f(q[i], 2), sb2f(q[i], 3)}, x2[16 * h + 2 * i + 1], a1);
            }
            acc = fmaf(d, hsum(a0, a1), acc);
        }
    }
    return acc;
}

template <bool A16> struct Dot<NTK_DT_Q4_0, A16> {
    __device__ static float run(const uint8_t* st, int shift, int lane, int ncols, const f32x2 (&x2)[32],
                                const float (&)[4], const float (&sx32)[2]) {
        float acc = 0.0f;
        const int o = shift + 36 * lane;
#pragma unroll
        for (int h = 0; h < 2; ++h) {
            if (ncols > 32 * h) {
                const int ob = o + 18 * h;
                const float d = h2f(lds_u16_at(st, ob));
                uint32_t q[4];
                lds_read_dwords<4>(q, st, ob + 2);
                f32x2 a0 = {0.0f, 0.0f}, a1 = {0.0f, 0.0f};
#pragma unroll
                for (int i = 0; i < 4; ++i) {
                    const uint32_t lo = opaque(q[i] & 0x0F0F0F0Fu), hi = opaque(q[i] & 0xF0F0F0F0u);
                    a0 = pkfma(ub01(lo), x2[16 * h + 2 * i], a0);
                    a1 = pkfma(ub23(lo), x2[16 * h + 2 * i + 1], a1);
                    a0 = pkfma(ub01(hi), x2[16 * h + 8 + 2 * i], a0);
                    a1 = pkfma(ub23(hi), x2[16 * h + 8 + 2 * i + 1], a1);
                }
                acc = fmaf(d, fmaf(-8.0f, sx32[h], hsum(a0, a1)), acc);
            }
        }
        return acc;
    }
};

template <bool A16>
__device__ __forceinline__ void kq_header(const uint8_t* st, int ob, int c, float& d1, float& m1, float& d2, float& m2) {
    uint32_t hd[4];
    if constexpr (A16) {
        const u32x4 v = *reinterpret_cast<const u32x4*>(st + ob);
        hd[0] = v.x; hd[1] = v.y; hd[2] = v.z; hd[3] = v.w;
    } else {
        lds_read_dwords<4>(hd, st, ob);
    }
    const float d = h2f((uint16_t)(hd[0] & 0xFFFFu)), dmin = h2f((uint16_t)(hd[0] >> 16));
    const uint32_t s0 = hd[1], s1 = hd[2], s2 = hd[3];
    const uint32_t sc_lo = s0 & 0x3F3F3F3Fu, mn_lo = s1 & 0x3F3F3F3Fu;
    const uint32_t sc_hi = (s2 & 0x0F0F0F0Fu) | ((s0 >> 2) & 0x30303030u);
    const uint32_t mn_hi = ((s2 >> 4) & 0x0F0F0F0Fu) | ((s1 >> 2) & 0x30303030u);
    const bool upper = c >= 2;
    const int sh = 16 * (c & 1);
    const uint32_t sc = (upper ? sc_hi : sc_lo) >> sh, mn = (upper ? mn_hi : mn_lo) >> sh;
    d1 = d * ub2f(sc, 0); m1 = dmin * ub2f(mn, 0);
    d2 = d * ub2f(sc, 1); m2 = dmin * ub2f(mn, 1);
}

template <int N, bool A16>
__device__ __forceinline__ void lds_read_q(uint32_t (&dst)[N], const uint8_t* st, int off) {
    if constexpr (A16) {
        static_assert(N % 4 == 0, "b128 reads");
#pragma unroll
        for (int i = 0; i < N / 4; ++i) {
            const u32x4 v = *reinterpret_cast<const u32x4*>(st + off + 16 * i);
            dst[4 * i] = v.x; dst[4 * i + 1] = v.y; dst[4 * i + 2] = v.z; dst[4 * i + 3] = v.w;
        }
    } else {
        lds_read_dwords<N>(dst, st, off);
    }
}

template <bool A16> struct Dot<NTK_DT_Q4_K, A16> {
    __device__ static float run(const uint8_t* st, int shift, int lane, int ncols, const f32x2 (&x2)[32],
                                const float (&)[4], const float (&sx32)[2]) {
        if (ncols <= 0) return 0.0f;
        const int c = lane & 3, ob = shift + 144 * (lane >> 2);
        float d1, m1, d2, m2;
        kq_header<A16>(st, ob, c, d1, m1, d2, m2);
        uint32_t q[8];
        lds_read_q<8, A16>(q, st, ob + 16 + 32 * c);
        f32x2 l0 = {0.0f, 0.0f}, l1 = {0.0f, 0.0f}, h0 = {0.0f, 0.0f}, h1 = {0.0f, 0.0f};
#pragma unroll
        for (int i = 0; i < 8; ++i) {
            const uint32_t lo = opaque(q[i] & 0x0F0F0F0Fu), hi = opaque(q[i] & 0xF0F0F0F0u);
            l0 = pkfma(ub01(lo), x2[2 * i], l0);
            l1 = pkfma(ub23(lo), x2[2 * i + 1], l1);
            h0 = pkfma(ub01(hi), x2[16 + 2 * i], h0);
            h1 = pkfma(ub23(hi), x2[16 + 2 * i + 1], h1);
        }
        float t = d1 * hsum(l0, l1);
        t = fmaf(-m1, sx32[0], t);
        t = fmaf(d2, hsum(h0, h1), t);
        t = fmaf(-m2, sx32[1], t);
        return t;
    }
};

struct XInt {
    uint32_t d[3][16];
    float inv[2];
    float sx[4];
};
template <int DT> struct DotI;

template <> struct DotI<NTK_DT_Q4_K> {
    __device__ static float run(const uint8_t* st, int lane, int ncols, const XInt& xi) {
// ... 139 lines not shown
```

Before: 561.0 tokens/s.

## Fuse greedy argmax into LM-head GEMV and carry next-token embedding

```diff
diff --git a/include/ntk_engine.h b/include/ntk_engine.h
--- a/include/ntk_engine.h
+++ b/include/ntk_engine.h
@@ -193,6 +193,11 @@
 
 int ntk_argmax_advance(const float* logits, int n, int* d_out_token, int* h_mirror, unsigned long long* h_ring4, int* d_pos,
                        float* scratch, void* stream);
+int ntk_argmax_partials(const float* logits, int n, float* scratch, int* nblk_out, void* stream);
+int ntk_gemv_rp_fused_argmax(const ntk_gemv_seg* segs, int nseg, const float* x, int in_features, const float* norm_w, float eps, float* scratch,
+                             int* nblk_out, void* stream);
+int ntk_argmax_advance_embed(const float* scratch, int nblk, int n, int* d_out_token, int* h_mirror, unsigned long long* h_ring4, int* d_pos,
+                             float* hidden_out, const void* table, int hidden, int dtype, void* stream);
 
 int ntk_debug_sclk(unsigned long long* d_out2, void* stream);
 int ntk_debug_sclk_begin(unsigned* d_flag, unsigned long long* d_out2, void* side_stream);
diff --git a/ntransformer_amd/csrc/common.hip.h b/ntransformer_amd/csrc/common.hip.h
--- a/ntransformer_amd/csrc/common.hip.h
+++ b/ntransformer_amd/csrc/common.hip.h
@@ -115,6 +115,10 @@
     return t;
 }
 
+__device__ __forceinline__ void amax_merge(float& v, int& i, float ov, int oi) {
+    if (ov > v || (ov == v && oi < i)) { v = ov; i = oi; }
+}
+
 template <int N>
 __device__ __forceinline__ void lds_read_dwords(uint32_t (&dst)[N], const uint8_t* base, int off) {
     const int a = off & ~3;
diff --git a/ntransformer_amd/csrc/elementwise.hip b/ntransformer_amd/csrc/elementwise.hip
--- a/ntransformer_amd/csrc/elementwise.hip
+++ b/ntransformer_amd/csrc/elementwise.hip
@@ -125,9 +125,6 @@
     if (e < hidden) out[(size_t)blockIdx.x * hidden + e] = embed_elem(table, tok, hidden, dt, e);
 }
 
-__device__ __forceinline__ void amax_merge(float& v, int& i, float ov, int oi) {
-    if (ov > v || (ov == v && oi < i)) { v = ov; i = oi; }
-}
 __global__ __launch_bounds__(256) void argmax_stage1(const float* __restrict__ x, int n, float* __restrict__ sv, int* __restrict__ si) {
     __shared__ float rv[4];
     __shared__ int ri[4];
@@ -211,6 +208,34 @@
     }
 }
 
+__global__ __launch_bounds__(256) void argmax_advance_embed_kernel(const float* __restrict__ sv, const int* __restrict__ si, int nblk, int n_rows,
+                                                                   int* __restrict__ d_out, int* __restrict__ h_mirror,
+                                                                   unsigned long long* __restrict__ h_ring, int* __restrict__ d_pos,
+                                                                   float* __restrict__ hidden_out, const uint8_t* __restrict__ table, int hidden, int dt) {
+    __shared__ float rv[4];
+    __shared__ int ri[4];
+    float v = -FLT_MAX;
+    int idx = 0x7FFFFFFF;
+    for (int i = threadIdx.x; i < nblk; i += blockDim.x) amax_merge(v, idx, sv[i], si[i]);
+    for (int off = 32; off > 0; off >>= 1) amax_merge(v, idx, __shfl_xor(v, off, 64), __shfl_xor(idx, off, 64));
+    if ((threadIdx.x & 63) == 0) { rv[threadIdx.x >> 6] = v; ri[threadIdx.x >> 6] = idx; }
+    __syncthreads();
+    v = rv[0]; idx = ri[0];
+    for (int w = 1; w < 4; ++w) amax_merge(v, idx, rv[w], ri[w]);
+    if ((unsigned)idx >= (unsigned)n_rows) idx = 0;
+    if (blockIdx.x == 0 && threadIdx.x == 0) {
+        const int pos = *d_pos;
+        *d_out = idx;
+        if (h_mirror) *h_mirror = idx;
+        if (h_ring)
+            __hip_atomic_store(h_ring + (pos & 3), (unsigned long long)(unsigned)idx | ((unsigned long long)(unsigned)(pos + 1) << 32),
+                               __ATOMIC_RELEASE, __HIP_MEMORY_SCOPE_SYSTEM);
+        *d_pos = pos + 1;
+    }
+    const int e = blockIdx.x * blockDim.x + threadIdx.x;
+    if (e < hidden) hidden_out[e] = embed_elem(table, idx, hidden, dt, e);
+}
+
 static inline dim3 g1(int n) { return dim3((n + 255) / 256); }
 
 }
@@ -301,10 +326,11 @@
         default: return NTK_E_DTYPE;
     }
 }
+static int argmax_blocks(int n) { return n < 256 * 8 ? 1 : (n / (256 * 8) < 1024 ? n / (256 * 8) : 1024); }
 int ntk_argmax(const float* logits, int n, int* d_out_token, int* h_mirror, float* scratch, void* stream) {
     if (!logits || !d_out_token || !scratch) return NTK_E_NULL;
     if (n <= 0) return NTK_E_SHAPE;
-    const int nblk = n < 256 * 8 ? 1 : (n / (256 * 8) < 1024 ? n / (256 * 8) : 1024);
+    const int nblk = argmax_blocks(n);
     float* sv = scratch;
     int* si = reinterpret_cast<int*>(scratch + 1024);
     hipStream_t st = resolve_stream(stream);
@@ -316,7 +342,7 @@
                        void* stream) {
     if (!logits || !d_out_token || !scratch || !d_pos) return NTK_E_NULL;
     if (n <= 0) return NTK_E_SHAPE;
-    const int nblk = n < 256 * 8 ? 1 : (n / (256 * 8) < 1024 ? n / (256 * 8) : 1024);
+    const int nblk = argmax_blocks(n);
     float* sv = scratch;
     int* si = reinterpret_cast<int*>(scratch + 1024);
     hipStream_t st = resolve_stream(stream);
@@ -324,6 +350,28 @@
     hipLaunchKernelGGL(argmax_advance_stage2, dim3(1), dim3(256), 0, st, (const float*)sv, (const int*)si, nblk, d_out_token, h_mirror, h_ring4, d_pos);
     return last_launch_status();
 }
+int ntk_argmax_partials(const float* logits, int n, float* scratch, int* nblk_out, void* stream) {
+    if (!logits || !scratch || !nblk_out) return NTK_E_NULL;
+    if (n <= 0) return NTK_E_SHAPE;
+    const int nblk = argmax_blocks(n);
+    hipLaunchKernelGGL(argmax_stage1, dim3(nblk), dim3(256), 0, resolve_stream(stream), logits, n, scratch, reinterpret_cast<int*>(scratch + 1024));
+    *nblk_out = nblk;
+    return last_launch_status();
+}
+int ntk_argmax_advance_embed(const float* scratch, int nblk, int n, int* d_out_token, int* h_mirror, unsigned long long* h_ring4, int* d_pos,
+                             float* hidden_out, const void* table, int hidden, int dtype, void* stream) {
+    if (!scratch || !d_out_token || !d_pos || !hidden_out || !table) return NTK_E_NULL;
+    if (nblk < 1 || nblk > 1024 || n <= 0 || hidden <= 0) return NTK_E_SHAPE;
+    hipLaunchKernelGGL(argmax_advance_embed_kernel, dim3((hidden + 255) / 256), dim3(256), 0, resolve_stream(stream), scratch,
+                       reinterpret_cast<const int*>(scratch + 1024), nblk, n, d_out_token, h_mirror, h_ring4, d_pos, hidden_out, (const uint8_t*)table,
+                       hidden, dtype);
+    const int st = last_launch_status();
+    if (st != NTK_OK) return st;
+    switch (dtype) {
+        case NTK_DT_F32: case NTK_DT_F16: case NTK_DT_BF16: case NTK_DT_Q8_0: case NTK_DT_Q4_0: case NTK_DT_Q4_K: case NTK_DT_Q6_K: return NTK_OK;
+        default: return NTK_E_DTYPE;
+    }
+}
 int ntk_debug_sclk(unsigned long long* d_out2, void* stream) {
     if (!d_out2) return NTK_E_NULL;
     hipLaunchKernelGGL(sclk_probe_kernel, dim3(1), dim3(64), 0, resolve_stream(stream), d_out2);
diff --git a/ntransformer_amd/csrc/engine/capi.cpp b/ntransformer_amd/csrc/engine/capi.cpp
--- a/ntransformer_amd/csrc/engine/capi.cpp
+++ b/ntransformer_amd/csrc/engine/capi.cpp
@@ -110,6 +110,11 @@
     else if (k == "prefill_row_max") E(e)->model().set_prefill_row_max(on);
     else if (k == "prefill_fused_split") E(e)->model().set_prefill_fused_split(on);
     else if (k == "attention_merge") return E(e)->model().set_attention_merge(on);
+    else if (k == "greedy_tail") {
+        const std::string v = value;
+        if (v != "0" && v != "1") { E(e)->set_error("greedy_tail must be 0 or 1"); return NTK_E_SHAPE; }
+        return E(e)->model().set_greedy_tail(on);
+    }
     else if (k == "repack") return E(e)->model().set_repack(atoi(value));
     else if (k == "score_rows") {
         const int rc = E(e)->model().set_score_rows(atoi(value));
diff --git a/ntransformer_amd/csrc/engine/embed_carry.h b/ntransformer_amd/csrc/engine/embed_carry.h
--- /dev/null
+++ b/ntransformer_amd/csrc/engine/embed_carry.h
@@ -0,0 +1,16 @@
+#pragma once
+
+namespace nt {
+
+struct EmbedCarry {
+    bool carried = false;
+
+    bool before_greedy_step() {
+        const bool need = !carried;
+        carried = true;
+        return need;
+    }
+    void invalidate() { carried = false; }
+};
+
+}
diff --git a/ntransformer_amd/csrc/engine/model.cpp b/ntransformer_amd/csrc/engine/model.cpp
--- a/ntransformer_amd/csrc/engine/model.cpp
+++ b/ntransformer_amd/csrc/engine/model.cpp
@@ -46,6 +46,7 @@
     arena_owner_ = false;
     arena_device_ = -1;
     hidden1_ = arena_attn_ = arena_gate_ = nullptr;
+    embed_carry_.invalidate();
     auto free_host = [](auto*& p) { if (p) nt_hip_free_host(p); p = nullptr; };
     free_host(h_token_); free_host(h_ring_); free_host(h_recent_); free_host(h_batch_recent_); free_host(h_batch_next_);
     sample_scratch_ = gemm_ws_ = gemm_ws2_ = nullptr;
@@ -119,6 +120,21 @@
     return NTK_OK;
 }
 
+int Model::set_greedy_tail(bool on) {
+    if (on == greedy_tail_) return NTK_OK;
+    if (!layers_.empty()) {
+        NT_TRY(sync());
+        drop_graphs();
+    }
+    greedy_tail_ = on;
+    embed_carry_.invalidate();
+    return NTK_OK;
+}
+
+bool Model::lm_head_argmax() const {
+    return repack_ && (rp_mask() & 16) && output_.rp && output_.dtype == NTK_DT_Q8_0 && output_.in_f <= 4096;
+}
+
 bool Model::fusable(int dt) const { return is_quant(dt) || (dense_fused_ && is_dense16(dt)); }
 
 int Model::set_repack(int level) {
@@ -157,6 +173,7 @@
 int Model::set_device_token(int token) {
     if (token < 0 || token >= cfg_.vocab_size) { err_ = "token id out of range"; return NTK_E_SHAPE; }
     *h_token_ = token;
+    embed_carry_.invalidate();
     return ntk_memcpy_h2d_async(d_token_, h_token_, 4, stream_);
 }
 int Model::set_device_pos(int pos) {
@@ -176,6 +193,7 @@
 int Model::sample_on_device(const int* recent, int n_recent, float repeat_penalty, float temperature, int top_k, float top_p, float r) {
     if (!sample_scratch_ || !d_recent_ || !h_recent_) return NTK_E_NOMEM;
     if (n_recent > kRecentCap) { recent += n_recent - kRecentCap; n_recent = kRecentCap; }
+    embed_carry_.invalidate();
     void* s = stream_;
     if (repeat_penalty > 1.0f && n_recent > 0) {
         memcpy(h_recent_, recent, (size_t)n_recent * 4);
@@ -314,6 +332,10 @@
 }
 
 const char* Model::decode_path() const {
+    if (greedy_tail_active() && lm_head_argmax())
+        return arena_owner_ ? "fused (5 launches/layer; static activations; greedy tail 1 launch, arg-max in the LM head)"
+                            : "fused (5 launches/layer; greedy tail 1 launch, arg-max in the LM head)";
+    if (greedy_tail_active()) return arena_owner_ ? "fused (5 launches/layer; static activations; greedy tail 1 launch)" : "fused (5 launches/layer; greedy tail 1 launch)";
     return arena_owner_ ? "fused (5 launches/layer; static activations)" : "fused (5 launches/layer)";
 }
 
diff --git a/ntransformer_amd/csrc/engine/model.h b/ntransformer_amd/csrc/engine/model.h
--- a/ntransformer_amd/csrc/engine/model.h
+++ b/ntransformer_amd/csrc/engine/model.h
@@ -5,6 +5,7 @@
 #include <cstdint>
 #include <string>
 #include <vector>
+#include "embed_carry.h"
 #include "gguf.h"
 #include "kv_cache.h"
 #include "rope_scaling.h"
@@ -120,6 +121,9 @@
     uint64_t resident_weight_bytes() const { return weight_bytes_ - raw_freed_bytes_ + repack_bytes_ + raw_scratch_bytes_; }
     int set_dense_fused(bool on);
     void set_dense_mfma16(bool on) { dense_mfma16_ = on; }
+    int set_greedy_tail(bool on);
+    bool greedy_tail_active() const { return greedy_tail_ && tp_world_ == 1; }
+    bool lm_head_argmax() const;
     bool fusable(int dt) const;
     void set_bf16_prefill(bool on) { bf16_prefill_ = on; }
     const char* decode_path() const;
@@ -163,6 +167,7 @@
     struct Views { float *q, *k, *v, *attn_out, *gate, *up; };
     Views views(int T, bool fused = false) const;
     int enqueue_token(bool greedy);
+    int embed_device_token();
     int enqueue_layers(int first, int last);
     int decode_project(const DevTensor* const* ws, float* const* ys, int n, const float* x, const DevTensor* norm, const float* resid, int kind,
                        int silu_pair = 0, bool timed = true);
@@ -217,6 +222,8 @@
     float* hidden_ = nullptr;
     float* hidden1_ = nullptr;
     bool static_act_ = true;
+    bool greedy_tail_ = true;
+    EmbedCarry embed_carry_;
     bool arena_owner_ = false;
     int arena_device_ = -1;
     float* arena_attn_ = nullptr;
diff --git a/ntransformer_amd/csrc/engine/model_debug.cpp b/ntransformer_amd/csrc/engine/model_debug.cpp
--- a/ntransformer_amd/csrc/engine/model_debug.cpp
+++ b/ntransformer_amd/csrc/engine/model_debug.cpp
@@ -10,6 +10,7 @@
     const size_t bytes = (size_t)T * cfg_.hidden_size * 4;
     void* s = stream_;
     float* const hid = mode == 0 ? hidden_ : hidden1_;
+    embed_carry_.invalidate();
     NT_TRY(ntk_memcpy_h2d_async(hid, hidden_in, bytes, s));
     int rc;
     if (mode == 0) {
diff --git a/ntransformer_amd/csrc/engine/model_decode.cpp b/ntransformer_amd/csrc/engine/model_decode.cpp
--- a/ntransformer_amd/csrc/engine/model_decode.cpp
+++ b/ntransformer_amd/csrc/engine/model_decode.cpp
@@ -20,22 +20,43 @@
     if (begin) prof_->push_back({cls, e, nullptr, 1, false}); else prof_->back().b = e;
 }
 
+int Model::embed_device_token() {
+    const int est = ntk_embed_rows(hidden1_, token_embd_.ptr, d_token_, 1, cfg_.hidden_size, token_embd_.dtype, stream_);
+    return est == NTK_E_DTYPE ? (int)NTK_OK : est;
+}
+
 int Model::enqueue_token(bool greedy) {
     const int H = cfg_.hidden_size;
     void* s = stream_;
     tp_call_ = 0;
-    prof_mark(2, true);
-    const int est = ntk_embed_rows(hidden1_, token_embd_.ptr, d_token_, 1, H, token_embd_.dtype, s);
-    prof_mark(2, false);
-    if (est != NTK_OK && est != NTK_E_DTYPE) return est;
+    const bool tail = greedy && greedy_tail_active();
+    if (!tail) {
+        prof_mark(2, true);
+        const int est = embed_device_token();
+        prof_mark(2, false);
+        NT_TRY(est);
+    }
     NT_TRY(enqueue_layers(0, cfg_.n_layers));
     const DevTensor* const w = &output_;
     const bool timed = fusable(w->dtype);
+    int nblk = 0;
     if (timed) prof_mark(0, true);
-    NT_TRY(decode_project(&w, &logits_, 1, hidden1_, &output_norm_, nullptr, 16, 0, false));
+    int st = NTK_E_DTYPE;
+    if (tail && lm_head_argmax()) {
+        const ntk_gemv_seg seg{w->rp, logits_, (int)w->out_f, w->dtype};
+        st = ntk_gemv_rp_fused_argmax(&seg, 1, hidden1_, (int)w->in_f, (const float*)output_norm_.ptr, cfg_.norm_eps, argmax_scratch_, &nblk, s);
+    }
+    if (not_taken(st)) { nblk = 0; st = decode_project(&w, &logits_, 1, hidden1_, &output_norm_, nullptr, 16, 0, false); }
     if (timed) prof_mark(0, false);
+    NT_TRY(st);
     prof_mark(2, true);
-    if (greedy) NT_TRY(ntk_argmax_advance(logits_, cfg_.vocab_size, d_token_, h_token_, h_ring_, d_pos_, argmax_scratch_, s));
+    if (tail) {
+        if (nblk == 0) NT_TRY(ntk_argmax_partials(logits_, cfg_.vocab_size, argmax_scratch_, &nblk, s));
+        const int est = ntk_argmax_advance_embed(argmax_scratch_, nblk, cfg_.vocab_size, d_token_, h_token_, h_ring_, d_pos_, hidden1_, token_embd_.ptr, H,
+                                                 token_embd_.dtype, s);
+        if (est != NTK_OK && est != NTK_E_DTYPE) return est;
+    }
+    else if (greedy) NT_TRY(ntk_argmax_advance(logits_, cfg_.vocab_size, d_token_, h_token_, h_ring_, d_pos_, argmax_scratch_, s));
     else NT_TRY(ntk_advance_pos(d_pos_, s));
     if (tp_world_ > 1) NT_TRY(ntk_tp_advance_epoch(tp_comm_, s));
     prof_mark(2, false);
@@ -161,6 +182,8 @@
 }
 
 int Model::decode_step_fused(bool greedy, bool use_graph) {
+    if (greedy && greedy_tail_active()) { if (embed_carry_.before_greedy_step()) NT_TRY(embed_device_token()); }
+    else embed_carry_.invalidate();
     pick_attention_regime();
     if (!use_graph) return enqueue_token(greedy);
     ihipGraphExec_t*& slot = graphs_[greedy ? 1 : 0][attn_regime_];
@@ -176,6 +199,8 @@
 int Model::profile_token(float ms[4], int calls[4], bool coarse) {
     std::vector<Timed> rec;
     rec.reserve(1024);
+    if (greedy_tail_active() && embed_carry_.before_greedy_step()) NT_TRY(embed_device_token());
+    embed_carry_.invalidate();
     prof_ = &rec;
     prof_coarse_ = coarse;
     pick_attention_regime();
diff --git a/ntransformer_amd/csrc/engine/model_prompt.cpp b/ntransformer_amd/csrc/engine/model_prompt.cpp
--- a/ntransformer_amd/csrc/engine/model_prompt.cpp
+++ b/ntransformer_amd/csrc/engine/model_prompt.cpp
@@ -30,6 +30,7 @@
 }
 
 int Model::embed_rows(float* out, const int* ids_dev, int n) {
+    embed_carry_.invalidate();
     const int st = ntk_embed_rows(out, token_embd_.ptr, ids_dev, n, cfg_.hidden_size, token_embd_.dtype, stream_);
     if (st != NTK_E_DTYPE) return st;
     fprintf(stderr, "Error: Unsupported embedding dtype: %s\n", dtype_name(token_embd_.dtype));
@@ -91,6 +92,7 @@
     void* s = stream_;
     const Views act = views(T);
     PassStatus ok;
+    embed_carry_.invalidate();
     const bool batched = batched_prefill_ && T > 1;
     const bool bf16_now = bf16_prefill_ && gemm_ws_ && T > 1;
     OperandPlanes planes{{gemm_ws_, gemm_ws2_}};
diff --git a/ntransformer_amd/csrc/gemv.hip b/ntransformer_amd/csrc/gemv.hip
--- a/ntransformer_amd/csrc/gemv.hip
+++ b/ntransformer_amd/csrc/gemv.hip
@@ -1,6 +1,7 @@
 #include "gemv_core.hip.h"
 #include <algorithm>
 #include <atomic>
+#include <cfloat>
 #include <cmath>
 #include <cstddef>
 #include <mutex>
@@ -23,12 +24,13 @@
     return XS == XS_HIDDEN ? g_decode_arena.hidden : XS == XS_ATTN ? g_decode_arena.attn_out : g_decode_arena.gate;
 }
 
-template <int DT, bool NORM, bool XFAST, bool A16, bool XI = false, bool LM = false, int NSF = NS_ANY, int XS = XS_NONE>
+template <int DT, bool NORM, bool XFAST, bool A16, bool XI = false, bool LM = false, int NSF = NS_ANY, int XS = XS_NONE, bool AMAX = false>
 __device__ __forceinline__ void gemv_quant_body(const GemvParams& p, const int bid, const int nblk) {
     using F = Fmt<DT>;
     static_assert(!LM || (DT == NTK_DT_Q8_0 && !A16 && !XI), "lane-major rows: Q8_0");
     static_assert(NSF == NS_ANY || LM, "compile-time slice forms: the lane-major kernels");
     static_assert(XS == XS_NONE || (LM && XFAST && NSF != NS_ANY), "early-x forms: the lane-major kernels, fast prologue");
+    static_assert(!AMAX || (LM && NSF == NS_ONE), "arg-max epilogue: lane-major rows of one slice");
     constexpr int NL = LM ? 4 : F::NL;
     constexpr int STAGE = LM ? 0 : NL * 1024 + 64;
     extern __shared__ __attribute__((aligned(16))) uint8_t smem[];
@@ -402,6 +404,8 @@
         for (int j = 0; j < 32; ++j) if ((j & 8) != 0) x2[j] *= 0.0625f;
     }
     float gate_carry = 0.0f;
+    float am_v = -FLT_MAX;
+    int am_i = 0x7FFFFFFF;
     float pair_g = 0.0f, pair_u = 0.0f;
     auto silu_flush = [&](const int last_pair) {
         const int base = last_pair & ~63;
@@ -488,6 +492,7 @@
                 float v = tot;
                 if (p.resid != nullptr && seg == 0) v = res + v;
                 p.seg[seg].y[row] = v;
+                if constexpr (AMAX) amax_merge(am_v, am_i, v, row);
             }
         } else {
             const int b = q / RB, i = q % RB;
@@ -511,6 +516,18 @@
         }
         for (; done < p.nbatch; ++done) __syncthreads();
     }
+    if constexpr (AMAX) {
+        int* const red_i = reinterpret_cast<int*>(red) + 8;
+        if (lane == 63) { red[wave] = am_v; red_i[wave] = am_i; }
+        __syncthreads();
+        if (tid == 0) {
+            float v = red[0];
+            int i = red_i[0];
+            for (int w = 1; w < nwaves; ++w) amax_merge(v, i, red[w], red_i[w]);
+            p.amax_v[bid] = v;
+            p.amax_i[bid] = i;
+        }
+    }
 #ifdef NTK_GEMV_TRACE
     GV_STAMP(6);
     if (tid == 0 && bid < GT_WG) {
@@ -523,6 +540,10 @@
 template <bool NORM, bool XFAST, int NSF, int XS = XS_NONE>
 __global__ __launch_bounds__(512, Fmt<NTK_DT_Q8_0>::MINW) void gemv_q8l_kernel(const GemvParams p) {
     gemv_quant_body<NTK_DT_Q8_0, NORM, XFAST, false, false, true, NSF, XS>(p, (int)blockIdx.x, (int)gridDim.x);
+}
+template <bool NORM, bool XFAST, int XS = XS_NONE>
+__global__ __launch_bounds__(512, Fmt<NTK_DT_Q8_0>::MINW) void gemv_q8l_amax_kernel(const GemvParams p) {
+    gemv_quant_body<NTK_DT_Q8_0, NORM, XFAST, false, false, true, NS_ONE, XS, true>(p, (int)blockIdx.x, (int)gridDim.x);
 }
 template <bool UNPACK>
 __global__ __launch_bounds__(256) void q8l_pack_kernel(uint8_t* __restrict__ dst, const uint8_t* __restrict__ src, const int rows, const int in,
@@ -810,8 +831,8 @@
     return XS_NONE;
 }
 
-int q8l_gemv_fused(const ntk_gemv_seg* segs, int nseg, const float* x, int in, const float* norm_w, float eps, const float* resid,
-                   int silu_pair, hipStream_t st) {
+static int q8l_launch(const ntk_gemv_seg* segs, int nseg, const float* x, int in, const float* norm_w, float eps, const float* resid, int silu_pair,
+                      float* amax_v, int* amax_i, int* nblk_out, hipStream_t st) {
     int ns, sc;
     t_last_static_x = XS_NONE;
     if (!q8l_layout(in, ns, sc)) return NTK_E_SHAPE;
@@ -820,8 +841,23 @@
     GemvLaunch L;
     const int rc = prepare_quant<NTK_DT_Q8_0>(segs, nseg, x, in, norm_w, eps, resid, silu_pair, max_workgroups(), L, true);
     if (rc != NTK_OK) return rc;
+    using KernelFn = void (*)(const GemvParams);
+    if (amax_v) {
+        if (nseg != 1 || resid || silu_pair || L.p.ns != 1 || L.p.total_rows == 0 || L.nwaves > 8 || L.grid > 1024 || L.lds > 64 * 1024) return NTK_E_SHAPE;
+        L.p.amax_v = amax_v;
+        L.p.amax_i = amax_i;
+        static const KernelFn atable[2][2] = {{gemv_q8l_amax_kernel<false, false>, gemv_q8l_amax_kernel<false, true>},
+                                              {gemv_q8l_amax_kernel<true, false>, gemv_q8l_amax_kernel<true, true>}};
+        KernelFn fn = atable[norm_w ? 1 : 0][L.xfast ? 1 : 0];
+        if (L.xfast && L.nwaves == 8 && norm_w && static_x_slot(x, in) == XS_HIDDEN) {
+            fn = gemv_q8l_amax_kernel<true, true, XS_HIDDEN>;
+            t_last_static_x = XS_HIDDEN;
+        }
+        hipLaunchKernelGGL(fn, dim3(L.grid), dim3(64 * L.nwaves), L.lds, st, L.p);
+        *nblk_out = L.grid;
+        return last_launch_status();
+    }
     if (L.p.total_rows == 0) return NTK_OK;
-    using KernelFn = void (*)(const GemvParams);
 #define Q8L_FORMS(NORM, XFAST) {gemv_q8l_kernel<NORM, XFAST, NS_ONE>, gemv_q8l_kernel<NORM, XFAST, NS_SPLIT>}
     static const KernelFn table[2][2][2] = {{Q8L_FORMS(false, false), Q8L_FORMS(false, true)}, {Q8L_FORMS(true, false), Q8L_FORMS(true, true)}};
 #undef Q8L_FORMS
@@ -855,6 +891,10 @@
     return last_launch_status();
 }
 
+int q8l_gemv_fused(const ntk_gemv_seg* segs, int nseg, const float* x, int in, const float* norm_w, float eps, const float* resid,
+                   int silu_pair, hipStream_t st) {
+    return q8l_launch(segs, nseg, x, in, norm_w, eps, resid, silu_pair, nullptr, nullptr, nullptr, st);
+}
 
 template <int DTA, int DTB>
 static int launch_pair(const ntk_gemv_seg* sa, int na, const ntk_gemv_seg* sb, int nb, const float* x, int in, const float* norm_w,
@@ -934,6 +974,18 @@
 }
 int ntk_debug_gemv_static_x(void) { return ntk::t_last_static_x; }
 
+int ntk_gemv_rp_fused_argmax(const ntk_gemv_seg* segs, int nseg, const float* x, int in_features, const float* norm_w, float eps, float* scratch,
+                             int* nblk_out, void* stream) {
+    if (!segs || !x || !scratch || !nblk_out) return NTK_E_NULL;
+    if (nseg != 1 || segs[0].rows <= 0) return NTK_E_SHAPE;
+    if (segs[0].dtype != NTK_DT_Q8_0) return NTK_E_DTYPE;
+    if (!segs[0].W || !segs[0].y) return NTK_E_NULL;
+    if (in_features <= 0 || in_features % 256 != 0 || in_features > 32768) return NTK_E_SHAPE;
+    if ((reinterpret_cast<uintptr_t>(x) & 15) || (norm_w && (reinterpret_cast<uintptr_t>(norm_w) & 15))) return NTK_E_ALIGN;
+    return ntk::q8l_launch(segs, 1, x, in_features, norm_w, eps, nullptr, 0, scratch, reinterpret_cast<int*>(scratch + 1024), nblk_out,
+                           ntk::resolve_stream(stream));
+}
+
 size_t ntk_q8l_bytes(int rows, int in_features) { return ntk::q8l_bytes(rows, in_features); }
 int ntk_q8l_pack(void* dst, const void* raw, int rows, int in_features, void* stream) {
     if (!dst || !raw) return NTK_E_NULL;
diff --git a/ntransformer_amd/csrc/gemv_core.hip.h b/ntransformer_amd/csrc/gemv_core.hip.h
--- a/ntransformer_amd/csrc/gemv_core.hip.h
+++ b/ntransformer_amd/csrc/gemv_core.hip.h
@@ -63,10 +63,15 @@
     const float* resid;
     int silu_pair;
     unsigned row_bytes;
+    float* amax_v;
+    int* amax_i;
 #ifdef NTK_GEMV_TRACE
     int trace_slot;
 #endif
 };
+#ifndef NTK_GEMV_TRACE
+static_assert(sizeof(GemvParams) == 160, "GemvParams: 160 bytes of kernel arguments");
+#endif
 
 template <int DT, bool A16> struct Dot;
 
```

Result: no change. 564.1 tokens/s, median of 6 (+0.5%).
